# buckbaskin/parakeet_slam

Measured on AMD Instinct MI355X. Metric: particle*landmark EKF updates/sec (whole filter step), higher is better.
Workload: dtype f64

## Files before the change

include/parakeet_slam.h:

```cpp
#ifndef PARAKEET_SLAM_H_
#define PARAKEET_SLAM_H_

#include <stddef.h>
#include <stdint.h>

#ifdef __cplusplus
extern "C" {
#endif
#if defined(__GNUC__)
#pragma GCC visibility push(default)
#endif

#define PK_ABI_VERSION 1

typedef enum pk_status {
  PK_OK = 0,
  PK_ERR_INVALID = -1,
  PK_ERR_HIP = -2,
  PK_ERR_STATE = -3,
  PK_ERR_UNSUPPORTED = -4,
  PK_ERR_NOMEM = -5
} pk_status;

#define PK_LANDMARK_POTENTIAL 0x40000000
// ... 154 lines not shown
int pk_proposal_ranges_state(const pk_filter* f, int32_t* on);

int pk_proposal_grow(pk_filter* f, int32_t on);
int pk_proposal_grow_state(const pk_filter* f, int32_t* on);

int pk_assoc_unique(pk_filter* f, int32_t on);
int pk_assoc_unique_state(const pk_filter* f, int32_t* on);
int pk_assoc_unique_stats(pk_filter* f, int64_t out[4]);

int pk_set_shard(pk_filter* f, int64_t global_offset);
int pk_shard_max_logw(pk_filter* f, double* max_logw);
int64_t pk_shard_num_blocks(const pk_filter* f);
int pk_shard_block_totals(pk_filter* f, double gmax, int32_t weight_domain, double* totals);
int pk_shard_offspring(pk_filter* f, const double* global_totals, int64_t n_global_blocks,
                       int64_t first_block, int64_t global_particles, double u, int32_t last_shard,
                       int64_t* slot_hi);
int64_t pk_particle_bytes(const pk_filter* f);
int pk_pack_particles(pk_filter* f, const int64_t* local_idx, int64_t n, void* dev_buf);
int pk_adopt_particles(pk_filter* f, const int64_t* src, const void* dev_buf, int64_t n_received);

int pk_shard_max_logw_dev(pk_filter* f, double* dev_out);
int pk_shard_block_totals_dev(pk_filter* f, const double* dev_gmax, int32_t weight_domain,
                              double* dev_totals);
int pk_shard_plan_dev(pk_filter* f, const double* dev_global_totals, int64_t n_global_blocks,
                      int64_t first_block, int64_t global_particles, double u, int32_t last_shard,
                      int32_t world, int64_t* dev_ranges);
int pk_shard_pack_slots_dev(pk_filter* f, int64_t j0, int64_t j1, int64_t slot_lo, int64_t slot_hi, void* dev_buf);
int pk_shard_logw_dev(pk_filter* f, double* dev_out);
int pk_shard_plan_global_dev(pk_filter* f, const double* dev_global_logw, int64_t global_particles, const double* dev_gmax,
                             int32_t weight_domain, double u, int32_t last_shard, int32_t world, int64_t* dev_ranges);
int pk_shard_download_offspring(pk_filter* f, int64_t* slot_hi);
int pk_shard_pack_dev(pk_filter* f, const int64_t* ranges, int32_t world, int32_t rank, void* dev_buf);
int pk_shard_adopt_dev(pk_filter* f, int32_t rank, const void* dev_recv, int64_t n_received);

int pk_shard_local_span_dev(pk_filter* f, int64_t* dev_out2);
int pk_shard_adopt_local_dev(pk_filter* f, int32_t rank);
int pk_shard_adopt_remote_dev(pk_filter* f, int32_t rank, const void* dev_recv, int64_t n_received);
int pk_motion_range(pk_filter* f, double v, double w, double dt, uint64_t seed, uint64_t draw, int64_t p0, int64_t p1);
int pk_staged_takes_regs(pk_filter* f);
int pk_observe_staged_range(pk_filter* f, int32_t fresh, int64_t p0, int64_t p1, int32_t first, int32_t last);

int pk_shard_state_dev(pk_filter* f, double* dev_out);
int pk_shard_plan_balanced_dev(pk_filter* f, const double* dev_global_state, int64_t global_particles, const double* dev_gmax,
                               int32_t weight_domain, double u, int32_t world, int32_t rank, int64_t* dev_table);
int pk_shard_pack_balanced_dev(pk_filter* f, const int64_t* table, int32_t world, int32_t rank, void* dev_buf);
int pk_shard_adopt_balanced_dev(pk_filter* f, const int64_t* table, int32_t world, int32_t rank, const void* dev_recv,
                                int64_t n_received, int32_t mode);
int pk_shard_pack_balanced_loop_dev(pk_filter* f, int64_t keep, int64_t a0, int64_t a1, void* dev_buf);
int pk_shard_download_logical(pk_filter* f, int64_t* logical);
int pk_shard_upload_logical(pk_filter* f, const int64_t* logical);
int pk_shard_download_balanced_plan(pk_filter* f, int64_t* rel, int64_t* Hl, int32_t* alive);
int pk_shard_reset_placement(pk_filter* f);
int pk_shard_download_balanced_offspring(pk_filter* f, int64_t global_particles, int64_t* H);
int pk_shard_balanced_errors(pk_filter* f, int64_t* count);

#define PK_PROBE_LEN 79
int pk_probe(int32_t device, const double pose[3], const double mean[5], const double cov[25],
             const double blob[4], const double Qt[16], double* out);

enum {
  PK_MATH_LOG_FEW_ULP = 0,
  PK_MATH_PUB_LOG = 1,
  PK_MATH_PUB_RECIP = 2,
  PK_MATH_ATAN2 = 3,
  PK_MATH_ROUND_DOWN_F32 = 4,
  PK_MATH_KEY = 5,
  PK_MATH_FAR_BOUND = 6,
  PK_MATH_PR_FROM_PARTS = 7,
  PK_MATH_EKF_UPDATE = 9,
  PK_MATH_MATCH = 10,
  PK_MATH_COUNT = 11
};
int pk_probe_math(int32_t device, int32_t op, int64_t n, const double* in, double* out);

int pk_probe_bearing(int32_t device, int32_t what, int64_t n, const double* in, double* out);

int pk_probe_range(int32_t device, int32_t what, int64_t n, const double* in, double* out);

int pk_enable_timing(pk_filter* f, int32_t mask);
int pk_reset_timings(pk_filter* f);
int pk_timings(pk_filter* f, double ms[PK_T_COUNT], int64_t launches[PK_T_COUNT]);
int pk_observe_bytes(const pk_filter* f, int32_t num_blobs, int64_t* algorithmic, int64_t* moved);
int pk_colour_table_stats(pk_filter* f, int64_t out[4]);
enum {
  PK_ROUTE_NONE = 0,
  PK_ROUTE_KNOWN_IDS = 1,
  PK_ROUTE_ML_GENERAL = 2,
  PK_ROUTE_ML_HANDOFF = 3,
  PK_ROUTE_ML_SWEEP = 4,
  PK_ROUTE_ML_FUSED = 5,
  PK_ROUTE_ML_REGS = 6,
  PK_ROUTE_DENSE = 8,
  PK_ROUTE_ML_PUB_BIG = 9,
};
int pk_observe_route(const pk_filter* f);
int pk_download_sources(pk_filter* f, int32_t* src);
int pk_observe_flagged(pk_filter* f, int64_t* flagged, int64_t* cand_overflow);
int pk_observe_retry_rows(pk_filter* f, int64_t* wanted, int64_t* capacity);
int pk_observe_published(pk_filter* f, int32_t* published);
int pk_observe_pub_stats(pk_filter* f, int64_t stats[6]);
int pk_observe_lean_stats(pk_filter* f, int64_t out[3]);
int pk_observe_flags(pk_filter* f, uint8_t* flags);

typedef struct pk_rng pk_rng;
int pk_rng_create_numpy(uint32_t seed, pk_rng** out);
int pk_rng_create_python(uint32_t seed, pk_rng** out);
int pk_rng_destroy(pk_rng* r);
int pk_rng_standard_normal(pk_rng* r, int64_t n, double* out);
int pk_rng_random(pk_rng* r, int64_t n, double* out);

#if defined(__GNUC__)
#pragma GCC visibility pop
#endif
#ifdef __cplusplus
}
#endif
#endif
```

parakeet_slam_amd/_lib.py:

```python
from __future__ import annotations

import ctypes as C
import os

import numpy as np

from . import adaptive, mapsum, path

HERE = os.path.dirname(os.path.abspath(__file__))
LIB_PATH = os.path.join(HERE, "libparakeet_slam.so")

PK_OK = 0
PK_ERR_INVALID, PK_ERR_HIP, PK_ERR_STATE, PK_ERR_UNSUPPORTED, PK_ERR_NOMEM = -1, -2, -3, -4, -5
PK_WEIGHTS_LINEAR, PK_WEIGHTS_LOG = 0, 1
PK_PATH_UNIFORM = 2
PK_MAP_UNIFORM, PK_MAP_WEIGHTED = mapsum.UNIFORM, mapsum.WEIGHTED
PK_LANDMARK_POTENTIAL = 0x40000000
PK_GROW_VIEW_STATS_BYTES = 32
PK_T_NAMES = ("motion", "assoc", "observe", "weights", "resample", "summary", "materialise", "propose")
PK_T_COUNT = len(PK_T_NAMES)
PK_PROBE_LEN = 79
(PK_MATH_LOG_FEW_ULP, PK_MATH_PUB_LOG, PK_MATH_PUB_RECIP, PK_MATH_ATAN2, PK_MATH_ROUND_DOWN_F32, PK_MATH_KEY, PK_MATH_FAR_BOUND,
 PK_MATH_PR_FROM_PARTS) = range(8)
PK_MATH_EKF_UPDATE, PK_MATH_MATCH = 9, 10
# ... 68 lines not shown
    "pk_path_download": (C.c_int, [_h, C.c_int32, C.c_int32, _dp, _ip]),
    "pk_path_upload": (C.c_int, [_h, C.c_int32, C.c_int64, _dp, _ip]),
    "pk_path_trace": (C.c_int, [_h, _lp, C.c_int64, _dp]),
    "pk_path_summary": (C.c_int, [_h, _dp, _dp, _lp]),
    "pk_path_summary_weighted": (C.c_int, [_h, C.c_int32, _dp, _dp, _dp]),
    "pk_path_trunk_enable": (C.c_int, [_h, C.c_int32]),
    "pk_path_settle": (C.c_int, [_h, C.c_int32, C.c_int32]),
    "pk_path_trunk_shape": (C.c_int, [_h, C.POINTER(C.c_int32), _lp, _lp]),
    "pk_path_trunk_download": (C.c_int, [_h, C.c_int64, C.c_int64, _dp]),
    "pk_path_trunk_upload": (C.c_int, [_h, C.c_int64, C.c_int64, _dp]),
    "pk_path_trunk_summary": (C.c_int, [_h, C.c_int64, C.c_int64, _dp, _dp, _lp]),
    "pk_best_particle": (C.c_int, [_h, _lp, _dp]),
    "pk_step": (C.c_int, [_h, C.c_double, C.c_double, C.c_double, _dp, C.c_uint64, C.c_uint64, _dp, C.c_int32,
                          _ip, C.c_double, C.c_int32]),
    "pk_resample_adaptive": (C.c_int, [_h, C.c_double, C.c_int32, C.c_double, _lp]),
    "pk_step_adaptive": (C.c_int, [_h, C.c_double, C.c_double, C.c_double, _dp, C.c_uint64, C.c_uint64, _dp, C.c_int32,
                                   _ip, C.c_double, C.c_int32, C.c_double]),
    "pk_resample_stats": (C.c_int, [_h, _dp, C.POINTER(C.c_int32), _lp]),
    "pk_weight_sums": (C.c_int, [_h, C.c_int32, C.c_double, _dp]),
    "pk_summary_weighted": (C.c_int, [_h, C.c_int32, _dp, _dp, _dp]),
    "pk_odom_delta": (C.c_int, [_dp, _dp, C.c_double, _dp]),
    "pk_odom_sigmas": (C.c_int, [_dp, _dp, _dp]),
    "pk_motion_odom": (C.c_int, [_h, _dp, _dp, _dp, C.c_uint64, C.c_uint64]),
    "pk_propose": (C.c_int, [_h, C.c_double, C.c_double, C.c_double, _dp, C.c_uint64, C.c_uint64, _dp, C.c_int32, _ip, C.c_int32, _ip]),
    "pk_propose_odom": (C.c_int, [_h, _dp, _dp, _dp, C.c_uint64, C.c_uint64, _dp, C.c_int32, _ip, C.c_int32, _ip]),
    "pk_proposal_download": (C.c_int, [_h, _dp, _dp, _ip]),
    "pk_proposal_ranges": (C.c_int, [_h, C.c_int32]),
    "pk_proposal_ranges_state": (C.c_int, [_h, C.POINTER(C.c_int32)]),
    "pk_proposal_grow": (C.c_int, [_h, C.c_int32]),
    "pk_proposal_grow_state": (C.c_int, [_h, C.POINTER(C.c_int32)]),
    "pk_assoc_unique": (C.c_int, [_h, C.c_int32]),
    "pk_assoc_unique_state": (C.c_int, [_h, C.POINTER(C.c_int32)]),
    "pk_assoc_unique_stats": (C.c_int, [_h, _lp]),
    "pk_motion_odom_range": (C.c_int, [_h, _dp, _dp, C.c_uint64, C.c_uint64, C.c_int64, C.c_int64]),
    "pk_step_odom": (C.c_int, [_h, _dp, _dp, _dp, C.c_uint64, C.c_uint64, _dp, C.c_int32, _ip, C.c_double, C.c_int32, C.c_double]),
    "pk_shard_max_logw": (C.c_int, [_h, _dp]),
    "pk_shard_num_blocks": (C.c_int64, [_h]),
    "pk_shard_block_totals": (C.c_int, [_h, C.c_double, C.c_int32, _dp]),
    "pk_set_shard": (C.c_int, [_h, C.c_int64]),
    "pk_shard_offspring": (C.c_int, [_h, _dp, C.c_int64, C.c_int64, C.c_int64, C.c_double, C.c_int32, _lp]),
    "pk_shard_max_logw_dev": (C.c_int, [_h, C.c_void_p]),
    "pk_shard_block_totals_dev": (C.c_int, [_h, C.c_void_p, C.c_int32, C.c_void_p]),
    "pk_shard_plan_dev": (C.c_int, [_h, C.c_void_p, C.c_int64, C.c_int64, C.c_int64, C.c_double, C.c_int32, C.c_int32,
                                    C.c_void_p]),
    "pk_shard_logw_dev": (C.c_int, [_h, C.c_void_p]),
    "pk_shard_plan_global_dev": (C.c_int, [_h, C.c_void_p, C.c_int64, C.c_void_p, C.c_int32, C.c_double, C.c_int32, C.c_int32,
                                           C.c_void_p]),
    "pk_shard_download_offspring": (C.c_int, [_h, _lp]),
    "pk_shard_pack_dev": (C.c_int, [_h, _lp, C.c_int32, C.c_int32, C.c_void_p]),
    "pk_shard_pack_slots_dev": (C.c_int, [_h, C.c_int64, C.c_int64, C.c_int64, C.c_int64, C.c_void_p]),
    "pk_shard_adopt_dev": (C.c_int, [_h, C.c_int32, C.c_void_p, C.c_int64]),
    "pk_shard_local_span_dev": (C.c_int, [_h, C.c_void_p]),
    "pk_shard_adopt_local_dev": (C.c_int, [_h, C.c_int32]),
    "pk_shard_adopt_remote_dev": (C.c_int, [_h, C.c_int32, C.c_void_p, C.c_int64]),
    "pk_shard_state_dev": (C.c_int, [_h, C.c_void_p]),
    "pk_shard_plan_balanced_dev": (C.c_int, [_h, C.c_void_p, C.c_int64, C.c_void_p, C.c_int32, C.c_double, C.c_int32, C.c_int32,
                                             C.c_void_p]),
    "pk_shard_pack_balanced_dev": (C.c_int, [_h, _lp, C.c_int32, C.c_int32, C.c_void_p]),
    "pk_shard_adopt_balanced_dev": (C.c_int, [_h, _lp, C.c_int32, C.c_int32, C.c_void_p, C.c_int64, C.c_int32]),
    "pk_shard_pack_balanced_loop_dev": (C.c_int, [_h, C.c_int64, C.c_int64, C.c_int64, C.c_void_p]),
    "pk_shard_download_logical": (C.c_int, [_h, _lp]),
    "pk_shard_reset_placement": (C.c_int, [_h]),
    "pk_shard_upload_logical": (C.c_int, [_h, _lp]),
    "pk_shard_download_balanced_plan": (C.c_int, [_h, _lp, _lp, _ip]),
    "pk_shard_download_balanced_offspring": (C.c_int, [_h, C.c_int64, _lp]),
    "pk_shard_balanced_errors": (C.c_int, [_h, _lp]),
    "pk_motion_range": (C.c_int, [_h, C.c_double, C.c_double, C.c_double, C.c_uint64, C.c_uint64, C.c_int64, C.c_int64]),
    "pk_staged_takes_regs": (C.c_int, [_h]),
    "pk_observe_staged_range": (C.c_int, [_h, C.c_int32, C.c_int64, C.c_int64, C.c_int32, C.c_int32]),
    "pk_particle_bytes": (C.c_int64, [_h]),
    "pk_pack_particles": (C.c_int, [_h, _lp, C.c_int64, C.c_void_p]),
    "pk_adopt_particles": (C.c_int, [_h, _lp, C.c_void_p, C.c_int64]),
    "pk_probe": (C.c_int, [C.c_int32, _dp, _dp, _dp, _dp, _dp, _dp]),
    "pk_probe_math": (C.c_int, [C.c_int32, C.c_int32, C.c_int64, _dp, _dp]),
    "pk_probe_bearing": (C.c_int, [C.c_int32, C.c_int32, C.c_int64, _dp, _dp]),
    "pk_probe_range": (C.c_int, [C.c_int32, C.c_int32, C.c_int64, _dp, _dp]),
    "pk_scan_ranges": (C.c_int, [_h, _dp, _dp, C.c_int32]),
    "pk_scan_ranges_state": (C.c_int, [_h, C.POINTER(C.c_int32), C.POINTER(C.c_int32)]),
    "pk_enable_timing": (C.c_int, [_h, C.c_int32]),
    "pk_reset_timings": (C.c_int, [_h]),
    "pk_timings": (C.c_int, [_h, _dp, _lp]),
    "pk_observe_bytes": (C.c_int, [_h, C.c_int32, _lp, _lp]),
    "pk_colour_table_stats": (C.c_int, [_h, _lp]),
    "pk_observe_route": (C.c_int, [_h]),
    "pk_download_sources": (C.c_int, [_h, _ip]),
    "pk_observe_flagged": (C.c_int, [_h, _lp, _lp]),
    "pk_observe_retry_rows": (C.c_int, [_h, _lp, _lp]),
    "pk_grow_enable": (C.c_int, [_h, C.c_int32, C.c_int32, C.c_double]),
    "pk_grow_download": (C.c_int, [_h, C.c_int64, C.c_int64, _ip, _dp, _ip]),
    "pk_grow_upload": (C.c_int, [_h, C.c_int64, C.c_int64, _ip, _dp, _ip]),
    "pk_grow_shape": (C.c_int, [_h, C.POINTER(C.c_int32), C.POINTER(C.c_int32), C.POINTER(C.c_int32)]),
    "pk_grow_init": (C.c_int, [_h, C.c_int32, C.c_double]),
    "pk_grow_init_mode": (C.c_int, [_h, C.POINTER(C.c_int32), _dp]),
    "pk_grow_ranges": (C.c_int, [_h, C.c_int32]),
    "pk_grow_ranges_state": (C.c_int, [_h, C.POINTER(C.c_int32)]),
    "pk_grow_retire": (C.c_int, [_h, C.c_int32, C.c_int32]),
    "pk_grow_clocks_download": (C.c_int, [_h, C.c_int64, C.c_int64, _ip, _up, _ip, _ip, _up]),
    "pk_grow_clocks_upload": (C.c_int, [_h, C.c_int64, C.c_int64, _ip, _up, _ip, _ip, _up]),
    "pk_grow_view": (C.c_int, [_h, C.c_double, C.c_double, C.c_double, C.c_int32]),
    "pk_grow_view_state": (C.c_int, [_h, C.POINTER(C.c_int32), _dp, C.POINTER(C.c_int32)]),
    "pk_grow_view_stats": (C.c_int, [_h, _lp]),
    "pk_observe_published": (C.c_int, [_h, C.POINTER(C.c_int32)]),
    "pk_observe_flags": (C.c_int, [_h, _bp]),
    "pk_observe_pub_stats": (C.c_int, [_h, _lp]),
    "pk_observe_lean_stats": (C.c_int, [_h, _lp]),
    "pk_rng_create_numpy": (C.c_int, [C.c_uint32, C.POINTER(_h)]),
    "pk_rng_create_python": (C.c_int, [C.c_uint32, C.POINTER(_h)]),
    "pk_rng_destroy": (C.c_int, [_h]),
    "pk_rng_standard_normal": (C.c_int, [_h, C.c_int64, _dp]),
    "pk_rng_random": (C.c_int, [_h, C.c_int64, _dp]),
}


class PkError(RuntimeError):
    def __init__(self, status, message):
        super().__init__("parakeet_slam [%d]: %s" % (status, message))
        self.status = status


_lib = None


def load():
    global _lib
    if _lib is not None:
        return _lib
    if not os.path.exists(LIB_PATH):
        raise OSError(
            "%s is missing: build it with `python -m parakeet_slam_amd.build` (hipcc, gfx950). "
            "There is no CPU fallback for the particle update." % LIB_PATH
        )
    lib = C.CDLL(LIB_PATH)
    for name, (res, args) in SIGNATURES.items():
        fn = getattr(lib, name)
        fn.restype = res
        fn.argtypes = args
    ver = lib.pk_abi_version()
    if ver != PK_ABI_VERSION:
        raise OSError("libparakeet_slam.so has ABI %d, the binding expects %d: rebuild" % (ver, PK_ABI_VERSION))
    _lib = lib
    return lib


def check(status):
    if status != PK_OK:
        lib = load()
        msg = lib.pk_last_error().decode("utf-8", "replace") or lib.pk_status_string(status).decode()
        raise PkError(status, msg)


def dptr(a):
    return a.ctypes.data_as(_dp) if a is not None else None


def iptr(a):
    return a.ctypes.data_as(_ip) if a is not None else None


def lptr(a):
    return a.ctypes.data_as(_lp) if a is not None else None


def f64(a, shape=None):
    a = np.ascontiguousarray(a, dtype=np.float64)
    if shape is not None:
        a = a.reshape(shape)
# ... 455 lines not shown
        check(self._lib.pk_shard_state_dev(self._h, C.c_void_p(out_ptr)))

    def shard_plan_balanced_dev(self, gstate_ptr, global_particles, gmax_ptr, domain, u, world, rank, table_ptr):
        check(self._lib.pk_shard_plan_balanced_dev(self._h, C.c_void_p(gstate_ptr), int(global_particles), C.c_void_p(gmax_ptr),
                                                   int(domain), float(u), int(world), int(rank), C.c_void_p(table_ptr)))

    def shard_pack_balanced_dev(self, table, world, rank, buf_ptr):
        t = np.ascontiguousarray(table, dtype=np.int64)
        check(self._lib.pk_shard_pack_balanced_dev(self._h, lptr(t), int(world), int(rank), C.c_void_p(buf_ptr)))

    def shard_adopt_balanced_dev(self, table, world, rank, recv_ptr, n_received, mode):
        t = np.ascontiguousarray(table, dtype=np.int64)
        check(self._lib.pk_shard_adopt_balanced_dev(self._h, lptr(t), int(world), int(rank), C.c_void_p(recv_ptr), int(n_received),
                                                    int(mode)))

    def shard_pack_balanced_loop_dev(self, keep, a0, a1, buf_ptr):
        check(self._lib.pk_shard_pack_balanced_loop_dev(self._h, int(keep), int(a0), int(a1), C.c_void_p(buf_ptr)))

    def download_logical(self):
        out = np.empty(self.P, dtype=np.int64)
        check(self._lib.pk_shard_download_logical(self._h, lptr(out)))
        return out

    def upload_logical(self, logical):
        a = np.ascontiguousarray(logical, dtype=np.int64).reshape(self.P)
        check(self._lib.pk_shard_upload_logical(self._h, lptr(a)))

    def shard_download_balanced_plan(self):
        rel, Hl, alive = np.empty(self.P + 1, dtype=np.int64), np.empty(self.P, dtype=np.int64), np.empty(self.P, dtype=np.int32)
        check(self._lib.pk_shard_download_balanced_plan(self._h, lptr(rel), lptr(Hl), iptr(alive)))
        return rel, Hl, alive[alive >= 0]

    def reset_placement(self):
        check(self._lib.pk_shard_reset_placement(self._h))

    def shard_download_balanced_offspring(self, global_particles):
        out = np.empty(int(global_particles) + 1, dtype=np.int64)
        check(self._lib.pk_shard_download_balanced_offspring(self._h, int(global_particles), lptr(out)))
        return out

    def shard_balanced_errors(self):
        out = np.zeros(1, dtype=np.int64)
        check(self._lib.pk_shard_balanced_errors(self._h, lptr(out)))
        return int(out[0])

    def motion_range(self, v, w, dt, seed, draw, p0, p1):
        check(self._lib.pk_motion_range(self._h, float(v), float(w), float(dt), int(seed), int(draw), int(p0), int(p1)))

    def motion_odom_range(self, delta, alphas, seed, draw, p0, p1):
        d, a = f64(delta, (3,)), f64(alphas, (4,))
        check(self._lib.pk_motion_odom_range(self._h, dptr(d), dptr(a), int(seed), int(draw), int(p0), int(p1)))

    def staged_takes_regs(self):
        return bool(self._lib.pk_staged_takes_regs(self._h))

    def observe_staged_range(self, fresh, p0, p1, first, last):
        check(self._lib.pk_observe_staged_range(self._h, 1 if fresh else 0, int(p0), int(p1), 1 if first else 0, 1 if last else 0))

    ROUTES = {0: "none", 1: "known_ids", 2: "ml_general", 3: "ml_handoff", 4: "ml_sweep", 5: "ml_fused", 6: "ml_regs", 8: "dense", 9: "ml_pub_big"}

    def observe_route(self):
        return self.ROUTES[int(self._lib.pk_observe_route(self._h))]

    def observe_flagged(self):
        a, b = C.c_int64(), C.c_int64()
        check(self._lib.pk_observe_flagged(self._h, C.byref(a), C.byref(b)))
        return int(a.value), int(b.value)

    def observe_pub_stats(self):
        a = np.zeros(6, dtype=np.int64)
        check(self._lib.pk_observe_pub_stats(self._h, lptr(a)))
        return dict(zip(("entries", "contested_blobs", "multi_landmarks", "longest_list", "entry_capacity", "instance"), (int(v) for v in a)))

    def observe_lean_stats(self):
        a = np.zeros(3, dtype=np.int64)
        check(self._lib.pk_observe_lean_stats(self._h, lptr(a)))
        return dict(zip(("marked", "in_use", "fallbacks"), (int(v) for v in a)))

    def colour_table_stats(self):
        a = np.zeros(4, dtype=np.int64)
        check(self._lib.pk_colour_table_stats(self._h, lptr(a)))
        return dict(zip(("engaged", "depth", "scans", "materialisations"), (int(v) for v in a)))

    def grow_enable(self, preset_landmarks, reading_capacity=64, pair_threshold=30.0):
        check(self._lib.pk_grow_enable(self._h, int(preset_landmarks), int(reading_capacity), float(pair_threshold)))

    def grow_shape(self):
        a, b, c = C.c_int32(), C.c_int32(), C.c_int32()
        check(self._lib.pk_grow_shape(self._h, C.byref(a), C.byref(b), C.byref(c)))
        return int(a.value), int(b.value), int(c.value)

    def grow_init(self, mode, min_parallax=0.0):
        if isinstance(mode, str):
            if mode not in LANDMARK_INITS:
                raise ValueError("grow_init: %r is neither %s" % (mode, " nor ".join(repr(k) for k in LANDMARK_INITS)))
            mode = LANDMARK_INITS[mode]
        check(self._lib.pk_grow_init(self._h, int(mode), float(min_parallax)))

    def grow_init_mode(self):
        m, a = C.c_int32(), C.c_double()
        check(self._lib.pk_grow_init_mode(self._h, C.byref(m), C.byref(a)))
        return {v: k for k, v in LANDMARK_INITS.items()}[int(m.value)], float(a.value)

    def grow_ranges(self, on=True):
        check(self._lib.pk_grow_ranges(self._h, int(on)))

    def grow_ranges_state(self):
        on = C.c_int32()
        check(self._lib.pk_grow_ranges_state(self._h, C.byref(on)))
        return bool(on.value)

    def grow_download(self, p0=0, p1=None, counters=True, readings=True, slot_ids=True):
        p1 = self.P if p1 is None else p1
        _, S, R = self.grow_shape()
        n = p1 - p0
        c = np.empty((n, 4), dtype=np.int32) if counters else None
        r = np.empty((n, R, 8), dtype=np.float64) if readings else None
        s = np.empty((n, S), dtype=np.int32) if slot_ids else None
        check(self._lib.pk_grow_download(self._h, int(p0), int(p1), iptr(c), dptr(r), iptr(s)))
        return c, r, s

    def grow_upload(self, p0, p1, counters=None, readings=None, slot_ids=None):
        _, S, R = self.grow_shape()
        n = p1 - p0
        c = None if counters is None else np.ascontiguousarray(counters, dtype=np.int32).reshape(n, 4)
        r = None if readings is None else f64(readings, (n, R, 8))
        s = None if slot_ids is None else np.ascontiguousarray(slot_ids, dtype=np.int32).reshape(n, S)
        check(self._lib.pk_grow_upload(self._h, int(p0), int(p1), iptr(c), dptr(r), iptr(s)))

    def grow_retire(self, reading_max_age=0, potential_max_idle=0):
        check(self._lib.pk_grow_retire(self._h, int(reading_max_age), int(potential_max_idle)))

    def grow_clocks_download(self, p0=0, p1=None):
        p1 = self.P if p1 is None else p1
        _, S, R = self.grow_shape()
        n = p1 - p0
        c, sc = np.empty((n, 4), dtype=np.int32), np.empty((n, R), dtype=np.uint32)
        se, si = np.empty((n, S), dtype=np.int32), np.empty((n, S), dtype=np.int32)
        now = C.c_uint32(0)
        check(self._lib.pk_grow_clocks_download(self._h, int(p0), int(p1), iptr(c), sc.ctypes.data_as(_up), iptr(se), iptr(si), C.byref(now)))
        return c, sc, se, si, int(now.value)

    def grow_clocks_upload(self, p0, p1, counters=None, reading_scan=None, slot_seen=None, slot_idle=None, scan_now=None):
        _, S, R = self.grow_shape()
        n = p1 - p0
        c = None if counters is None else np.ascontiguousarray(counters, dtype=np.int32).reshape(n, 4)
        sc = None if reading_scan is None else np.ascontiguousarray(reading_scan, dtype=np.uint32).reshape(n, R)
        se = None if slot_seen is None else np.ascontiguousarray(slot_seen, dtype=np.int32).reshape(n, S)
        si = None if slot_idle is None else np.ascontiguousarray(slot_idle, dtype=np.int32).reshape(n, S)
        now = None if scan_now is None else C.byref(C.c_uint32(int(scan_now) & 0xFFFFFFFF))
        check(self._lib.pk_grow_clocks_upload(self._h, int(p0), int(p1), iptr(c), None if sc is None else sc.ctypes.data_as(_up), iptr(se),
                                              iptr(si), now))

    def grow_view(self, half_fov, range_min=0.0, range_max=float("inf"), confirmed_max_misses=0):
        check(self._lib.pk_grow_view(self._h, float(half_fov), float(range_min), float(range_max), int(confirmed_max_misses)))

    def grow_view_state(self):
        on, c, v = C.c_int32(), C.c_int32(), np.zeros(3, dtype=np.float64)
        check(self._lib.pk_grow_view_state(self._h, C.byref(on), dptr(v), C.byref(c)))
        return bool(on.value), (float(v[0]), float(v[1]), float(v[2])), int(c.value)

    def grow_view_stats(self):
        out = np.zeros(4, dtype=np.int64)
        check(self._lib.pk_grow_view_stats(self._h, out.ctypes.data_as(_lp)))
        return out

# ... 121 lines not shown
```

parakeet_slam_amd/csrc/pk_api.hip:

```cpp
#include "pk_filter.hpp"

extern "C" {
int pk_download_landmarks(pk_filter* f, int64_t p0, int64_t p1, double* means, double* covs, int32_t* counts);
int pk_upload_landmarks(pk_filter* f, int64_t p0, int64_t p1, const double* means, const double* covs, const int32_t* counts);
}

#ifdef PK_STAMPS
namespace pk { void debug_read_stamps(unsigned long long* out, bool reset); void debug_read_fused_stamps(unsigned long long* out, bool reset); void debug_read_regs_stamps(unsigned long long* out, bool reset); void debug_read_pub_stamps(unsigned long long* out, bool reset); void debug_read_pub_wave_stamps(unsigned long long* out, bool reset); }
#endif

namespace {
thread_local std::string g_last_error;
}

int fail(int code, const char* fmt, ...) {
  char buf[512];
  va_list ap;
  va_start(ap, fmt);
  vsnprintf(buf, sizeof(buf), fmt, ap);
  va_end(ap);
  g_last_error = buf;
  return code;
}

// ... 264 lines not shown
  delete f;
  return PK_OK;
}

int pk_set_stream(pk_filter* f, void* hip_stream) {
  if (!f) return fail(PK_ERR_INVALID, "pk_set_stream: NULL handle");
  int rc;
  if ((rc = use_device(f))) return rc;
  if ((rc = drain_timings(f))) return rc;
  PK_HIP(hipStreamSynchronize(f->stream));
  f->stream = hip_stream ? (hipStream_t)hip_stream : f->own_stream;
  return PK_OK;
}

int pk_synchronize(pk_filter* f) {
  if (!f) return fail(PK_ERR_INVALID, "pk_synchronize: NULL handle");
  int rc;
  if ((rc = use_device(f))) return rc;
  PK_HIP(hipStreamSynchronize(f->stream));
  return unique_error(f, "pk_synchronize");
}

int64_t pk_num_particles(const pk_filter* f) { return f ? f->d.P : -1; }
int32_t pk_num_landmarks(const pk_filter* f) { return f ? f->d.lay.L : -1; }
int64_t pk_device_bytes(const pk_filter* f) { return f ? (int64_t)f->mem.device_bytes() : -1; }

int pk_set_measurement_noise(pk_filter* f, const double Qt[16]) {
  if (!f || !Qt) return fail(PK_ERR_INVALID, "pk_set_measurement_noise: NULL argument");
  for (int i = 0; i < 16; ++i)
    if (!std::isfinite(Qt[i])) return fail(PK_ERR_INVALID, "Qt is not finite");
  double scale = 0;
  for (int i = 0; i < 4; ++i) scale = fmax(scale, fabs(Qt[i * 5]));
  bool coupled = false;
  for (int j = 1; j < 4; ++j)
    if (fabs(Qt[j]) > 1e-14 * scale || fabs(Qt[j * 4]) > 1e-14 * scale) coupled = true;
  for (int i = 1; i < 4; ++i)
    for (int j = i + 1; j < 4; ++j)
      if (fabs(Qt[i * 4 + j] - Qt[j * 4 + i]) > 1e-9 * (scale > 0 ? scale : 1.0)) coupled = true;
  int rc;
  if ((rc = use_device(f))) return rc;
  if (f->ct_updated) {
    bool untouched = false;
    if (f->ct_eligible && f->ct_built && !coupled && (rc = ct_maps_untouched(f, &untouched))) return rc;
    if (untouched) f->ct_updated = false;
    else if ((rc = ct_end(f))) return rc;
  }
  if (coupled && !f->dense && (rc = relayout(f, true, f->map_loaded))) return rc;
  for (int i = 0; i < 16; ++i) f->qt16[i] = Qt[i];
  f->qt_dense = coupled;
  f->qt = NoiseD{Qt[0], Qt[5], 0.5 * (Qt[6] + Qt[9]), 0.5 * (Qt[7] + Qt[13]), Qt[10], 0.5 * (Qt[11] + Qt[14]), Qt[15]};
  return PK_OK;
}

int pk_upload_map(pk_filter* f, const double* means, const double* covs, const uint8_t* immutable) {
  if (!f) return fail(PK_ERR_INVALID, "pk_upload_map: NULL handle");
  const MapLayout& lay = f->d.lay;
  const int L = lay.L;
  if (L > 0 && (!means || !covs)) return fail(PK_ERR_INVALID, "pk_upload_map: NULL means/covs");
  int rc;
  if ((rc = use_device(f))) return rc;
  bool need_dense = f->qt_dense;
  for (int l = 0; l < L; ++l) {
    for (int i = 0; i < 5; ++i)
      if (!std::isfinite(means[l * 5 + i])) return fail(PK_ERR_INVALID, "landmark %d: mean is not finite", l + 1);
    const int c = classify_covariance(covs + (size_t)l * 25, l);
    if (c < 0) return c;
    need_dense |= c == 1;
  }
  if ((rc = relayout(f, need_dense, false))) return rc;
  std::vector<unsigned char> slot(lay.slot_bytes, 0);
  std::vector<unsigned char> imm((size_t)lay.Lp, 0);
  for (int l = 0; l < L; ++l) {
    pack_landmark(lay, slot.data(), l, means + (size_t)l * 5, covs + (size_t)l * 25);
    imm[l] = immutable ? (immutable[l] != 0) : 0;
  }
  PK_HIP(hipMemcpyAsync(f->slot_tmp, slot.data(), lay.slot_bytes, hipMemcpyHostToDevice, f->stream));
  PK_HIP(hipMemcpyAsync(f->d.immutable, imm.data(), imm.size(), hipMemcpyHostToDevice, f->stream));
  launch_broadcast_slot(f->stream, f->d, f->slot_tmp);
  f->colour_rows_valid = true;
  f->ct_engaged = false;
  f->ct_built = false;
  f->ct_updated = false;
  f->ct_eligible = false;
  if (!f->dense && lay.Lp > 2 * kPubSmallThreads && L <= kRegsMaxL) {
    if ((rc = dev_lazy(f, &f->ct_base, (size_t)6 * lay.Lp))) return rc;
    PK_HIP(hipMemcpyAsync(f->ct_base, slot.data() + (size_t)F_CRR * lay.Lp * sizeof(double), (size_t)6 * lay.Lp * sizeof(double),
                          hipMemcpyHostToDevice, f->stream));
    f->ct_eligible = true;
  }
  PK_HIP(hipStreamSynchronize(f->stream));
  f->src_identity = true;
  f->map_loaded = true;
  return PK_OK;
}

int pk_upload_poses(pk_filter* f, const double* xyhw) {
  poses_change(f);
  if (!f || !xyhw) return fail(PK_ERR_INVALID, "pk_upload_poses: NULL argument");
  int rc;
  if ((rc = use_device(f))) return rc;
  const int64_t P = f->d.P;
  std::vector<double> soa((size_t)P * 4);
  for (int64_t i = 0; i < P; ++i) {
    soa[i] = xyhw[4 * i];
    soa[P + i] = xyhw[4 * i + 1];
    soa[2 * P + i] = xyhw[4 * i + 2];
    double w = xyhw[4 * i + 3];
    if (!(w >= 0.0) || !std::isfinite(w)) return fail(PK_ERR_INVALID, "pk_upload_poses: weight of particle %lld is negative, infinite or NaN", (long long)i);
    soa[3 * P + i] = std::log(w);
  }
  const int c = f->d.cur;
  PK_HIP(hipMemcpyAsync(f->d.x[c], soa.data(), P * 8, hipMemcpyHostToDevice, f->stream));
  PK_HIP(hipMemcpyAsync(f->d.y[c], soa.data() + P, P * 8, hipMemcpyHostToDevice, f->stream));
  PK_HIP(hipMemcpyAsync(f->d.h[c], soa.data() + 2 * P, P * 8, hipMemcpyHostToDevice, f->stream));
  PK_HIP(hipMemcpyAsync(f->d.logw[c], soa.data() + 3 * P, P * 8, hipMemcpyHostToDevice, f->stream));
  PK_HIP(hipStreamSynchronize(f->stream));
  f->gmax_fused = false;
  path_clear(f);
  return PK_OK;
}

int pk_upload_pose(pk_filter* f, int64_t p, const double xyhw[4]) {
  if (!f || !xyhw) return fail(PK_ERR_INVALID, "pk_upload_pose: NULL argument");
  if (p < 0 || p >= f->d.P) return fail(PK_ERR_INVALID, "pk_upload_pose: particle %lld of %lld", (long long)p, (long long)f->d.P);
  for (int i = 0; i < 3; ++i)
    if (!std::isfinite(xyhw[i])) return fail(PK_ERR_INVALID, "pk_upload_pose: pose component %d is not finite", i);
  if (!(xyhw[3] >= 0.0) || !std::isfinite(xyhw[3])) return fail(PK_ERR_INVALID, "pk_upload_pose: the weight is negative, infinite or NaN");
  int rc;
  if ((rc = use_device(f))) return rc;
  f->pose_part_ok = false;
  const double v4[4] = {xyhw[0], xyhw[1], xyhw[2], std::log(xyhw[3])};
  const int c = f->d.cur;
  double* const dst[4] = {f->d.x[c] + p, f->d.y[c] + p, f->d.h[c] + p, f->d.logw[c] + p};
  for (int i = 0; i < 4; ++i) PK_HIP(hipMemcpyAsync(dst[i], &v4[i], 8, hipMemcpyHostToDevice, f->stream));
  PK_HIP(hipStreamSynchronize(f->stream));
  f->gmax_fused = false;
  return PK_OK;
}

int pk_download_poses(pk_filter* f, double* xyhw) {
  if (!f || !xyhw) return fail(PK_ERR_INVALID, "pk_download_poses: NULL argument");
  int rc;
  if ((rc = use_device(f))) return rc;
  const int64_t P = f->d.P;
  std::vector<double> soa((size_t)P * 4);
  const int c = f->d.cur;
  PK_HIP(hipMemcpyAsync(soa.data(), f->d.x[c], P * 8, hipMemcpyDeviceToHost, f->stream));
  PK_HIP(hipMemcpyAsync(soa.data() + P, f->d.y[c], P * 8, hipMemcpyDeviceToHost, f->stream));
  PK_HIP(hipMemcpyAsync(soa.data() + 2 * P, f->d.h[c], P * 8, hipMemcpyDeviceToHost, f->stream));
  PK_HIP(hipMemcpyAsync(soa.data() + 3 * P, f->d.logw[c], P * 8, hipMemcpyDeviceToHost, f->stream));
  PK_HIP(hipStreamSynchronize(f->stream));
  for (int64_t i = 0; i < P; ++i) {
    xyhw[4 * i] = soa[i];
    xyhw[4 * i + 1] = soa[P + i];
    xyhw[4 * i + 2] = soa[2 * P + i];
    xyhw[4 * i + 3] = std::exp(soa[3 * P + i]);
  }
  return PK_OK;
}

int pk_download_log_weights(pk_filter* f, double* logw) {
  if (!f || !logw) return fail(PK_ERR_INVALID, "pk_download_log_weights: NULL argument");
  int rc;
  if ((rc = use_device(f))) return rc;
  PK_HIP(hipMemcpyAsync(logw, f->d.logw[f->d.cur], (size_t)f->d.P * sizeof(double), hipMemcpyDeviceToHost, f->stream));
  PK_HIP(hipStreamSynchronize(f->stream));
  return PK_OK;
}

int pk_upload_log_weights(pk_filter* f, const double* logw) {
  if (!f || !logw) return fail(PK_ERR_INVALID, "pk_upload_log_weights: NULL argument");
// ... 607 lines not shown
```

parakeet_slam_amd/csrc/pk_api_observe.hip:

```cpp
#include "pk_filter.hpp"

static int host_word(pk_filter* f, unsigned** p) {
  if (*p) return PK_OK;
  int rc;
  if ((rc = host_alloc(f, p, 16, hipHostMallocDefault))) return rc;
  **p = 0u;
  return PK_OK;
}

int refuse_bearing(const pk_filter* f, const char* who, const char* what) {
  if (f && f->model == PK_MODEL_BEARING)
    return fail(PK_ERR_UNSUPPORTED, "%s: the bearing measurement model (pk_set_measurement_model) has no kernel for %s; "
                                    "pk_set_measurement_model(f, PK_MODEL_REFERENCE) takes it", who, what);
  return PK_OK;
}

static void observe_done(pk_filter* f) {
  f->src_identity = true;
  f->d.alt = nullptr;
  f->gmax_fused = true;
}

static ColourTable ct_view(const pk_filter* f) { return ColourTable{f->ct_tab, f->ct_depth}; }
static int ensure_colour_rows(pk_filter* f) {
  if (f->colour_rows_valid) return PK_OK;
  {
    Span t(f, PK_T_MATERIALISE);
    launch_colour_rows(f->stream, f->d, ct_view(f), f->ct_qt);
  }
  PK_LAUNCH_CHECK("ensure_colour_rows");
  f->colour_rows_valid = true;
  f->ct_whole += 1;
  return PK_OK;
}
int colour_rows_for_download(pk_filter* f, int64_t p0, int64_t p1) {
  if (f->colour_rows_valid || p0 >= p1) return PK_OK;
  if (p0 == 0 && p1 == f->d.P) return ensure_colour_rows(f);
  {
    Span t(f, PK_T_MATERIALISE);
    ParticleRange range;
    range.p0 = p0;
    range.p1 = p1;
    launch_colour_rows(f->stream, f->d, ct_view(f), f->ct_qt, range);
  }
  PK_LAUNCH_CHECK("colour_rows_for_download");
  return PK_OK;
}
int ct_end(pk_filter* f) {
  f->ct_eligible = false;
  f->ct_engaged = false;
  return ensure_colour_rows(f);
}
static bool ct_state_ok(const pk_filter* f) {
  if (f->opt.colour_table == 0 || !f->ct_eligible || f->ct_sharded || f->grow_on || f->dense || !f->ct_base) return false;
  if (f->d.lay.Lp <= 2 * kPubSmallThreads) return false;
  const int margin = f->opt.colour_table_margin >= 0 ? f->opt.colour_table_margin : std::min(16, f->ct_depth > 0 ? f->ct_depth / 2 : 16);
  if (margin > 0 && f->ct_built && f->ct_seen && (int64_t)*reinterpret_cast<volatile unsigned*>(f->ct_seen) + margin >= f->ct_depth) return false;
  return true;
}
int ct_maps_untouched(pk_filter* f, bool* untouched) {
  *untouched = false;
  if (!f->ct_max_dev || !f->ct_seen) return PK_OK;
  PK_HIP(hipMemsetAsync(f->ct_max_dev + 1, 0, sizeof(unsigned), f->stream));
  launch_colour_counts_any(f->stream, f->d, f->ct_max_dev + 1);
  PK_LAUNCH_CHECK("colour counts");
  PK_HIP(hipMemcpyAsync(f->ct_seen + 1, f->ct_max_dev + 1, sizeof(unsigned), hipMemcpyDeviceToHost, f->stream));
  PK_HIP(hipStreamSynchronize(f->stream));
  *untouched = f->ct_seen[1] == 0u;
  return PK_OK;
}
static int ct_engage(pk_filter* f) {
  int rc;
  const int Lp = f->d.lay.Lp;
  const int depth = f->ct_built ? f->ct_depth : f->opt.colour_table_depth;
  if ((rc = host_word(f, &f->ct_seen))) return rc;
  if ((rc = dev_lazy(f, &f->ct_max_dev, 16))) return rc;
  const bool same_qt = memcmp(&f->ct_qt, &f->qt, sizeof(NoiseD)) == 0;
  if (f->ct_built && same_qt && f->ct_depth == depth) return PK_OK;
  if (!f->ct_tab || f->ct_depth != depth) {
    PK_HIP(hipStreamSynchronize(f->stream));
    dev_free(f, &f->ct_tab);
    if ((rc = dev_alloc(f, &f->ct_tab, (size_t)depth * 6 * Lp))) return rc;
    f->ct_depth = depth;
  }
  f->ct_qt = f->qt;
  launch_colour_table(f->stream, f->ct_base, f->ct_tab, depth, Lp, f->ct_qt);
  PK_HIP(hipMemsetAsync(f->ct_max_dev, 0, 16, f->stream));
  *f->ct_seen = 0u;
  PK_LAUNCH_CHECK("colour table");
  f->ct_built = true;
  return PK_OK;
}

static int64_t retry_rows(const pk_filter* f) {
  return std::min<int64_t>(f->d.P, std::max<int64_t>(std::max<int64_t>(1024, f->d.P / 16), f->retry_rows_min));
}
static int ensure_handoff(pk_filter* f, int B, int slots, bool lists = true, bool retry_only = false) {
  if (retry_only && f->retry_seen) {
    const int64_t wanted = *reinterpret_cast<volatile unsigned*>(f->retry_seen);
    if (wanted > retry_rows(f)) f->retry_rows_min = std::min<int64_t>(f->d.P, wanted + wanted / 4);
  }
  const int64_t rows = retry_only ? retry_rows(f) : f->d.P;
  const int64_t need_l = lists ? rows * (int64_t)f->d.lay.Lp * (slots == kSweepSlots ? 2 : 1) : 0;
  const int64_t need_b = lists ? rows * (int64_t)std::max(B, 1) : 0;
  int rc;
  if (retry_only && (rc = dev_lazy(f, &f->fh.row_of, (size_t)f->d.P))) return rc;
  if ((rc = dev_reserve(f, &f->fh.lmpass, &f->fh_cap_l, need_l, need_l))) return rc;
  if ((rc = dev_reserve(f, &f->fh.bcount, &f->fh_cap_b, need_b, need_b))) return rc;
  return dev_lazy(f, &f->fh.pflag, (size_t)f->d.P);
}

constexpr int64_t kPubSmallAutoWork = 5000000;
constexpr int kPubSmallAutoLandmarks = 128;

static ScanPlan plan_scan(const pk_filter* f, int B, bool use_grid, int ncell, int n9, bool want_fast, bool finalize, bool grow, bool whole) {
  ScanPlan p;
  if (!use_grid) return p;
  p.kind = ScanKind::General;
  if (f->model == PK_MODEL_BEARING) return p;
  if (f->uq.on) return p;
  const int L = f->d.lay.L, Lp = f->d.lay.Lp;
  const bool sweep = L > kFastMaxL || f->opt.fast_observe >= 2;
  auto sweep_fits = [&] { return observe_sweep_plan(f->d, B).grid > 0; };
  auto limited = [&](int ecap) { return f->opt.pub_entry_limit > 0 && ecap > f->opt.pub_entry_limit ? f->opt.pub_entry_limit : ecap; };
  const bool lists_both_ways = f->opt.pub_step && f->opt.cand_lists;
  const bool onepass = want_fast && !finalize && f->opt.fast_observe == 1 && B > 0 && (!grow || (lists_both_ways && B <= 32 * 176));
  if (onepass && f->opt.fused_step && !sweep && n9 > 0 && fused_lds_bytes(ncell, B, n9) <= kFusedMaxLds &&
      (!grow || (step_pub_entry_capacity_small(B) > 0 && B <= 32 * 32))) {
    const bool wanted = grow || (f->opt.pub_small >= 0 ? f->opt.pub_small != 0
                                                   : f->d.P * (int64_t)L >= kPubSmallAutoWork && L >= kPubSmallAutoLandmarks);
    p.kind = wanted && lists_both_ways && step_pub_entry_capacity_small(B) > 0 ? ScanKind::PubSmall : ScanKind::Fused;
    p.route = PK_ROUTE_ML_FUSED;
    if (p.kind == ScanKind::PubSmall) {
      p.cand_slots = kCandSlots;
      p.ecap = limited(step_pub_entry_capacity_small(B));
    }
  } else if (onepass && f->opt.regs_step && L > kFastMaxL && L <= kRegsMaxL && n9 > 0 && regs_lds_bytes(ncell, B, n9) <= kMaxDynLds &&
             (!grow || (step_pub_entry_capacity(B) > 0 && regs_cand_lds_bytes(Lp, B) <= kMaxDynLds && B <= 32 * 96))) {
    p.lists = f->opt.regs_retry && sweep_fits();
    p.retry = p.lists && !grow;
    p.slots = p.lists ? kSweepSlots : kFastSlots;
    p.kind = ScanKind::Regs;
    p.route = PK_ROUTE_ML_REGS;
    if (f->opt.cand_lists && regs_cand_lds_bytes(Lp, B) <= kMaxDynLds) {
      p.cand_slots = kCandSlots;
      p.ecap = f->opt.pub_step ? limited(step_pub_entry_capacity(B)) : 0;
      if (p.ecap > 0) p.kind = f->opt.far_prune || grow ? ScanKind::Pub : ScanKind::PubRegs;
    }
  } else if (onepass && lists_both_ways && L > kRegsMaxL && L <= kPubBigMaxL && step_pub_big_entry_capacity(B) > 0 && sweep_fits()) {
    p.kind = ScanKind::PubBig;
    p.route = PK_ROUTE_ML_PUB_BIG;
    p.lists = true;
    p.retry = !grow;
    p.slots = kSweepSlots;
    p.cand_slots = 2 * kCandSlots;
    p.ecap = limited(step_pub_big_entry_capacity(B));
    if (f->opt.duo_on) {
      step_pub_duo_limits(B, Lp, f->opt.duo_on, &p.duo);
      p.duo.ecap = limited(p.duo.ecap);
      p.duo.park_limit = f->opt.duo_park_limit;
    }
  } else if (want_fast && !grow && !finalize && f->opt.fast_observe && B > 0 && (sweep ? sweep_fits() : observe_fast_lds_bytes(B) <= kMaxDynLds)) {
    p.kind = sweep ? ScanKind::HandoffSweep : ScanKind::HandoffFast;
    p.route = sweep ? PK_ROUTE_ML_SWEEP : PK_ROUTE_ML_HANDOFF;
    p.lists = true;
    p.slots = sweep && (B >= 3000 || f->opt.fast_observe == 3) ? kSweepSlots : kFastSlots;
    if (f->opt.cand_lists && L < 65535) p.cand_slots = 2 * kCandSlots;
  }
  p.publish = p.ecap > 0;
// ... 148 lines not shown
  if ((rc = dev_lazy(f, &f->cand_dev, Lpp * 3))) return rc;
  if (!plan.publish) return PK_OK;
  if ((rc = big ? dev_lazy(f, &f->erec_dev2, Lpp * 2) : dev_lazy(f, &f->erec_dev, Lpp))) return rc;
  if ((rc = dev_lazy(f, &f->npass_dev, Lpp))) return rc;
  if ((rc = dev_lazy(f, &f->far_dev, Lpp * 3))) return rc;
  if (big && (rc = dev_lazy(f, &f->prim_dev, prim_table_uint4(f->d.lay.Lp)))) return rc;
  return ensure_inverse_lists(f, B, plan.cand_slots);
}
static int onepass_prepare(pk_filter* f, const AssocLaunch& al, PubTables* pub, int64_t ref = 0) {
  int rc;
  const ScanPlan& plan = al.plan;
  *pub = PubTables();
  f->pub_ecap = plan.ecap;
  if (!plan.cand_slots) return PK_OK;
  if ((rc = ensure_list_buffers(f, plan, al.scan.B))) return rc;
  Span t(f, PK_T_ASSOC);
  CandidatesLaunch cl{};
  cl.rec = f->cand_dev;
  cl.over = ctl_cand_over(f);
  cl.slots = plan.cand_slots;
  cl.ref_particle = ref;
  cl.pose_sums4 = f->out4;
  if (f->pose_part_ok)
    cl.pose_part = f->pose_part;
  else
    launch_summary_partials(f->stream, f->d, f->partial, f->out4);
  CandTable& cand = pub->cand;
  cand.rec = f->cand_dev;
  cand.over = ctl_cand_over(f);
  cand.slots = plan.cand_slots;
  if (!plan.publish) {
    launch_candidates(f->stream, f->d, al.scan, cl);
    return PK_OK;
  }
  const bool big = plan.kind == ScanKind::PubBig;
  pub->erec = big ? f->erec_dev2 : f->erec_dev;
  pub->glist = f->glist_dev;
  pub->bcnt = f->bcnt_dev;
  pub->brec = f->brec_dev;
  pub->binfo = f->binfo_dev;
  pub->npass = f->npass_dev;
  pub->stats = ctl_pub_stats(f);
  pub->skip_pub = ctl_skip_pub(f);
  pub->skip_cand = ctl_skip_cand(f);
  pub->ecap = plan.ecap;
  if (big) {
    pub->gate4 = f->gate4_dev;
    pub->prim = f->prim_dev;
    pub->skip_duo = ctl_skip_duo(f);
    pub->skip_big = ctl_skip_big(f);
  }
  pub->duo = plan.duo;
  cl.bcnt = pub->bcnt;
  cl.brec = pub->brec;
  cl.npass = pub->npass;
  if (plan.far) cl.far = f->far_dev;
  if (plan.colour_table) cl.ct = ct_view(f);
  if (!big) cl.qt = &f->ct_qt;
  launch_candidates(f->stream, f->d, al.scan, cl);
  CandEntriesLaunch ce;
  ce.pub = *pub;
  ce.pruned = plan.far;
  if (plan.flag_fold) {
    ce.flag_all = f->fh.pflag;
    ce.n_flagged = ctl_n_flagged(f);
  }
  launch_cand_entries(f->stream, f->d, al.scan, ce);
  cand.far = cl.far;
  if (!big) cand.skip_cand = ctl_skip_cand(f);
  return PK_OK;
}
static int onepass_launch(pk_filter* f, const AssocLaunch& al, const ObserveExtras& ex, const PubTables& pub, const ParticleRange& range) {
  const ScanPlan& plan = al.plan;
  FastHandoff fh = f->fh;
  fh.n_flagged = ctl_n_flagged(f);
  fh.flags_only = true;
  Span t(f, PK_T_OBSERVE);
  ObserveExtras e1 = ex;
  e1.flip = false;
  if (plan.colour_table) {
    e1.ctab = f->ct_tab;
    e1.ctab_depth = f->ct_depth;
    e1.ctab_max = f->ct_max_dev;
  }
  e1.lean = f->opt.pub_lean;
  e1.lean_stats = ctl_pub_stats(f);
  switch (plan.kind) {
    case ScanKind::PubBig:
      if (plan.duo.tbytes > 0) launch_step_pub_duo(f->stream, f->d, al.scan, fh, f->qt, e1, pub, range);
      launch_step_pub_big(f->stream, f->d, al.scan, fh, f->qt, e1, pub, range);
      break;
    case ScanKind::PubSmall:
    case ScanKind::Pub:
    case ScanKind::PubRegs:
      launch_step_pub(f->stream, f->d, al.scan, fh, f->qt, e1, pub, range);
      if (plan.kind != ScanKind::PubRegs) break;
      [[fallthrough]];
    case ScanKind::Regs:
      launch_step_regs(f->stream, f->d, al.scan, fh, f->qt, e1, f->opt.regs_warm, pub.cand, range);
      break;
    case ScanKind::Fused:
      launch_step_fused(f->stream, f->d, al.scan, fh, f->qt, e1);
      break;
    default:
      break;
  }
  if (plan.flag_range) launch_flag_range_if(f->stream, ctl_skip_pub(f), fh.pflag, fh.n_flagged, range.p0, range.end(f->d.P));
  return PK_OK;
}
static int ensure_sweep_results(pk_filter* f, const SweepPlan& plan) {
  const size_t need = (size_t)plan.grid * plan.results_per_wg;
  return dev_reserve(f, &f->sweep_results, &f->sweep_cap, need, need);
}
static int onepass_finish(pk_filter* f, const AssocLaunch& al, const ObserveExtras& ex, const CandTable& cand) {
  int rc;
  FastHandoff fh = f->fh;
  fh.n_flagged = ctl_n_flagged(f);
  fh.flags_only = true;
  if (al.plan.retry) {
    Span t(f, PK_T_ASSOC);
    const SweepPlan plan = observe_sweep_plan(f->d, al.scan.B);
    if ((rc = ensure_sweep_results(f, plan))) return rc;
    FastHandoff fr = f->fh;
    fr.slots = kSweepSlots;
    fr.retry = true;
    fr.n_flagged = ctl_n_flagged(f);
    fr.row_next = ctl_retry_rows(f);
    fr.row_cap = retry_rows(f);
    const CandTable unpruned = cand.far ? CandTable() : cand;
    launch_assoc_grid(f->stream, f->d, al.scan, f->ids_dev, false, fr, unpruned);
    ObserveExtras e3 = ex;
    e3.flip = false;
    e3.sweep_only_value = 2;
    e3.n_flagged = ctl_n_flagged(f);
    launch_observe_sweep(f->stream, f->d, al.scan, fr, f->qt, e3, plan, f->sweep_results);
    (void)host_word(f, &f->retry_seen);
    if (f->retry_seen) (void)hipMemcpyAsync(f->retry_seen, ctl_retry_rows(f), sizeof(unsigned), hipMemcpyDeviceToHost, f->stream);
    (void)hipGetLastError();
  }
  Span t(f, PK_T_ASSOC);
  launch_assoc_grid(f->stream, f->d, al.scan, f->ids_dev, false, fh);
  ObserveExtras e2 = ex;
  e2.only_flagged = f->fh.pflag;
  e2.n_flagged = ctl_n_flagged(f);
  launch_observe(f->stream, f->d, al.scan, f->ids_dev, f->qt, e2);
  return PK_OK;
}

int grow_bookkeeping(pk_filter* f, const char* who, const ScanTables& scan, int32_t B) {
  {
    Span t(f, PK_T_OBSERVE);
    launch_new_landmarks(f->stream, f->d, f->grow, f->grow_init, f->qt.q00, f->ids_dev, scan.blobs, B, f->grow_bits ? f->unm_dev : nullptr,
                         f->unm_words, f->grow_bits ? f->fh.pflag : nullptr,
                         f->grow_ranges ? scan.rng : nullptr);
    if (f->retire.on()) {
      f->retire.t += 1u;
      if (f->view.on)
        PK_HIP(hipMemsetAsync(f->view.stats, 0, 2 * sizeof(unsigned long long), f->stream));
      launch_grow_retire(f->stream, f->d, f->grow, f->retire, f->view);
    }
  }
  const std::string what = std::string(who) + " (new landmarks)";
  PK_LAUNCH_CHECK(what.c_str());
  return PK_OK;
}

int observe_impl(pk_filter* f, const double* blobs, int32_t B, const int32_t* ids, int32_t* ids_out,
                        bool reset) {
  if (!f) return fail(PK_ERR_INVALID, "pk_observe: NULL handle");
  int rc;
  RangeScan rs;
  if (!is_staged_scan(f, blobs, B)) {
    if ((rc = ranges_take(f, "pk_observe", B, &rs))) return rc;
  } else if (f->staged.with_ranges && (rc = refuse_ranges(f, "pk_observe", B, f->staged.B))) {
    f->staged.valid = false;
    return rc;
  }
  if ((rc = check_scan_shape(f, "pk_observe", blobs, B))) return rc;
  if (f->split.active) return fail(PK_ERR_STATE, "pk_observe: a split observe is in progress (pk_observe_staged_range with last = 1 ends it)");
  if ((rc = use_device(f))) return rc;
  if ((rc = check_scan_values(f, "pk_observe", blobs, B, &ids))) return rc;
  const bool grow = f->grow_on && B > 0;
  if (grow && ids) return refuse_grow_ids("pk_observe");
  if (grow && f->dense)
    return fail(PK_ERR_STATE, "pk_observe: the new-landmark bookkeeping (pk_grow_enable) writes the compact landmark layout; this filter "
                              "is on the dense one (a covariance or Qt that couples position and colour)");
  f->uq.last = false;
  if (!ids && B > 0 && (rc = unique_check(f, "pk_observe", B))) {
    f->staged.valid = false;
    f->dense_staged.clear();
    return rc;
  }
  f->ct_updated = true;
  if (f->dense) return dense_observe(f, blobs, B, ids, ids_out, reset, true);
  ObserveExtras ex;
  ex.reset = reset;
  ex.model = f->model;
  if (ids) {
    if ((rc = ct_end(f))) return rc;
    f->staged.valid = false;
    KnownScan ks;
    if ((rc = upload_known_scan(f, blobs, B, ids, false, &ks, &rs))) return rc;
    if (ks.lay.rng) ex.rng = reinterpret_cast<const double*>(f->scan_dev + ks.lay.rng);
    ex.single_sightings = ks.single_sightings;
    ex.gmax_key = ctl_gmax_key(f);
    {
      Span t(f, PK_T_OBSERVE);
      launch_observe(f->stream, f->d, known_scan_tables(f, ks, B), known_chains(f, ks), f->qt, ex);
    }
    PK_LAUNCH_CHECK("pk_observe");
    observe_done(f);
    f->route = PK_ROUTE_KNOWN_IDS;
    return return_ids(f, ids_out, B, ids);
  }
  AssocLaunch al;
  if ((rc = enqueue_association(f, blobs, B, false, ids_out == nullptr, &al, grow, true, &rs))) return rc;
  ex.rng = al.scan.rng;
  const ScanPlan& plan = al.plan;
  if (plan.colour_table ? (rc = ct_engage(f)) : (rc = ct_end(f))) return rc;
  f->grow_bits = false;
  if (grow && plan.onepass()) {
    const int words = 2 * ((B + 63) / 64);
    if ((rc = dev_reserve(f, &f->unm_dev, &f->unm_cap, (int64_t)f->d.P * words, (int64_t)f->d.P * (words + words / 4 + 2)))) return rc;
    f->unm_words = words;
    ex.unm = f->unm_dev;
    ex.unm_words = words;
    f->grow_bits = true;
  }
  ex.gmax_key = ctl_gmax_key(f);
  if (plan.onepass()) {
    PubTables pub;
    if ((rc = onepass_prepare(f, al, &pub))) return rc;
    if ((rc = onepass_launch(f, al, ex, pub, ParticleRange()))) return rc;
    if (plan.colour_table) {
      Span t(f, PK_T_ASSOC);
      launch_colour_rows(f->stream, f->d, ct_view(f), f->ct_qt, ParticleRange(), f->fh.pflag, ctl_n_flagged(f));
      (void)hipMemcpyAsync(f->ct_seen, f->ct_max_dev, sizeof(unsigned), hipMemcpyDeviceToHost, f->stream);
      (void)hipGetLastError();
      f->colour_rows_valid = false;
      f->ct_engaged = true;
      f->ct_scans += 1;
    }
    if ((rc = onepass_finish(f, al, ex, pub.cand))) return rc;
  } else {
    Span t(f, PK_T_OBSERVE);
    if (plan.lists) {
      ObserveExtras e1 = ex;
      e1.flip = false;
      if (plan.kind == ScanKind::HandoffSweep) {
        const SweepPlan sweep = observe_sweep_plan(f->d, B);
        if ((rc = ensure_sweep_results(f, sweep))) return rc;
        launch_observe_sweep(f->stream, f->d, al.scan, f->fh, f->qt, e1, sweep, f->sweep_results);
      } else {
        launch_observe_fast(f->stream, f->d, al.scan, f->fh, f->qt, e1);
      }
      ex.only_flagged = f->fh.pflag;
      ex.n_flagged = ctl_n_flagged(f);
    }
    launch_observe(f->stream, f->d, al.scan, f->ids_dev, f->qt, ex);
  }
  PK_LAUNCH_CHECK("pk_observe");
  observe_done(f);
  if (grow && (rc = grow_bookkeeping(f, "pk_observe", al.scan, B))) return rc;
  if ((rc = return_ids(f, ids_out, B, nullptr))) return rc;
  return ids_out && B > 0 ? unique_error(f, "pk_observe") : PK_OK;
}

int proposal_scan(pk_filter* f, const double* blobs, int32_t B, const int32_t* ids, ProposalScan* out, const RangeScan* rs, bool grow) {
  int rc;
  *out = ProposalScan();
  f->ct_updated = true;
  f->uq.last = false;
  if (ids) {
    if ((rc = ct_end(f))) return rc;
    f->staged.valid = false;
    KnownScan ks;
    if ((rc = upload_known_scan(f, blobs, B, ids, true, &ks, rs))) return rc;
    if (ks.lay.rng) out->rng = reinterpret_cast<const double*>(f->scan_dev + ks.lay.rng);
    f->gmax_fused = false;
    out->scan = known_scan_tables(f, ks, B);
    out->known = known_chains(f, ks);
    out->known.n_unmatched = 0;
    out->ids = reinterpret_cast<int32_t*>(f->scan_dev + ks.lay.ids);
    return PK_OK;
  }
  AssocLaunch al;
  if ((rc = enqueue_association(f, blobs, B, false, false, &al, grow, true, rs))) return rc;
  if (al.plan.onepass()) return fail(PK_ERR_UNSUPPORTED, "pk_propose: the scan did not take the general association");
  f->grow_bits = false;
  if ((rc = ct_end(f))) return rc;
  out->scan = al.scan;
  out->rng = al.scan.rng;
  out->ids = f->ids_dev;
  return PK_OK;
}
void proposal_observed(pk_filter* f, bool known) {
  observe_done(f);
  f->route = known ? PK_ROUTE_KNOWN_IDS : PK_ROUTE_ML_GENERAL;
}

extern "C" {

int pk_observe(pk_filter* f, const double* blobs, int32_t B, const int32_t* ids, int32_t* ids_out) {
  return observe_impl(f, blobs, B, ids, ids_out, false);
}

int pk_observe_fresh(pk_filter* f, const double* blobs, int32_t B, const int32_t* ids, int32_t* ids_out) {
  return observe_impl(f, blobs, B, ids, ids_out, true);
}

int pk_observe_staged(pk_filter* f, int32_t fresh) {
  if (!f) return fail(PK_ERR_INVALID, "pk_observe_staged: NULL handle");
  if (f->dense && !f->dense_staged.empty()) {
    std::vector<double> b;
    b.swap(f->dense_staged);
    return observe_impl(f, b.data(), (int32_t)(b.size() / 4), nullptr, nullptr, fresh != 0);
  }
  if (!f->staged.valid) return fail(PK_ERR_STATE, "pk_observe_staged: no staged scan (pk_stage_scan)");
  return observe_impl(f, staged_blobs(f->staged), f->staged.B, nullptr, nullptr, fresh != 0);
}

int pk_staged_takes_regs(pk_filter* f) {
  if (!f || f->dense || f->grow_on || !f->staged.valid) return 0;
// ... 95 lines not shown
    PK_HIP(hipMemcpyAsync(w, ctl_n_flagged(f), sizeof(w), hipMemcpyDeviceToHost, f->stream));
    PK_HIP(hipStreamSynchronize(f->stream));
  }
  if (flagged) *flagged = w[0];
  if (cand_overflow) *cand_overflow = w[1];
  return PK_OK;
}
int pk_observe_retry_rows(pk_filter* f, int64_t* wanted, int64_t* capacity) {
  if (!f) return fail(PK_ERR_INVALID, "pk_observe_retry_rows: NULL handle");
  int rc;
  if ((rc = use_device(f))) return rc;
  PK_HIP(hipStreamSynchronize(f->stream));
  if (wanted) *wanted = f->retry_seen ? (int64_t)*f->retry_seen : 0;
  if (capacity) *capacity = retry_rows(f);
  return PK_OK;
}
int pk_observe_flags(pk_filter* f, uint8_t* flags) {
  if (!f || !flags) return fail(PK_ERR_INVALID, "pk_observe_flags: NULL argument");
  int rc;
  if ((rc = use_device(f))) return rc;
  const bool onepass = f->route == PK_ROUTE_ML_REGS || f->route == PK_ROUTE_ML_FUSED || f->route == PK_ROUTE_ML_PUB_BIG;
  if (onepass && f->fh.pflag) {
    PK_HIP(hipMemcpyAsync(flags, f->fh.pflag, (size_t)f->d.P, hipMemcpyDeviceToHost, f->stream));
    PK_HIP(hipStreamSynchronize(f->stream));
  } else {
    memset(flags, 0, (size_t)f->d.P);
  }
  return PK_OK;
}
int pk_observe_published(pk_filter* f, int32_t* published) {
  if (!f || !published) return fail(PK_ERR_INVALID, "pk_observe_published: NULL argument");
  int rc;
  if ((rc = use_device(f))) return rc;
  *published = 0;
  if (f->scan_dev && (f->route == PK_ROUTE_ML_REGS || f->route == PK_ROUTE_ML_FUSED || f->route == PK_ROUTE_ML_PUB_BIG) && f->pub_ecap > 0) {
    unsigned w = 1u;
    PK_HIP(hipMemcpyAsync(&w, ctl_skip_pub(f), sizeof(w), hipMemcpyDeviceToHost, f->stream));
    PK_HIP(hipStreamSynchronize(f->stream));
    *published = w == 0u ? 1 : 0;
  }
  return PK_OK;
}
int pk_observe_pub_stats(pk_filter* f, int64_t stats[6]) {
  if (!f || !stats) return fail(PK_ERR_INVALID, "pk_observe_pub_stats: NULL argument");
  int rc;
  if ((rc = use_device(f))) return rc;
  for (int i = 0; i < 6; ++i) stats[i] = 0;
  if (f->scan_dev && (f->route == PK_ROUTE_ML_REGS || f->route == PK_ROUTE_ML_FUSED || f->route == PK_ROUTE_ML_PUB_BIG) && f->pub_ecap > 0) {
    unsigned w[4] = {0u, 0u, 0u, 0u}, sk[2] = {1u, 1u};
    PK_HIP(hipMemcpyAsync(w, ctl_pub_stats(f), sizeof(w), hipMemcpyDeviceToHost, f->stream));
    PK_HIP(hipMemcpyAsync(&sk[0], ctl_skip_pub(f), sizeof(unsigned), hipMemcpyDeviceToHost, f->stream));
    PK_HIP(hipMemcpyAsync(&sk[1], ctl_skip_duo(f), sizeof(unsigned), hipMemcpyDeviceToHost, f->stream));
    PK_HIP(hipStreamSynchronize(f->stream));
    for (int i = 0; i < 4; ++i) stats[i] = w[i];
    stats[4] = f->pub_ecap;
    stats[5] = sk[0] != 0u ? 0 : (f->route == PK_ROUTE_ML_PUB_BIG && f->opt.duo_on && sk[1] == 0u) ? 1 + f->opt.duo_on : 1;
  }
  return PK_OK;
}
int pk_observe_lean_stats(pk_filter* f, int64_t out[3]) {
  if (!f || !out) return fail(PK_ERR_INVALID, "pk_observe_lean_stats: NULL argument");
  int rc;
  if ((rc = use_device(f))) return rc;
  for (int i = 0; i < 3; ++i) out[i] = 0;
  if (f->scan_dev && f->route == PK_ROUTE_ML_REGS && f->pub_ecap > 0 && f->d.lay.Lp > 2 * kPubThreads && f->d.lay.Lp <= 4 * kPubThreads) {
    unsigned w[3] = {0u, 0u, 0u}, sk = 1u;
    PK_HIP(hipMemcpyAsync(w, ctl_pub_stats(f) + 4, sizeof(w), hipMemcpyDeviceToHost, f->stream));
    PK_HIP(hipMemcpyAsync(&sk, ctl_skip_pub(f), sizeof(unsigned), hipMemcpyDeviceToHost, f->stream));
    PK_HIP(hipStreamSynchronize(f->stream));
    if (sk == 0u)
      for (int i = 0; i < 3; ++i) out[i] = w[i];
  }
  return PK_OK;
}
int pk_observe_bytes(const pk_filter* f, int32_t B, int64_t* algorithmic, int64_t* moved) {
  if (!f) return fail(PK_ERR_INVALID, "pk_observe_bytes: NULL handle");
  const int64_t P = f->d.P, L = f->d.lay.L;
  if (algorithmic) *algorithmic = P * L * 28 * (int64_t)sizeof(double);
  const int64_t rows = f->ct_engaged ? 16 : 28;
  if (moved) *moved = P * (L * (rows * (int64_t)sizeof(double) + 8) + (int64_t)B * 32);
  return PK_OK;
}

int pk_colour_table_stats(pk_filter* f, int64_t out[4]) {
  if (!f || !out) return fail(PK_ERR_INVALID, "pk_colour_table_stats: NULL argument");
  out[0] = f->ct_engaged ? 1 : 0;
  out[1] = f->ct_built ? f->ct_depth : f->opt.colour_table_depth;
  out[2] = f->ct_scans;
  out[3] = f->ct_whole;
  return PK_OK;
}

}
```

parakeet_slam_amd/csrc/pk_colour.hpp:

```cpp
#pragma once
#include "pk_math.hpp"

namespace pk {

__device__ __forceinline__ unsigned colour_level(int count) { return (unsigned)(count & ~kPotentialBit) >> 1; }

constexpr unsigned kColourBeyondMax = 4096;

__device__ inline Sym3<double> colour_block_at(const double* tab, int depth, int Lp, int l, unsigned level, const Noise<double>& qt) {
  if (level > (unsigned)depth + kColourBeyondMax) level = (unsigned)depth + kColourBeyondMax;
  unsigned k = level < (unsigned)depth ? level : (unsigned)depth - 1u;
  const double* t = tab + ((size_t)k * 6) * Lp + l;
  Sym3<double> C{t[0], t[(size_t)Lp], t[2 * (size_t)Lp], t[3 * (size_t)Lp], t[4 * (size_t)Lp], t[5 * (size_t)Lp]};
#pragma unroll 1
  for (; k < level; ++k) C = colour_block_step(C, qt);
  return C;
}

}
```

parakeet_slam_amd/csrc/pk_filter.hpp:

```cpp
#pragma once
#include <hip/hip_runtime.h>

#include <cmath>
#include <cstdarg>
#include <cstdio>
#include <cstring>
#include <functional>
#include <new>
#include <string>
#include <vector>

#include "../../include/parakeet_slam.h"
#include "pk_devmem.hpp"
#include "pk_kernels.hpp"
#include "pk_pub_layout.hpp"
#include "pk_scan_block.hpp"

using namespace pk;

int fail(int code, const char* fmt, ...);

#define PK_HIP(call)                                                                         \
  do {                                                                                       \
    hipError_t e_ = (call);                                                                  \
// ... 14 lines not shown
struct TimedSpan {
  int slot;
  hipEvent_t a, b;
};

struct HipRaw {
  int device_alloc(void** p, size_t bytes) {
    hipError_t e = hipMalloc(p, bytes);
    if (e == hipSuccess) return PK_OK;
    (void)hipGetLastError();
    return fail(PK_ERR_NOMEM, "hipMalloc of %zu bytes failed: %s", bytes, hipGetErrorString(e));
  }
  void device_free(void* p) { (void)hipFree(p); }
  int host_alloc(void** p, size_t bytes, unsigned flags) {
    hipError_t e = hipHostMalloc(p, bytes, flags);
    if (e == hipSuccess) return PK_OK;
    (void)hipGetLastError();
    return fail(e == hipErrorOutOfMemory ? PK_ERR_NOMEM : PK_ERR_HIP, "hipHostMalloc of %zu bytes failed: %s", bytes, hipGetErrorString(e));
  }
  void host_free(void* p) { (void)hipHostFree(p); }
};

enum class ScanKind {
  Brute,
  General,
  HandoffFast,
  HandoffSweep,
  Fused,
  PubSmall,
  Regs,
  PubRegs,
  Pub,
  PubBig,
};
struct ScanPlan {
  ScanKind kind = ScanKind::Brute;
  int route = PK_ROUTE_ML_GENERAL;
  int slots = kFastSlots;
  bool lists = false;
  bool retry = false;
  int cand_slots = 0;
  bool publish = false;
  int ecap = 0;
  bool far = false;
  DuoLimits duo;
  bool flag_fold = false, flag_range = false;
  bool colour_table = false;
  bool onepass() const { return kind >= ScanKind::Fused; }
  bool ranged() const { return kind >= ScanKind::Regs; }
};

struct AssocLaunch {
  ScanTables scan;
  ScanPlan plan;
};

struct RangeScan {
  bool armed = false, any = false;
  std::vector<double> rv;
};

struct Options {
  int assoc_kernel = 0;
  int assoc_dup = 1;
  int fast_observe = 1;
  int timing_stride = 1;
  int upload_kernel = 1;
  int fused_step = 1;
  int cand_lists = 1;
  int pub_step = 1;
  int pub_small = -1;
  int pub_lean = 1;
  int far_prune = 1;
  int duo_on = 0;
  int duo_park_limit = -1;
  int pub_entry_limit = 0;
  int regs_step = 1;
  int regs_retry = 1;
  int regs_warm = 1;
  int split_reserve_cus = 16;
  int colour_table_depth = 1024;
  int colour_table_margin = -1;
  int colour_table = -1;
  int map_sum_groups = 0;
  int map_match_groups = 0;
};

enum class Take {
  Range,
  Flag,
  Tri,
};
struct OptionRow {
  const char* name;
  int Options::*member;
  Take take;
  int64_t lo, hi;
  const char* refusal;
};
inline constexpr OptionRow kOptionTable[] = {
    {"assoc_kernel", &Options::assoc_kernel, Take::Range, 0, 1, "assoc_kernel: 0 (colour grid) or 1 (brute force)"},
    {"assoc_dup", &Options::assoc_dup, Take::Flag, 0, 0, nullptr},
    {"fast_observe", &Options::fast_observe, Take::Range, 0, 3,
     "fast_observe: 0 (general kernels), 1 (default), 2 (always the sweep kernel) or 3 (... with eight slots)"},
    {"timing_stride", &Options::timing_stride, Take::Range, 1, 1000000, "timing_stride: 1 .. 1000000"},
    {"upload_kernel", &Options::upload_kernel, Take::Flag, 0, 0, nullptr},
    {"fused_step", &Options::fused_step, Take::Flag, 0, 0, nullptr},
    {"cand_lists", &Options::cand_lists, Take::Flag, 0, 0, nullptr},
    {"pub_step", &Options::pub_step, Take::Flag, 0, 0, nullptr},
    {"pub_small", &Options::pub_small, Take::Tri, 0, 0, nullptr},
    {"far_prune", &Options::far_prune, Take::Flag, 0, 0, nullptr},
    {"pub_lean", &Options::pub_lean, Take::Flag, 0, 0, nullptr},
    {"pub_duo", &Options::duo_on, Take::Range, 0, 2,
     "pub_duo: 0 (off), 1 (two 512-lane workgroups per CU) or 2 (three 256-lane workgroups per CU)"},
    {"pub_duo_park_limit", &Options::duo_park_limit, Take::Range, -1, 65535, "pub_duo_park_limit: -1 (what LDS holds) .. 65535"},
    {"pub_entry_limit", &Options::pub_entry_limit, Take::Range, 0, 65534, "pub_entry_limit: 0 (what LDS holds) .. 65534"},
    {"regs_step", &Options::regs_step, Take::Flag, 0, 0, nullptr},
    {"regs_retry", &Options::regs_retry, Take::Range, 0, 1, "regs_retry: 0 or 1"},
    {"regs_warm", &Options::regs_warm, Take::Range, 0, 2, "regs_warm: 0 (off), 1 (mean rows) or 2 (whole slot)"},
    {"split_reserve_cus", &Options::split_reserve_cus, Take::Range, 0, 128, "split_reserve_cus: 0..128"},
    {"colour_table_depth", &Options::colour_table_depth, Take::Range, 8, 32768,
     "colour_table_depth: 8 .. 32768 levels (the table stays below 4 GB: 32-bit offsets)"},
    {"colour_table_margin", &Options::colour_table_margin, Take::Range, -1, 32768,
     "colour_table_margin: -1 (auto), 0 (the host never leaves the mode for the table's end) or levels"},
    {"map_sum_groups", &Options::map_sum_groups, Take::Range, 0, 1024, "map_sum_groups: 0 (chosen from the shape) .. 1024"},
    {"map_match_groups", &Options::map_match_groups, Take::Range, 0, 1024, "map_match_groups: 0 (chosen from the shape) .. 1024"},
};

struct pk_filter {
  int device = 0;
  hipStream_t own_stream = nullptr;
  hipStream_t stream = nullptr;
  DeviceState d{};
  NoiseD qt{0.1, 0.1, 0.0, 0.0, 0.1, 0.0, 0.1};
  double qt16[16] = {0.1, 0, 0, 0, 0, 0.1, 0, 0, 0, 0, 0.1, 0, 0, 0, 0, 0.1};
  int model = PK_MODEL_REFERENCE;
  bool qt_dense = false;
  bool dense = false;
  std::vector<double> dense_staged;
  bool map_loaded = false;
  bool src_identity = true;
  int64_t nblocks = 0;
  DevMem<HipRaw> mem;
  double* z_dev = nullptr;
  unsigned char* scan_dev = nullptr;
  size_t scan_cap = 0;
  bool gmax_fused = false;
  int32_t* ids_dev = nullptr;
  int64_t ids_cap = 0;
  double* g_totals = nullptr;
  double* g_offsets = nullptr;
  int64_t gblocks_cap = 0;
  double* gl_clocal = nullptr;
  double* gl_totals = nullptr;
  double* gl_offsets = nullptr;
  int64_t gl_cap = 0;
  int64_t* hi_dev = nullptr;
  unsigned* plan_ticket = nullptr;
  int64_t* idx_dev = nullptr;
  int64_t* srcs_dev = nullptr;
  int64_t* rlohi_dev = nullptr;
  int64_t rlohi_cap = 0;
  BalancedBuffers bal{};
  int64_t bal_m = -1;
  int64_t bal_loop_keep = -1;
  int64_t loop_lo = INT64_MIN, loop_hi = INT64_MAX;
  Options opt;
  struct Staged {
    bool valid = false;
    int B = 0;
    unsigned char* st = nullptr;
    int slot = 0;
    BlobGrid g{};
    int n9 = 0;
    bool use_grid = false;
    MlScanLayout lay{};
    bool uploaded = false;
    bool with_ranges = false;
    bool ranged = false;
  } staged;
  struct Ranges {
    bool armed = false, any = false;
    int32_t B = 0;
    std::vector<double> rv;
  } rng;
  int route = PK_ROUTE_NONE;
  unsigned* bcnt_dev = nullptr;
  uint4* brec_dev = nullptr;
  int64_t bcand_cap = 0;
  uint4* cand_dev = nullptr;
  uint4* erec_dev = nullptr;
  uint4* erec_dev2 = nullptr;
  unsigned* binfo_dev = nullptr;
  unsigned char* npass_dev = nullptr;
  unsigned* unm_dev = nullptr;
  int unm_words = 0;
  int64_t unm_cap = 0;
  bool grow_bits = false;
  uint4* prim_dev = nullptr;
  float4* gate4_dev = nullptr;
  uint4* far_dev = nullptr;
  unsigned* glist_dev = nullptr;
  struct Split {
    bool active = false;
    AssocLaunch al;
    PubTables pub;
    bool reset = false;
  } split;
  bool ct_eligible = false;
  bool ct_updated = false;
  bool ct_sharded = false;
  bool ct_built = false;
  bool ct_engaged = false;
  bool colour_rows_valid = true;
  double* ct_base = nullptr;
  double* ct_tab = nullptr;
  int ct_depth = 0;
  NoiseD ct_qt{};
  unsigned* ct_max_dev = nullptr;
  unsigned* ct_seen = nullptr;
  int64_t ct_scans = 0, ct_whole = 0;
  bool adopt_local_done = false;
  int pub_ecap = 0;
  uint4* sweep_results = nullptr;
  size_t sweep_cap = 0;
  unsigned* retry_seen = nullptr;
  int64_t retry_rows_min = 0;
  FastHandoff fh{};
  int64_t fh_cap_l = 0, fh_cap_b = 0;
  static constexpr int kRing = 8;
  unsigned char* stage[kRing] = {nullptr};
  hipEvent_t stage_done[kRing] = {nullptr};
  uint64_t upload_seq = 0;
  uint64_t slot_seq[kRing] = {0};
  uint64_t event_seq[kRing] = {0};
  size_t stage_cap = 0;
  int stage_next = 0;
  double* partial = nullptr;
  double* gmax = nullptr;
  double* clocal = nullptr;
  double* totals = nullptr;
  double* offsets = nullptr;
  double* sum = nullptr;
  double* out4 = nullptr;
  double* pose_part = nullptr;
  bool pose_part_ok = false;
  double* ms_part = nullptr;
  double* ms_res = nullptr;
  size_t ms_cap = 0;
  double* mm_ref = nullptr;
  int32_t* mm_refi = nullptr;
  double* mm_res = nullptr;
  size_t mm_rows = 0;
  double* mm_part = nullptr;
  size_t mm_part_cap = 0;
  int32_t* mm_match = nullptr;
  size_t mm_match_cap = 0;
  PathRing path{};
  int64_t* pt_idx = nullptr;
  double* pt_out = nullptr;
  int64_t pt_cap = 0, pt_out_cap = 0;
  unsigned* ps_cnt = nullptr;
  double* ps_ref = nullptr;
  double* ps_part = nullptr;
  double* ps_res = nullptr;
  int64_t ps_rows = 0;
  int32_t* pw_idx = nullptr;
  double* pw_wgt = nullptr;
  double* pw_ref = nullptr;
  double* pw_part = nullptr;
  double* pw_res = nullptr;
  int64_t pw_rows = 0;
  PathTrunk trunk{};
  double* ad_s2 = nullptr;
  double* ad_words = nullptr;
  double* ad_part = nullptr;
  GateOutcome* ad_out = nullptr;
  int64_t ad_calls = 0;
  GrowState grow{};
  GrowInit grow_init{};
  bool grow_on = false;
  bool grow_ranges = false;
  RetireState retire{};
  RetireView view{};
  struct Proposal {
    double* pose = nullptr;
    double* zero = nullptr;
    double* xi = nullptr;
    double* dlogw = nullptr;
    int32_t* used = nullptr;
    bool valid = false;
    bool ranges = false;
    bool grow = false;
  } prop;
  struct Unique {
    bool on = false;
    bool last = false;
    unsigned long long* stats = nullptr;
    unsigned long long* seen = nullptr;
  } uq;
  int32_t* anc = nullptr;
  unsigned char* slot_tmp = nullptr;
  uint32_t timing_mask = 0;
  int64_t timing_seen[PK_T_COUNT] = {0};
// ... 154 lines not shown
```

parakeet_slam_amd/csrc/pk_k_colour.hip:

```cpp
#include <algorithm>

#include "pk_colour.hpp"
#include "pk_device.hpp"

namespace pk {

__global__ void __launch_bounds__(64) k_colour_table(const double* base, double* tab, int depth, int Lp, Noise<double> qt) {
  const int l = blockIdx.x * 64 + threadIdx.x;
  if (l >= Lp) return;
  Sym3<double> C{base[l], base[(size_t)Lp + l], base[2 * (size_t)Lp + l], base[3 * (size_t)Lp + l], base[4 * (size_t)Lp + l],
                 base[5 * (size_t)Lp + l]};
#pragma unroll 1
  for (int k = 0; k < depth; ++k) {
    double* t = tab + ((size_t)k * 6) * Lp + l;
    t[0] = C.a;
    t[(size_t)Lp] = C.b;
    t[2 * (size_t)Lp] = C.c;
    t[3 * (size_t)Lp] = C.d;
    t[4 * (size_t)Lp] = C.e;
    t[5 * (size_t)Lp] = C.f;
    C = colour_block_step(C, qt);
  }
}

void launch_colour_table(hipStream_t s, const double* base_dev, double* tab_dev, int depth, int Lp, const NoiseD& qt) {
  if (depth <= 0 || Lp <= 0) return;
  hipLaunchKernelGGL(k_colour_table, dim3((unsigned)((Lp + 63) / 64)), dim3(64), 0, s, base_dev, tab_dev, depth, Lp,
                     make_noise(qt.q00, qt.rr, qt.rg, qt.rb, qt.gg, qt.gb, qt.bb));
}

struct ColourRowsArgs {
  unsigned char* map;
  size_t slot_bytes, count_off;
  const int32_t* src;
  const unsigned char* pflag;
  const unsigned* n_flagged;
  const double* tab;
  int depth, Lp;
  int64_t P;
  int64_t p0, p1;
  Noise<double> qt;
};
__global__ void __launch_bounds__(256) k_colour_rows(ColourRowsArgs a) {
  if (a.pflag && *a.n_flagged == 0u) return;
  for (int64_t p = a.p0 + blockIdx.x; p < a.p1; p += gridDim.x) {
    int64_t sl = p;
    if (a.pflag) {
      if (a.pflag[p] == 0) continue;
      sl = a.src[p];
      if (sl < 0 || sl >= a.P) continue;
    }
    unsigned char* slot = a.map + (size_t)sl * a.slot_bytes;
    double* f = reinterpret_cast<double*>(slot);
    const int* cnt = reinterpret_cast<const int*>(slot + a.count_off);
    for (int l = threadIdx.x; l < a.Lp; l += 256) {
      const Sym3<double> C = colour_block_at(a.tab, a.depth, a.Lp, l, colour_level(cnt[l]), a.qt);
      f[(size_t)F_CRR * a.Lp + l] = C.a;
      f[(size_t)F_CRG * a.Lp + l] = C.b;
      f[(size_t)F_CRB * a.Lp + l] = C.c;
      f[(size_t)F_CGG * a.Lp + l] = C.d;
      f[(size_t)F_CGB * a.Lp + l] = C.e;
      f[(size_t)F_CBB * a.Lp + l] = C.f;
    }
  }
}

void launch_colour_rows(hipStream_t s, DeviceState& d, const ColourTable& ct, const NoiseD& qt, const ParticleRange& range,
                        const unsigned char* pflag_dev, const unsigned* n_flagged_dev) {
  const int64_t p0 = range.p0, p1 = range.end(d.P);
  if (!ct.tab || d.P == 0 || p0 < 0 || p1 > d.P || p0 >= p1) return;
  ColourRowsArgs a;
  a.map = d.map[d.mcur];
  a.slot_bytes = d.lay.slot_bytes;
  a.count_off = d.lay.count_off;
  a.src = d.src[d.cur];
  a.pflag = pflag_dev;
  a.n_flagged = n_flagged_dev;
  a.tab = ct.tab;
  a.depth = ct.depth;
  a.Lp = d.lay.Lp;
  a.P = d.P;
  a.p0 = p0;
  a.p1 = p1;
  a.qt = make_noise(qt.q00, qt.rr, qt.rg, qt.rb, qt.gg, qt.gb, qt.bb);
  const int64_t grid = std::min<int64_t>(p1 - p0, 4 * (int64_t)device_cu_count());
  hipLaunchKernelGGL(k_colour_rows, dim3((unsigned)grid), dim3(256), 0, s, a);
}

__global__ void __launch_bounds__(256) k_colour_counts_any(const unsigned char* map, size_t slot_bytes, size_t count_off, int L, int64_t P,
                                                           unsigned* any_dev) {
  bool any = false;
  for (int64_t p = blockIdx.x; p < P; p += gridDim.x) {
    const int* cnt = reinterpret_cast<const int*>(map + (size_t)p * slot_bytes + count_off);
    for (int l = threadIdx.x; l < L; l += 256) any |= cnt[l] != 0;
  }
  if (any) atomicOr(any_dev, 1u);
}

void launch_colour_counts_any(hipStream_t s, DeviceState& d, unsigned* any_dev) {
  if (d.P <= 0 || d.lay.L <= 0) return;
  const int64_t grid = std::min<int64_t>(d.P, 4 * (int64_t)device_cu_count());
  hipLaunchKernelGGL(k_colour_counts_any, dim3((unsigned)grid), dim3(256), 0, s, d.map[d.mcur], d.lay.slot_bytes, d.lay.count_off, d.lay.L,
                     d.P, any_dev);
}

}
```

parakeet_slam_amd/csrc/pk_k_mathprobe.hip:

```cpp
#include "pk_device.hpp"
#include "pk_filter.hpp"
#include "pk_pub_math.hpp"
#include "pk_range_math.hpp"

namespace pk {

__device__ __forceinline__ double bits_to_double(unsigned long long b) {
  double x;
  memcpy(&x, &b, 8);
  return x;
}

__device__ __forceinline__ Landmark<double> landmark_of_row(const double* __restrict__ r, int count) {
  Landmark<double> lm;
  lm.mx = r[F_MX];
  lm.my = r[F_MY];
  lm.mr = r[F_MR];
  lm.mg = r[F_MG];
  lm.mb = r[F_MB];
  lm.pxx = r[F_PXX];
  lm.pxy = r[F_PXY];
  lm.pyy = r[F_PYY];
  lm.crr = r[F_CRR];
  lm.crg = r[F_CRG];
  lm.crb = r[F_CRB];
  lm.cgg = r[F_CGG];
  lm.cgb = r[F_CGB];
  lm.cbb = r[F_CBB];
  lm.count = count;
  return lm;
}
__device__ __forceinline__ void row_of_landmark(const Landmark<double>& lm, double* __restrict__ r) {
  r[F_MX] = lm.mx;
  r[F_MY] = lm.my;
  r[F_MR] = lm.mr;
  r[F_MG] = lm.mg;
  r[F_MB] = lm.mb;
  r[F_PXX] = lm.pxx;
  r[F_PXY] = lm.pxy;
  r[F_PYY] = lm.pyy;
  r[F_CRR] = lm.crr;
  r[F_CRG] = lm.crg;
  r[F_CRB] = lm.crb;
  r[F_CGG] = lm.cgg;
  r[F_CGB] = lm.cgb;
  r[F_CBB] = lm.cbb;
}

constexpr int kEkfIn = 31, kEkfOut = 17, kMatchIn = 23, kMatchOut = 5;

template <bool COLOUR, bool KNOWN, bool FRO>
__device__ __forceinline__ double ekf_variant(Landmark<double>& lm, double sx, double sy, const BlobT<double>& z,
                                              const Noise<double>& qt, bool immutable, double zhat0, double& prod) {
  return ekf_update<double, COLOUR>(lm, sx, sy, z, qt, immutable, nullptr, KNOWN ? &zhat0 : nullptr, FRO ? &prod : nullptr);
}

template <int OP>
__global__ void __launch_bounds__(256) k_probe_math(const double* __restrict__ in, double* __restrict__ out, int64_t n) {
  const int64_t i = (int64_t)blockIdx.x * blockDim.x + threadIdx.x;
  if (i >= n) return;
  if constexpr (OP == PK_MATH_LOG_FEW_ULP) {
    out[i] = log_few_ulp(in[i]);
  } else if constexpr (OP == PK_MATH_PUB_LOG) {
    out[i] = pub_log(in[i]);
  } else if constexpr (OP == PK_MATH_PUB_RECIP) {
    out[i] = pub_recip(in[i]);
  } else if constexpr (OP == PK_MATH_ATAN2) {
    out[i] = pk_atan2(in[2 * i], in[2 * i + 1]);
  } else if constexpr (OP == PK_MATH_ROUND_DOWN_F32) {
    out[i] = (double)pub_round_down_to_float(in[i]);
  } else if constexpr (OP == PK_MATH_KEY) {
    const unsigned long long k = double_to_key(in[i]);
    out[2 * i] = bits_to_double(k);
    out[2 * i + 1] = key_to_double(k);
  } else if constexpr (OP == PK_MATH_FAR_BOUND) {
    Landmark<double> lm = landmark_of_row(in + (int64_t)F_COUNT_FIELDS * i, 0);
    double fk, fi;
    pub_far_bound(lm, fk, fi);
    out[2 * i] = fk;
    out[2 * i + 1] = fi;
  } else if constexpr (OP == PK_MATH_PR_FROM_PARTS) {
    out[i] = pr_from_parts(in[4 * i], in[4 * i + 1], in[4 * i + 2], in[4 * i + 3]);
  } else if constexpr (OP == PK_MATH_EKF_UPDATE) {
    const double* r = in + (int64_t)kEkfIn * i;
    Landmark<double> lm = landmark_of_row(r + 2, (int)r[16]);
    const BlobT<double> z{r[17], r[18], r[19], r[20]};
    const Noise<double> qt = make_noise(r[21], r[22], r[23], r[24], r[25], r[26], r[27]);
    const double zhat0 = r[28];
    const int flags = (int)r[29];
    double prod = r[30];
    const bool immutable = (flags & 1) != 0;
    double logw;
    switch ((flags >> 1) & 7) {
      case 0: logw = ekf_variant<true, false, false>(lm, r[0], r[1], z, qt, immutable, zhat0, prod); break;
      case 1: logw = ekf_variant<true, true, false>(lm, r[0], r[1], z, qt, immutable, zhat0, prod); break;
      case 2: logw = ekf_variant<false, false, false>(lm, r[0], r[1], z, qt, immutable, zhat0, prod); break;
      case 3: logw = ekf_variant<false, true, false>(lm, r[0], r[1], z, qt, immutable, zhat0, prod); break;
      case 4: logw = ekf_variant<true, false, true>(lm, r[0], r[1], z, qt, immutable, zhat0, prod); break;
      case 5: logw = ekf_variant<true, true, true>(lm, r[0], r[1], z, qt, immutable, zhat0, prod); break;
      case 6: logw = ekf_variant<false, false, true>(lm, r[0], r[1], z, qt, immutable, zhat0, prod); break;
      default: logw = ekf_variant<false, true, true>(lm, r[0], r[1], z, qt, immutable, zhat0, prod); break;
    }
    double* o = out + (int64_t)kEkfOut * i;
    o[0] = logw;
    row_of_landmark(lm, o + 1);
    o[15] = (double)lm.count;
    o[16] = prod;
  } else {
    static_assert(OP == PK_MATH_MATCH, "unknown op");
    const double* r = in + (int64_t)kMatchIn * i;
    const double sx = r[0], sy = r[1], heading = r[2], ux = r[21], uy = r[22];
    const Landmark<double> lm = landmark_of_row(r + 3, 0);
    const BlobT<double> z{r[17], r[18], r[19], r[20]};
    const double pse = pk_atan2(lm.my - sy, lm.mx - sx);
    double nx, ny;
    closest_point(lm.mx, lm.my, sx, sy, ux, uy, nx, ny);
    double* o = out + (int64_t)kMatchOut * i;
    o[0] = probability_of_match(lm, sx, sy, heading, z, ux, uy);
    o[1] = prob_position_match(lm, sx, sy, pse, z.bearing, ux, uy);
    o[2] = prob_color_match(lm, z.r, z.g, z.b);
    o[3] = nx;
    o[4] = ny;
  }
}

constexpr int kBearingEkfIn = 32;
template <int WHAT>
__global__ void __launch_bounds__(256) k_probe_bearing(const double* __restrict__ in, double* __restrict__ out, int64_t n) {
  const int64_t i = (int64_t)blockIdx.x * blockDim.x + threadIdx.x;
  if (i >= n) return;
  if constexpr (WHAT == 0) {
    const double* r = in + (int64_t)kMatchIn * i;
    const double sx = r[0], sy = r[1], heading = r[2];
    const Landmark<double> lm = landmark_of_row(r + 3, 0);
    const BlobT<double> z{r[17], r[18], r[19], r[20]};
    double sn, ch, wx, wy;
    sincos(heading, &sn, &ch);
    rotate_ray(r[21], r[22], ch, sn, wx, wy);
    const double pse = pk_atan2(lm.my - sy, lm.mx - sx);
    double nx, ny;
    closest_point<double, kModelBearing>(lm.mx, lm.my, sx, sy, wx, wy, nx, ny);
    double* o = out + (int64_t)kMatchOut * i;
    o[0] = probability_of_match<double, kModelBearing>(lm, sx, sy, heading, z, wx, wy);
    o[1] = prob_position_match<double, kModelBearing>(lm, sx, sy, pse, z.bearing, wx, wy);
    o[2] = prob_color_match(lm, z.r, z.g, z.b);
    o[3] = nx;
    o[4] = ny;
  } else {
    const double* r = in + (int64_t)kBearingEkfIn * i;
    Landmark<double> lm = landmark_of_row(r + 3, (int)r[17]);
    const BlobT<double> z{r[18], r[19], r[20], r[21]};
    const Noise<double> qt = make_noise(r[22], r[23], r[24], r[25], r[26], r[27], r[28]);
    const double pse = r[29];
    const int flags = (int)r[30];
    const bool immutable = (flags & 1) != 0;
    double logw;
    if (flags & 2)
      logw = ekf_update<double, true, kModelBearing>(lm, r[0], r[1], z, qt, immutable, nullptr, &pse, nullptr, r[2]);
    else
      logw = ekf_update<double, true, kModelBearing>(lm, r[0], r[1], z, qt, immutable, nullptr, nullptr, nullptr, r[2]);
    double* o = out + (int64_t)kEkfOut * i;
    o[0] = logw;
    row_of_landmark(lm, o + 1);
    o[15] = (double)lm.count;
    o[16] = r[31];
  }
}

constexpr int kRangeMatchIn = 26, kRangeEkfIn = 33, kRangeEkfOut = 16;
template <int WHAT>
__global__ void __launch_bounds__(256) k_probe_range(const double* __restrict__ in, double* __restrict__ out, int64_t n) {
  const int64_t i = (int64_t)blockIdx.x * blockDim.x + threadIdx.x;
  if (i >= n) return;
  if constexpr (WHAT == 0) {
    const double* r = in + (int64_t)kRangeMatchIn * i;
// ... 188 lines not shown
```

parakeet_slam_amd/csrc/pk_k_step_pub.hip:

```cpp
#include <type_traits>

#include "pk_colour.hpp"
#include "pk_device.hpp"
#include "pk_launch.hpp"
#include "pk_pub_math.hpp"
#include "pk_pub_layout.hpp"

namespace pk {

#ifndef PK_PUB_ABLATE
#define PK_PUB_ABLATE 0
#endif

typedef double Double2 __attribute__((ext_vector_type(2)));
typedef int Int2 __attribute__((ext_vector_type(2)));

__device__ __forceinline__ double pose_scalar(const double* a, int64_t p) {
  return ((const __attribute__((address_space(4))) double*)a)[p];
}
__device__ __forceinline__ int32_t regs_source_pub(const int32_t* src, int64_t p) {
  return ((const __attribute__((address_space(4))) int32_t*)src)[p];
}

struct PubArgs {
// ... 724 lines not shown
  for (int s = 0; s < kPubSlots; ++s) {
    const unsigned e = sw[s] >> 16;
    m[s] = pub[e == 0xFFFFu ? dump : e];
  }
#pragma unroll
  for (int s = 0; s < kPubSlots; ++s) {
    const unsigned e = sw[s] >> 16;
    const bool pos = ((q.st >> (4 * s)) & 1u) != 0u;
    if (pos && (e == 0xFFFFu || m[s] == pub_marker())) q.st |= 4u << (4 * s);
  }
}

#ifndef PK_DIAG_LOG_PER_UPDATE
#define PK_PROD_PTR(p_) (&(p_))
#else
#define PK_PROD_PTR(p_) ((double*)nullptr)
#endif
__device__ __forceinline__ void pub_fold_norms(double& acc, double& prod) {
#ifndef PK_DIAG_LOG_PER_UPDATE
  acc -= 0.25 * log_few_ulp(prod);
  prod = 1.0;
#else
  (void)acc;
  (void)prod;
#endif
}
template <bool TAB = false>
__device__ __forceinline__ double pub_apply(const PubSlots& q, const double* ex, const unsigned short* order, const Noise<double>& qt,
                                            Landmark<double>& lm, bool imm, double sx, double sy, double pse, double* prod = nullptr) {
  double acc = 0.0;
  const unsigned tk = q.st & 0x4444u;
  if (__ballot(tk != 0u) == 0ull) return acc;
  if (__ballot((tk & (tk - 1u)) != 0u) == 0ull) {
    if (tk != 0u) {
      const unsigned w = (tk & 0x0004u) ? q.s[0] : (tk & 0x0040u) ? q.s[1] : (tk & 0x0400u) ? q.s[2] : q.s[3];
      const double* rec = ex + 6 * (w & 0xFFFFu);
      const double2 z01 = *reinterpret_cast<const double2*>(rec);
      const double2 z23 = *reinterpret_cast<const double2*>(rec + 2);
      BlobT<double> z{z01.x, z01.y, z23.x, z23.y};
      acc = ekf_update<double, !TAB>(lm, sx, sy, z, qt, imm, (EkfAux<double>*)nullptr, &pse, prod);
    }
    return acc;
  }
  const unsigned sw[kPubSlots] = {q.s[0], q.s[1], q.s[2], q.s[3]};
  unsigned key[kPubSlots];
#pragma unroll
  for (int s = 0; s < kPubSlots; ++s) {
    const bool take = ((q.st >> (4 * s)) & 4u) != 0u;
    const unsigned t = sw[s] & 0xFFFFu;
    const unsigned o = order[take ? t : 0u];
    key[s] = take ? ((o << 16) | t) : 0xFFFFFFFFu;
  }
  auto cswap = [&](unsigned& u, unsigned& v) {
    const unsigned lo = min(u, v), hi = max(u, v);
    u = lo;
    v = hi;
  };
  cswap(key[0], key[1]);
  cswap(key[2], key[3]);
  cswap(key[0], key[2]);
  cswap(key[1], key[3]);
  cswap(key[1], key[2]);
  bool fresh = true;
#pragma unroll 1
  for (int it = 0; it < kPubSlots; ++it) {
    const unsigned kk = key[0];
    if (__ballot(kk != 0xFFFFFFFFu) == 0ull) break;
    key[0] = key[1];
    key[1] = key[2];
    key[2] = key[3];
    key[3] = 0xFFFFFFFFu;
    if (kk != 0xFFFFFFFFu) {
      const double* rec = ex + 6 * (kk & 0xFFFFu);
      const double2 z01 = *reinterpret_cast<const double2*>(rec);
      const double2 z23 = *reinterpret_cast<const double2*>(rec + 2);
      BlobT<double> z{z01.x, z01.y, z23.x, z23.y};
      acc += ekf_update(lm, sx, sy, z, qt, imm, (EkfAux<double>*)nullptr, fresh ? &pse : (const double*)nullptr, prod);
      fresh = imm;
    }
  }
  return acc;
}

template <bool PRIM = false>
__device__ __forceinline__ double pub_apply_loop(const PubSlots& q, const double* ex, const unsigned short* order, const Noise<double>& qt,
                                            Landmark<double>& lm, bool imm, double sx, double sy, double pse,
                                            const char* ptab = nullptr, size_t pstride = 0, int pidx = 0, unsigned t0 = 0xFFFFu,
                                            double* prod = nullptr) {
  double acc = 0.0;
  unsigned tk = q.st & 0x4444u;
  bool fresh = true;
#pragma unroll 1
  for (int it = 0; it < kPubSlots; ++it) {
    if (__ballot(tk != 0u) == 0ull) break;
    unsigned w, bit;
    if (__ballot((tk & (tk - 1u)) != 0u) == 0ull) {
      w = (tk & 0x0004u) ? q.s[0] : (tk & 0x0040u) ? q.s[1] : (tk & 0x0400u) ? q.s[2] : q.s[3];
      bit = tk;
    } else {
      const unsigned sw[kPubSlots] = {q.s[0], q.s[1], q.s[2], q.s[3]};
      unsigned best = 0xFFFFFFFFu;
      w = 0u;
      bit = 0u;
#pragma unroll
      for (int s = 0; s < kPubSlots; ++s) {
        const bool on = ((tk >> (4 * s)) & 4u) != 0u;
        const unsigned o = order[on ? (sw[s] & 0xFFFFu) : 0u];
        const bool first = on && o < best;
        best = first ? o : best;
        w = first ? sw[s] : w;
        bit = first ? (4u << (4 * s)) : bit;
      }
    }
    const char* rb0 = reinterpret_cast<const char*>(ex);
    size_t rks = 16;
    bool onp = false;
    if constexpr (PRIM) {
      onp = __ballot(tk != 0u && (w & 0xFFFFu) != t0) == 0ull;
      rb0 = onp ? ptab : rb0;
      rks = onp ? pstride : rks;
    }
    if (tk != 0u) {
      const unsigned roff = (PRIM && onp) ? (unsigned)pidx * 16u : (w & 0xFFFFu) * 48u;
      const double2 z01 = *reinterpret_cast<const double2*>(rb0 + roff);
      const double2 z23 = *reinterpret_cast<const double2*>(rb0 + rks + roff);
      BlobT<double> z{z01.x, z01.y, z23.x, z23.y};
      acc += ekf_update(lm, sx, sy, z, qt, imm, (EkfAux<double>*)nullptr, fresh ? &pse : (const double*)nullptr, prod);
      fresh = imm;
    }
    tk &= ~bit;
  }
  return acc;
}

#ifdef PK_STAMPS
__device__ unsigned long long pk_pstamp_wave[8][12];
#define PK_PSTAMP(slot, a, b) pst[slot] += (b) - (a);
void debug_read_pub_wave_stamps(unsigned long long* out, bool reset) {
  (void)hipDeviceSynchronize();
  (void)hipMemcpyFromSymbol(out, HIP_SYMBOL(pk_pstamp_wave), sizeof(unsigned long long) * 96);
  if (reset) {
    unsigned long long z[96] = {0};
    (void)hipMemcpyToSymbol(HIP_SYMBOL(pk_pstamp_wave), z, sizeof(z));
  }
}
void debug_read_pub_stamps(unsigned long long* out, bool reset) {
  (void)hipDeviceSynchronize();
  (void)hipMemcpyFromSymbol(out, HIP_SYMBOL(pk_pstamp_acc), sizeof(unsigned long long) * 16);
  if (reset) {
    unsigned long long z[16] = {0};
    (void)hipMemcpyToSymbol(HIP_SYMBOL(pk_pstamp_acc), z, sizeof(z));
  }
}
#else
#define PK_PSTAMP(slot, a, b)
#endif

typedef const __attribute__((address_space(4))) PubArgs* PubArgsPtr;
__device__ __forceinline__ PubArgsPtr pub_args_now(PubArgsPtr rp) {
  asm volatile("" : "+s"(rp));
  return rp;
}
__device__ __forceinline__ SlotSource pub_slot_source(PubArgsPtr R) {
  return SlotSource{R->ss.map, R->ss.slot_bytes, R->ss.alt, R->ss.alt_stride, R->ss.alt_off};
}
__device__ __forceinline__ Noise<double> pub_noise(PubArgsPtr R) {
  return Noise<double>{R->qt.q00, R->qt.rr, R->qt.rg, R->qt.rb, R->qt.gg, R->qt.gb, R->qt.bb, R->qt.diag};
}

#ifdef PK_DIAG_NO_XCD_RUNS
__device__ __forceinline__ int64_t pub_walk_first(int64_t p_begin, int64_t) { return p_begin + blockIdx.x; }
__device__ __forceinline__ int64_t pub_walk_stride() { return (int64_t)gridDim.x; }
__device__ __forceinline__ int64_t pub_walk_limit(int64_t, int64_t p_end) { return p_end; }
#else
__device__ __forceinline__ int64_t pub_walk_first(int64_t p_begin, int64_t p_end) {
  const unsigned g = gridDim.x, b = blockIdx.x;
  if ((g & 7u) != 0u) return p_begin + b;
  const int64_t chunk = (p_end - p_begin + 7) / 8;
  return p_begin + (int64_t)(b & 7u) * chunk + (int64_t)(b >> 3);
}
__device__ __forceinline__ int64_t pub_walk_stride() { return (gridDim.x & 7u) != 0u ? (int64_t)gridDim.x : (int64_t)(gridDim.x >> 3); }
__device__ __forceinline__ int64_t pub_walk_limit(int64_t p_begin, int64_t p_end) {
  const unsigned g = gridDim.x, b = blockIdx.x;
  if ((g & 7u) != 0u) return p_end;
  const int64_t chunk = (p_end - p_begin + 7) / 8, e = p_begin + (int64_t)((b & 7u) + 1u) * chunk;
  return e < p_end ? e : p_end;
}
#endif
template <int NP, int THREADS, bool TAB>
__device__ __forceinline__ void step_pub_body() {
  static_assert(!TAB || THREADS == 512, "table mode: the 512-lane instances");
  constexpr int kPubThreads = THREADS, kPubWaves = THREADS / kWave;
  extern __shared__ __align__(16) unsigned char smem[];
  __shared__ double red[2][kPubWaves];
  __shared__ int wg_flag[2];
  constexpr bool kPerm = NP == 2 && THREADS == 512;
  __shared__ unsigned short s_perm[kPerm ? 2 * kPubOctets : 1];
  __shared__ unsigned s_rb[kCandSlots];
  constexpr int kUnmWords = THREADS == kPubSmallThreads ? 32 : 96;
  __shared__ unsigned s_ubits[kUnmWords];
  __shared__ unsigned s_kmax;
#ifdef PK_DIAG_NO_LEAN_BODY
  constexpr bool kLean = false;
#else
  constexpr bool kLean = kPerm;
#endif
  __shared__ unsigned s_fallbacks;
#define PK_PUB_L0(q_, t_) (!kPerm ? 2 * kPubThreads * (q_) + 2 * (t_) : (int)(((lw >> (16 + 8 * (q_))) & 0xFFu) << 4) + 2 * ((t_)&7))
  PubArgsPtr rp = (PubArgsPtr)__builtin_amdgcn_kernarg_segment_ptr();
  const int tid0 = threadIdx.x;
  int B, Lp, L, ecap;
  {
    PubArgsPtr R = pub_args_now(rp);
    if (*R->skip != 0u) return;
    B = R->B;
    Lp = R->Lp;
    L = R->L;
    ecap = R->ecap;
  }
  const unsigned Bp = ((unsigned)B + 15u) & ~15u;
  const unsigned o_pub = Bp * 48u, o_binfo = o_pub + ((unsigned)ecap + 2u) * 8u, o_order = o_binfo + Bp * 4u, o_any = o_order + Bp * 2u;
  const unsigned o_imm = o_any + 2u * (Bp + 16u);
  const unsigned o_bnd = o_imm + (unsigned)kPubImmBytes;
  const unsigned dump = (unsigned)ecap, anydump = Bp;
  unsigned G;
  {
    const int tid = tid0;
    PubArgsPtr R = pub_args_now(rp);
    {
      const uint4* gf = R->far;
      float2* bnd = reinterpret_cast<float2*>(smem + o_bnd);
      for (int i = tid; i < Lp; i += kPubThreads) {
        float2 v = make_float2(-3.0e38f, 0.f);
        if (gf) {
          const uint4 hdr = gf[2 * (size_t)i];
          if (hdr.z != 0u) v = make_float2(__uint_as_float(hdr.x), __uint_as_float(hdr.y));
        }
        bnd[i] = v;
      }
    }
    double* ex = reinterpret_cast<double*>(smem);
    const double* gex = R->exact;
    for (int i = tid; i < 6 * B; i += kPubThreads) ex[i] = gex[i];
    unsigned* glist = reinterpret_cast<unsigned*>(smem + o_binfo);
    unsigned short* order = reinterpret_cast<unsigned short*>(smem + o_order);
    const unsigned* gb = R->glist;
    const unsigned short* go = R->order;
    G = gb[B];
    for (int i = tid; i < B; i += kPubThreads) {
      glist[i] = (unsigned)i < G ? gb[i] : 0u;
      order[i] = go[i];
    }
    for (unsigned i = (unsigned)tid; i < 2u * (Bp + 16u) / 4u; i += kPubThreads) reinterpret_cast<unsigned*>(smem + o_any)[i] = 0u;
    const unsigned char* gi = R->immutable;
    for (int i = tid; i < Lp; i += kPubThreads) smem[o_imm + (unsigned)i] = i < L ? gi[i] : (unsigned char)0;
    if constexpr (kPerm) {
      if (tid < 2 * kPubOctets) s_perm[tid] = reinterpret_cast<const unsigned short*>(gb + B + 1)[tid];
    }
    if (tid < kCandSlots) s_rb[tid] = gb[B + 1 + kPubTailWords + tid];
    for (int i = tid; i < kUnmWords; i += kPubThreads) s_ubits[i] = 0u;
    if (tid == 0) {
      wg_flag[0] = 0;
      wg_flag[1] = 0;
      s_kmax = 0u;
      if constexpr (kLean) s_fallbacks = 0u;
    }
  }
  unsigned lean_bits = 0u;
  if constexpr (kLean) {
    PubArgsPtr R = pub_args_now(rp);
    if (R->lean != 0) {
      const unsigned m = R->glist[B + 1 + kPubLeanWord], wave = (unsigned)tid0 / kWave;
      lean_bits = __builtin_amdgcn_readfirstlane(((m >> wave) & 1u) | (((m >> (8u + wave)) & 1u) << 1));
    }
// ... 50 lines not shown
      const unsigned bo_ = (min(k_, D_ - 1u) * 6u * (unsigned)Lp + (unsigned)(lbt_ + j_)) * 8u;   \
      const char* tc_ = reinterpret_cast<const char*>(tb_);                                       \
      const size_t rs_ = (size_t)Lp * 8;                                                          \
      S[2 * (q_) + j_].crr = *reinterpret_cast<const double*>(tc_ + bo_);                         \
      S[2 * (q_) + j_].crg = *reinterpret_cast<const double*>(tc_ + rs_ + bo_);                   \
      S[2 * (q_) + j_].crb = *reinterpret_cast<const double*>(tc_ + 2 * rs_ + bo_);               \
      S[2 * (q_) + j_].cgg = *reinterpret_cast<const double*>(tc_ + 3 * rs_ + bo_);               \
      S[2 * (q_) + j_].cgb = *reinterpret_cast<const double*>(tc_ + 4 * rs_ + bo_);               \
      S[2 * (q_) + j_].cbb = *reinterpret_cast<const double*>(tc_ + 5 * rs_ + bo_);               \
    }                                                                                             \
    if (__ballot(beyond_) != 0ull) {                                                              \
      const Noise<double> qtt_ = pub_noise(pub_args_now(rp));                                     \
      _Pragma("unroll 1") for (int j_ = 0; j_ < 2; ++j_) {                                        \
        Landmark<double>& lmt_ = j_ == 0 ? S[2 * (q_)] : S[2 * (q_) + 1];                         \
        const unsigned k_ = min(colour_level(lmt_.count), D_ + kColourBeyondMax);                 \
        Sym3<double> C_{lmt_.crr, lmt_.crg, lmt_.crb, lmt_.cgg, lmt_.cgb, lmt_.cbb};              \
        _Pragma("unroll 1") for (unsigned kk_ = D_ - 1u; kk_ < k_; ++kk_) C_ = colour_block_step(C_, qtt_); \
        lmt_.crr = C_.a;                                                                          \
        lmt_.crg = C_.b;                                                                          \
        lmt_.crb = C_.c;                                                                          \
        lmt_.cgg = C_.d;                                                                          \
        lmt_.cgb = C_.e;                                                                          \
        lmt_.cbb = C_.f;                                                                          \
      }                                                                                           \
    }                                                                                             \
    asm volatile("" ::: "memory");                                                                \
  }
#define PK_PUB_LOAD_COVS(q_, sslot_, coff_, lb_)                                                  \
  {                                                                                               \
    const double* sf_ = reinterpret_cast<const double*>(sslot_);                                  \
    const int lbq_ = (lb_);                                                                       \
    PK_PUB_ROW(q_, pxx, F_PXX)                                                                    \
    PK_PUB_ROW(q_, pxy, F_PXY)                                                                    \
    PK_PUB_ROW(q_, pyy, F_PYY)                                                                    \
    if constexpr (!TAB) {                                                                         \
      const int* sc_ = reinterpret_cast<const int*>((sslot_) + (coff_));                          \
      PK_PUB_ROW(q_, crr, F_CRR)                                                                  \
      PK_PUB_ROW(q_, crg, F_CRG)                                                                  \
      PK_PUB_ROW(q_, crb, F_CRB)                                                                  \
      PK_PUB_ROW(q_, cgg, F_CGG)                                                                  \
      PK_PUB_ROW(q_, cgb, F_CGB)                                                                  \
      PK_PUB_ROW(q_, cbb, F_CBB)                                                                  \
      const Int2 c_ = *reinterpret_cast<const Int2*>(sc_ + lbq_);                                 \
      S[2 * (q_)].count = c_.x;                                                                   \
      S[2 * (q_) + 1].count = c_.y;                                                               \
      asm volatile("" ::: "memory");                                                              \
    } else {                                                                                      \
      PK_PUB_TAB_ROWS(q_, lbq_)                                                                   \
    }                                                                                             \
  }
#define PK_PUB_LOAD_PAIR(q_, sslot_, coff_, lb_)                                                  \
  {                                                                                               \
    const double* sf_ = reinterpret_cast<const double*>(sslot_);                                  \
    const int* sc_ = reinterpret_cast<const int*>((sslot_) + (coff_));                            \
    const int lbq_ = (lb_);                                                                       \
    if constexpr (TAB) {                                                                          \
      const Int2 c_ = *reinterpret_cast<const Int2*>(sc_ + lbq_);                                 \
      S[2 * (q_)].count = c_.x;                                                                   \
      S[2 * (q_) + 1].count = c_.y;                                                               \
    }                                                                                             \
    PK_PUB_ROW(q_, mx, F_MX)                                                                      \
    PK_PUB_ROW(q_, my, F_MY)                                                                      \
    PK_PUB_ROW(q_, mr, F_MR)                                                                      \
    PK_PUB_ROW(q_, mg, F_MG)                                                                      \
    PK_PUB_ROW(q_, mb, F_MB)                                                                      \
    asm volatile("" ::: "memory");                                                                \
    PK_PUB_ROW(q_, pxx, F_PXX)                                                                    \
    PK_PUB_ROW(q_, pxy, F_PXY)                                                                    \
    PK_PUB_ROW(q_, pyy, F_PYY)                                                                    \
    if constexpr (!TAB) {                                                                         \
      PK_PUB_ROW(q_, crr, F_CRR)                                                                  \
      PK_PUB_ROW(q_, crg, F_CRG)                                                                  \
      PK_PUB_ROW(q_, crb, F_CRB)                                                                  \
      PK_PUB_ROW(q_, cgg, F_CGG)                                                                  \
      PK_PUB_ROW(q_, cgb, F_CGB)                                                                  \
      PK_PUB_ROW(q_, cbb, F_CBB)                                                                  \
      const Int2 c_ = *reinterpret_cast<const Int2*>(sc_ + lbq_);                                 \
      S[2 * (q_)].count = c_.x;                                                                   \
      S[2 * (q_) + 1].count = c_.y;                                                               \
    }                                                                                             \
    asm volatile("" ::: "memory");                                                                \
  }
  Landmark<double> S[2 * NP];
  constexpr int kPipe = 1;
  unsigned lane_word = (unsigned)tid0;
  if constexpr (kPerm) {
    const unsigned octs = (unsigned)(s_perm[tid0 >> 3] & 0xFFu) | ((unsigned)(s_perm[kPubOctets + (tid0 >> 3)] & 0xFFu) << 8);
    lane_word = (unsigned)tid0 | (octs << 16);
  }
  {
    const unsigned lw = lane_word;
    PubArgsPtr R = pub_args_now(rp);
    const unsigned char* ns = pub_slot_source(R).at(nsrc);
    const int coff = R->count_off;
#pragma unroll
    for (int q = 0; q < kPipe; ++q) PK_PUB_LOAD_PAIR(q, ns, coff, min(PK_PUB_L0(q, tid0), Lp - 2))
  }
  for (int64_t p = pub_walk_first(pub_args_now(rp)->p_begin, pub_args_now(rp)->P);; p += pub_walk_stride(), cur ^= 1) {
    unsigned lw = lane_word;
    asm volatile("" : "+v"(lw));
    int tid;
    if constexpr (!kPerm) {
      tid = (int)lw;
    } else {
      tid = (int)(lw & 0xFFFFu);
    }
    double* ex = reinterpret_cast<double*>(smem);
    double* pub = reinterpret_cast<double*>(smem + o_pub);
    const unsigned* glist = reinterpret_cast<const unsigned*>(smem + o_binfo);
    const unsigned short* order = reinterpret_cast<const unsigned short*>(smem + o_order);
    unsigned char* anyc = smem + o_any + (unsigned)cur * (Bp + 16u);
    PubSlots Q[2 * NP];
    double pse[2 * NP];
    bool done;
    unsigned lean_ok = 0u;
    PK_STAMP(s0)
#ifdef PK_STAMPS
    unsigned long long s3 = s0;
#endif
    {
      PubArgsPtr R = pub_args_now(rp);
      const int64_t Pn = pub_walk_limit(R->p_begin, R->P);
      done = p >= Pn;
      const int64_t pc = done ? Pn - 1 : p;
      {
        const SlotSource ss = pub_slot_source(R);
        const unsigned char* sslot = ss.at(nsrc);
        const double sx = pose_scalar(R->x, pc), sy = pose_scalar(R->y, pc), sh = pose_scalar(R->h, pc);
        int lbase[NP];
#pragma unroll
        for (int q = 0; q < NP; ++q) lbase[q] = min(PK_PUB_L0(q, tid), Lp - 2);
        uint4 cref[2 * NP], ccw[2 * NP], cew[2 * NP];
        auto request_cand = [&](int q) {
          PubArgsPtr R2 = pub_args_now(rp);
#ifdef PK_DIAG_TAIL_LISTS
          const int lc = lbase[q];
#else
          const int lc = min(PK_PUB_L0(q, tid), Lp);
#endif
          const uint4* cr = R2->cand + 2 * (size_t)lc;
          const uint4* er = R2->erec + lc;
          cref[2 * q] = cr[0];
          ccw[2 * q] = cr[1];
          cref[2 * q + 1] = cr[2];
          ccw[2 * q + 1] = cr[3];
          cew[2 * q] = er[0];
          cew[2 * q + 1] = er[1];
        };
        request_cand(0);
        asm volatile("" ::: "memory");
        if constexpr (TAB) {
          static_assert(kPipe == 1, "the pairs asked for ahead take their table rows here");
          PK_PUB_TAB_ROWS(0, lbase[0])
        }
        {
          PubArgsPtr R4 = pub_args_now(rp);
          const int64_t pn = p + pub_walk_stride(), pl = pub_walk_limit(R4->p_begin, R4->P);
          nsrc = regs_source_pub(R4->src, pn < pl ? pn : pl - 1);
          asm volatile("" : "+s"(nsrc));
        }
        PK_STAMP(s1)
        PK_PSTAMP(0, s0, s1)
        auto do_pair = [&](auto qc) {
          constexpr int q = decltype(qc)::value;

    const int l0 = PK_PUB_L0(q, tid);
    const PubGateIn gi[2] = {{cref[2 * q], {ccw[2 * q], ccw[2 * q]}, {cew[2 * q], cew[2 * q]}, S[2 * q].mx, S[2 * q].my,
                              S[2 * q].mr, S[2 * q].mg, S[2 * q].mb, l0 < L},
                             {cref[2 * q + 1], {ccw[2 * q + 1], ccw[2 * q + 1]}, {cew[2 * q + 1], cew[2 * q + 1]},
                              S[2 * q + 1].mx, S[2 * q + 1].my, S[2 * q + 1].mr, S[2 * q + 1].mg, S[2 * q + 1].mb,
                              l0 + 1 < L}};
    PubSlots qq[2] = {kPubNoSlots,
                      kPubNoSlots};
    double pp[2] = {0.0, 0.0};
    if constexpr (THREADS == kPubSmallThreads) {
      
#pragma unroll
      for (int j_ = 0; j_ < 2; ++j_) {
        const PubGateIn g1[1] = {gi[j_]};
        PubSlots q1[1] = {qq[j_]};
        double p1[1] = {0.0};
        const Landmark<double>* const l1[1] = {&S[2 * q + j_]};
        if (PK_PUB_ABLATE < 4) pub_gatesN<1>(q1, p1, g1, ex, pub, dump, &wg_flag[cur], sx, sy, sh);
        if (PK_PUB_ABLATE < 3) {
          struct Chk1 {
            const float2* bnd_;
            int l_, L_, Lp_;
            PubArgsPtr rp_;
            double sh;
            __device__ __forceinline__ float2 bnd(int) const { return bnd_[min(l_, Lp_ - 1)]; }
            __device__ __forceinline__ bool has(int) const { return l_ < L_; }
            __device__ __forceinline__ const uint4* far_row() const {
              const uint4* fr = pub_args_now(rp_)->far;
              return fr ? fr + 2 * (size_t)min(l_, Lp_) : nullptr;
            }
          };
          const Chk1 chk{reinterpret_cast<const float2*>(smem + o_bnd), l0 + j_, L, Lp, rp, sh};
          pub_keysN<1, kPubSlots, false, true, 1, Chk1>(q1, l1, p1, ex, pub, dump, anyc, anydump, &wg_flag[cur], sx, sy, nullptr, nullptr, chk);
        }
        qq[j_] = q1[0];
        pp[j_] = p1[0];
      }
    } else {
      const Landmark<double>* const l2[2] = {&S[2 * q], &S[2 * q + 1]};
      bool usual = true;
      if constexpr (kLean) {
        if (((lean_bits >> q) & 1u) != 0u && PK_PUB_ABLATE == 0) {
          const float2* bt = reinterpret_cast<const float2*>(smem + o_bnd);
          const float2 b2[2] = {bt[min(l0, Lp - 1)], bt[min(l0 + 1, Lp - 1)]};
          usual = !pub_lean_pair(qq, pp, gi, l2, b2, ex, anyc, anydump, sx, sy, sh);
          lean_ok |= usual ? 0u : (1u << q);
          if (usual && (tid & (kWave - 1)) == 0) atomicAdd(&s_fallbacks, 1u);
        }
      }
      if (usual) {
      if (PK_PUB_ABLATE < 4) pub_gatesN<2, 1, kPubSlots, true>(qq, pp, gi, ex, pub, dump, &wg_flag[cur], sx, sy, sh);
      PK_STAMP(sk0_)
      if (PK_PUB_ABLATE < 3) {
        struct Chk2 {
          const float2* bnd_;
          unsigned lw, tid_;
          int L_, Lp_;
          PubArgsPtr rp_;
          double sh;
          __device__ __forceinline__ int l0() const { const unsigned lw = this->lw; const int tid = (int)tid_; (void)tid; return PK_PUB_L0(q, tid); }
          __device__ __forceinline__ float2 bnd(int j) const { return bnd_[min(l0() + j, Lp_ - 1)]; }
          __device__ __forceinline__ bool has(int j) const { return l0() + j < L_; }
          __device__ __forceinline__ const uint4* far_row() const {
            const uint4* fr = pub_args_now(rp_)->far;
            return fr ? fr + 2 * (size_t)min(l0(), Lp_) : nullptr;
          }
        };
        const Chk2 chk{reinterpret_cast<const float2*>(smem + o_bnd), lw, (unsigned)tid, L, Lp, rp, sh};
        pub_keysN<2, kPubSlots, false, true, 1, Chk2>(qq, l2, pp, ex, pub, dump, anyc, anydump, &wg_flag[cur], sx, sy, nullptr, nullptr, chk);
        {
          PubArgsPtr R9 = pub_args_now(rp);
          const int lc9 = min(l0, Lp);
          if (pub_refill_slots<2>(qq, R9->cand + 2 * (size_t)lc9, R9->erec + lc9, &wg_flag[cur]))
            pub_keysN<2>(qq, l2, pp, ex, pub, dump, anyc, anydump, &wg_flag[cur], sx, sy);
        }
      }
      PK_STAMP(sk1_)
      PK_PSTAMP(2, sk0_, sk1_)
      }
    }
    Q[2 * q] = qq[0];
    Q[2 * q + 1] = qq[1];
    pse[2 * q] = pp[0];
    pse[2 * q + 1] = pp[1];
  
        };
        if (!done) {
          do_pair(std::integral_constant<int, 0>{});
          if constexpr (NP > 1) {
            if constexpr (TAB) {
              PubArgsPtr R8 = pub_args_now(rp);
              PK_PUB_LOAD_COUNT(1, sslot, R8->count_off, lbase[1])
              asm volatile("" ::: "memory");
            }
            PK_PUB_LOAD_MEANS(1, sslot, lbase[1])
            request_cand(NP - 1);
            {
              asm volatile("" ::: "memory");
              PubArgsPtr R7 = pub_args_now(rp);
              PK_PUB_LOAD_COVS(1, sslot, R7->count_off, lbase[1])
            }
            do_pair(std::integral_constant<int, 1>{});
            if constexpr (TAB) {
              PK_PUB_TAB_ROWS(0, lbase[0])
            }
          }
        }
        PK_STAMP(s2)
        PK_PSTAMP(1, s1, s2)
#ifdef PK_STAMPS
        s3 = s2;
#endif
      }
    }
    lds_barrier();
    PK_STAMP(s4)
    PK_PSTAMP(3, s3, s4)
    if (prev >= 0 && tid == 0) {
      PubArgsPtr R = pub_args_now(rp);
      double tot = red[cur ^ 1][0];
#pragma unroll
      for (int i = 1; i < kPubWaves; ++i) tot += red[cur ^ 1][i];
      double* logw = R->logw;
      const double w = (R->reset ? 0.0 : logw[prev]) + tot;
      logw[prev] = w;
      unsigned long long* gk = R->gmax_key;
      if (gk) atomicMax(gk + (prev & (kGmaxKeys - 1)), double_to_key(w));
      R->src[prev] = (int32_t)prev;
    }
    if (done) break;
    prev = -1;
    double acc;
    {
      int nun = 0;
      for (unsigned w = (unsigned)tid; w < Bp / 4u; w += kPubThreads) {
        const unsigned v = reinterpret_cast<const unsigned*>(anyc)[w];
#pragma unroll
        for (int b = 0; b < 4; ++b) nun += ((int)(4 * w + b) < B && ((v >> (8 * b)) & 0xFFu) == 0u) ? 1 : 0;
      }
      acc = (double)nun * Consts<double>::log_no_match;
      unsigned* anyn = reinterpret_cast<unsigned*>(smem + o_any + (unsigned)(cur ^ 1) * (Bp + 16u));
      for (unsigned w = (unsigned)tid; w < Bp / 4u; w += kPubThreads) anyn[w] = 0u;
      if (tid == 0) wg_flag[cur ^ 1] = 0;
    }
    if (pub_args_now(rp)->unm != nullptr) pub_note_unmatched<THREADS>(tid, anyc, order, B, Bp, s_ubits);
    if (PK_PUB_ABLATE < 2) pub_settle_blobs<THREADS>(tid, glist, G, pub, dump, &wg_flag[cur], s_rb);
    PK_STAMP(s5)
    PK_PSTAMP(4, s4, s5)
    lds_barrier();
    {
      PubArgsPtr Ru = pub_args_now(rp);
      if (Ru->unm != nullptr) pub_store_unmatched<THREADS>(tid, s_ubits, Ru->unm + (size_t)p * Ru->unm_words, Ru->unm_words);
    }
#pragma unroll
    for (int i = 0; i < 2 * NP; ++i)
      if (PK_PUB_ABLATE < 2 && (!kLean || ((lean_ok >> (i / 2)) & 1u) == 0u)) pub_take(Q[i], pub, dump);
    lds_barrier();
    PK_STAMP(s6)
    PK_PSTAMP(5, s5, s6)
    if (wg_flag[cur] && PK_PUB_ABLATE == 0) {
      if (tid == 0) {
        PubArgsPtr R = pub_args_now(rp);
        R->pflag_out[p] = 1;
        atomicAdd(R->n_flagged, 1u);
      }
      {
        PubArgsPtr R6 = pub_args_now(rp);
        const unsigned char* ns = pub_slot_source(R6).at(nsrc);
        const int coff = R6->count_off;
#pragma unroll
        for (int q = 0; q < kPipe; ++q) PK_PUB_LOAD_PAIR(q, ns, coff, min(PK_PUB_L0(q, tid), Lp - 2))
      }
      continue;
    }
    {
      PubArgsPtr R = pub_args_now(rp);
      if (tid == 0) R->pflag_out[p] = 0;
      const Noise<double> qt = pub_noise(R);
      const double sx = pose_scalar(R->x, p), sy = pose_scalar(R->y, p);
      unsigned char* dslot = R->map_dst + (size_t)p * R->ss.slot_bytes;
      double* df = reinterpret_cast<double*>(dslot);
      int* dc = reinterpret_cast<int*>(dslot + R->count_off);
      const unsigned char* immutable = smem + o_imm;
      {
        double nprod = 1.0;
        auto do_apply = [&](auto qc) {
          constexpr int q = decltype(qc)::value;
          const int l0 = PK_PUB_L0(q, tid);
#pragma unroll
          for (int j = 0; j < 2; ++j) {
            const int i = 2 * q + j;
            const bool imm = immutable[min(l0 + j, Lp - 1)] != 0;
            if (PK_PUB_ABLATE < 1)
              acc += THREADS == kPubSmallThreads ? pub_apply_loop(Q[i], ex, order, qt, S[i], imm, sx, sy, pse[i], nullptr, 0, 0, 0xFFFFu, PK_PROD_PTR(nprod))
                                                 : pub_apply<TAB>(Q[i], ex, order, qt, S[i], imm, sx, sy, pse[i], PK_PROD_PTR(nprod));
          }
          if constexpr (q == NP - 1) pub_fold_norms(acc, nprod);
        };
        auto do_store = [&](auto qc) {
          constexpr int q = decltype(qc)::value;
          const int l0 = PK_PUB_L0(q, tid);
          PK_STAMP(su0_)
          if (l0 < Lp) {
#define PK_PUB_STORE(field, F)                                                             \
    {                                                                                        \
      const Double2 v = {S[2 * q].field, S[2 * q + 1].field};                                \
      __builtin_nontemporal_store(v, reinterpret_cast<Double2*>(df + (size_t)F * Lp + l0)); \
    }
            PK_PUB_STORE(mx, F_MX)
            PK_PUB_STORE(my, F_MY)
            PK_PUB_STORE(mr, F_MR)
            PK_PUB_STORE(mg, F_MG)
            PK_PUB_STORE(mb, F_MB)
            PK_PUB_STORE(pxx, F_PXX)
            PK_PUB_STORE(pxy, F_PXY)
            PK_PUB_STORE(pyy, F_PYY)
            if constexpr (!TAB) {
              PK_PUB_STORE(crr, F_CRR)
              PK_PUB_STORE(crg, F_CRG)
              PK_PUB_STORE(crb, F_CRB)
              PK_PUB_STORE(cgg, F_CGG)
              PK_PUB_STORE(cgb, F_CGB)
              PK_PUB_STORE(cbb, F_CBB)
            }
#undef PK_PUB_STORE
            const Int2 c = {S[2 * q].count, S[2 * q + 1].count};
            __builtin_nontemporal_store(c, reinterpret_cast<Int2*>(dc + l0));
          }
          if (q < kPipe) {
            PubArgsPtr R6 = pub_args_now(rp);
            const unsigned char* ns = pub_slot_source(R6).at(nsrc);
            PK_PUB_LOAD_PAIR(q, ns, R6->count_off, min(PK_PUB_L0(q, tid), Lp - 2))
          }
          PK_STAMP(su1_)
          PK_PSTAMP(10, su0_, su1_)
        };
        using Q0 = std::integral_constant<int, 0>;
        using Q1 = std::integral_constant<int, 1>;
        do_apply(Q0{});
        do_store(Q0{});
        if constexpr (NP == 2) {
          do_apply(Q1{});
          do_store(Q1{});
        }
      }
    }
    PK_STAMP(s7)
    PK_PSTAMP(6, s6, s7)
    {
      const double ws = wave_sum(acc);
      if ((tid & (kWave - 1)) == 0) red[cur][tid / kWave] = ws;
      prev = p;
    }
    PK_STAMP(s8)
    PK_PSTAMP(7, s7, s8)
    PK_PSTAMP(8, s0, s8)
#ifdef PK_STAMPS
    pst[9] += 1ull;
#endif
  }
#ifdef PK_STAMPS
  if ((tid0 & 63) == 0)
    for (int k = 0; k < 12; ++k) {
      atomicAdd(&pk_pstamp_acc[k], pst[k]);
      if (THREADS == 512) atomicAdd(&pk_pstamp_wave[tid0 >> 6][k], pst[k]);
    }
#endif
  if constexpr (TAB) {
    if (tid0 == 0) atomicMax(pub_args_now(rp)->ctab_max, s_kmax);
  }
  if constexpr (kLean) {
    if (tid0 == 0 && s_fallbacks != 0u) {
      unsigned* st = const_cast<unsigned*>((const unsigned*)pub_args_now(rp)->stats);
      if (st) atomicAdd(st + 6, s_fallbacks);
    }
  }
}
template <int NP, int THREADS>
__global__ void __launch_bounds__(THREADS, THREADS == 256 ? 3 : 1) k_step_pub(PubArgs a_unused) {
  step_pub_body<NP, THREADS, false>();
}
template <int NP, int THREADS, bool TAB>
__global__ void __launch_bounds__(THREADS, 1) k_step_pub(PubArgs a_unused) {
  static_assert(TAB, "the plain instances are k_step_pub<NP, THREADS>");
  step_pub_body<NP, THREADS, true>();
}

constexpr int kPubBigSlots = 2 * kCandSlots;
constexpr int kPubBigGateSlots = 8;
__device__ __forceinline__ PubSlots pub_keep_positive(const PubSlotsT<kPubBigGateSlots>& g, int* flag) {
  PubSlots o = kPubNoSlots;
#pragma unroll
  for (int k = kPubBigGateSlots - 1; k >= 0; --k) {
    const bool pos = ((g.st >> (4 * k)) & 1u) != 0u;
    o.s[3] = pos ? o.s[2] : o.s[3];
    o.s[2] = pos ? o.s[1] : o.s[2];
    o.s[1] = pos ? o.s[0] : o.s[1];
    o.s[0] = pos ? g.s[k] : o.s[0];
    o.st = pos ? ((o.st << 4) | 1u) : o.st;
  }
  if (flag && __popc(g.st & 0x11111111u) > kPubSlots) *flag = 1;
  o.st &= 0xFFFFu;
  return o;
}
__device__ __forceinline__ uint4 pub_positive_beyond_four(const PubSlotsT<kPubBigGateSlots>& g) {
  unsigned x[4] = {0xFFFFFFFFu, 0xFFFFFFFFu, 0xFFFFFFFFu, 0xFFFFFFFFu};
  int c = 0;
#pragma unroll
  for (int k = 0; k < kPubBigGateSlots; ++k) {
    const bool pos = ((g.st >> (4 * k)) & 1u) != 0u;
    x[0] = (pos && c == 4) ? g.s[k] : x[0];
    x[1] = (pos && c == 5) ? g.s[k] : x[1];
    x[2] = (pos && c == 6) ? g.s[k] : x[2];
    x[3] = (pos && c == 7) ? g.s[k] : x[3];
    c += pos ? 1 : 0;
  }
  return make_uint4(x[0], x[1], x[2], x[3]);
}
__device__ __forceinline__ void pub_park_beyond_four(PubSlots& q, const PubSlotsT<kPubBigGateSlots>& g, uint4* ovf, unsigned n_places, unsigned* counter,
                                                     int* flag) {
  if (__popc(g.st & 0x11111111u) > kPubSlots) {
    const unsigned place = atomicAdd(counter, 1u);
    if (place < n_places) {
      ovf[place] = pub_positive_beyond_four(g);
      q.st |= (place + 1u) << 16;
    } else {
      *flag = 1;
    }
  }
}
__device__ __forceinline__ void pub_take_parked(PubSlots& q, const uint4* ovf, const double* pub, unsigned dump, int* flag) {
  const unsigned pl = q.st >> 16;
  if (__ballot(pl != 0u) == 0ull) return;
  if (pl != 0u) {
    const uint4 s4 = ovf[pl - 1u];
    const unsigned xw[4] = {s4.x, s4.y, s4.z, s4.w};
    double m[4];
#pragma unroll
    for (int x = 0; x < 4; ++x) {
      const unsigned e = xw[x] >> 16;
      m[x] = pub[e == 0xFFFFu ? dump : e];
    }
#pragma unroll
    for (int x = 0; x < 4; ++x) {
      const unsigned e = xw[x] >> 16;
      const bool take = (xw[x] & 0xFFFFu) != 0xFFFFu && (e == 0xFFFFu || m[x] == pub_marker());
      bool placed = !take;
#pragma unroll
      for (int sidx = 0; sidx < kPubSlots; ++sidx) {
        const bool here = !placed && ((q.st >> (4 * sidx)) & 4u) == 0u;
        q.s[sidx] = here ? xw[x] : q.s[sidx];
        q.st = here ? ((q.st & ~(0xFu << (4 * sidx))) | (5u << (4 * sidx))) : q.st;
        placed |= here;
      }
      if (!placed) *flag = 1;
    }
  }
  q.st &= 0xFFFFu;
}
__host__ __device__ inline size_t pub_big_fixed_lds_bytes(int B) {
  const size_t Bp = ((size_t)B + 15) & ~(size_t)15;
  return 16 + Bp * 4 + 2 * (Bp + 16);
}
int step_pub_big_entry_capacity(int B) {
  const size_t fixed = pub_big_fixed_lds_bytes(B);
  if (fixed + 64 * 8 > kMaxDynLds) return 0;
  const size_t e = (kMaxDynLds - fixed) / 8;
  return (int)(e > 65534 ? 65534 : e);
// ... 420 lines not shown
        PK_STAMP(d3)
        PK_PSTAMP(10, d2, d3)
      }
#pragma unroll
      for (int i = 0; i + 2 < 2 * NCH; ++i) {
        Q[i] = Q[i + 2];
        pse[i] = pse[i + 2];
      }
    }
#undef PK_BIG_STORE
#undef PK_BIG_ROWS
#undef PK_BIG_LOAD
    pub_fold_norms(acc, nprod);
    {
      const double ws = wave_sum(acc);
      if ((tid & (kWave - 1)) == 0) red[cur][tid / kWave] = ws;
      prev = p;
    }
#ifdef PK_STAMPS
    {
      PK_STAMP(b5)
      PK_PSTAMP(11, b0, b5)
      pst[9] += 1ull;
    }
#endif
  }
#ifdef PK_STAMPS
  if ((tid0 & 63) == 0)
    for (int k = 0; k < 12; ++k) atomicAdd(&pk_pstamp_wave[tid0 >> 6][k], pst[k]);
#endif
#undef PK_BIG_WAIT_ALL
}

static PubArgs pub_args(const DeviceState& d, const ScanTables& scan, const FastHandoff& fh, const NoiseD& qt, const ObserveExtras& ex,
                        const PubTables& pub, const ParticleRange& range) {
  PubArgs a{};
  fill_state(a, d);
  fill_scan(a, scan, ex, qt);
  a.cand = pub.cand.rec;
  a.far = pub.cand.far;
  a.erec = pub.erec;
  a.glist = pub.glist;
  a.unm = ex.unm;
  a.unm_words = ex.unm_words;
  a.pflag_out = fh.pflag;
  a.n_flagged = fh.n_flagged;
  a.P = range.end(d.P);
  a.p_begin = range.p0;
  return a;
}

void launch_step_pub_big(hipStream_t s, DeviceState& d, const ScanTables& scan, const FastHandoff& fh, const NoiseD& qt,
                         const ObserveExtras& ex, const PubTables& pub, const ParticleRange& range) {
  const int64_t grid_n = persistent_grid(device_cu_count(), 1, range, d.P);
  if (grid_n == 0) return;
  static bool attr_set[kMaxDevices] = {false};
  allow_dynamic_lds(attr_set, kMaxDynLds, k_step_pub_big<3>, k_step_pub_big<5>, k_step_pub_big<6>);
  PubArgs a = pub_args(d, scan, fh, qt, ex, pub, range);
  a.skip = pub.skip_big;
  a.gate4 = pub.gate4;
  a.prim = pub.prim;
  a.stats = pub.stats;
  a.ecap = pub.ecap;
  const size_t lds = step_pub_big_lds_bytes(scan.B, pub.ecap);
  const int nch = (d.lay.Lp + 2 * kPubThreads - 1) / (2 * kPubThreads);
  if (nch <= 3)
    hipLaunchKernelGGL(k_step_pub_big<3>, dim3((unsigned)grid_n), dim3(kPubThreads), lds, s, a);
  else if (nch <= 5)
    hipLaunchKernelGGL(k_step_pub_big<5>, dim3((unsigned)grid_n), dim3(kPubThreads), lds, s, a);
  else
    hipLaunchKernelGGL(k_step_pub_big<6>, dim3((unsigned)grid_n), dim3(kPubThreads), lds, s, a);
}

void launch_step_pub(hipStream_t s, DeviceState& d, const ScanTables& scan, const FastHandoff& fh, const NoiseD& qt,
                     const ObserveExtras& ex, const PubTables& pub, const ParticleRange& range) {
  const bool small = d.lay.Lp <= 2 * kPubSmallThreads;
  const size_t lds = step_pub_lds_bytes(scan.B, pub.ecap, small);
  int per_cu = 1;
  if (small) per_cu = (int)std::min<size_t>(3, std::max<size_t>(1, (160 * 1024 - 1024) / (lds + 256)));
  const int64_t grid_n = persistent_grid(device_cu_count(), per_cu, range, d.P);
  if (grid_n == 0) return;
  static bool attr_set[kMaxDevices] = {false};
  allow_dynamic_lds(attr_set, kMaxDynLds, k_step_pub<1, kPubSmallThreads>, k_step_pub<1, kPubThreads>, k_step_pub<2, kPubThreads>,
                    k_step_pub<1, kPubThreads, true>, k_step_pub<2, kPubThreads, true>);
  PubArgs a = pub_args(d, scan, fh, qt, ex, pub, range);
  a.skip = pub.skip_pub;
  a.stats = ex.lean_stats;
  a.ecap = pub.ecap;
  const bool tab = ex.ctab != nullptr && !small;
  a.ctab = tab ? ex.ctab : nullptr;
  a.ctab_max = ex.ctab_max;
  a.ctab_depth = ex.ctab_depth;
  a.lean = ex.lean;
  if (small)
    hipLaunchKernelGGL((k_step_pub<1, kPubSmallThreads>), dim3((unsigned)grid_n), dim3(kPubSmallThreads), lds, s, a);
  else if (d.lay.Lp <= 2 * kPubThreads) {
    if (tab)
      hipLaunchKernelGGL((k_step_pub<1, kPubThreads, true>), dim3((unsigned)grid_n), dim3(kPubThreads), lds, s, a);
    else
      hipLaunchKernelGGL((k_step_pub<1, kPubThreads>), dim3((unsigned)grid_n), dim3(kPubThreads), lds, s, a);
  } else {
    if (tab)
      hipLaunchKernelGGL((k_step_pub<2, kPubThreads, true>), dim3((unsigned)grid_n), dim3(kPubThreads), lds, s, a);
    else
      hipLaunchKernelGGL((k_step_pub<2, kPubThreads>), dim3((unsigned)grid_n), dim3(kPubThreads), lds, s, a);
  }
}

#include "pk_k_step_duo.inl"

}
```

parakeet_slam_amd/csrc/pk_kernels.hpp:

```cpp
#pragma once
#include <cmath>
#include <hip/hip_runtime.h>

#include <cstdint>

#include "pk_layout.hpp"

namespace pk {

struct NoiseD {
  double q00, rr, rg, rb, gg, gb, bb;
};

struct DeviceState {
  int64_t P;
  MapLayout lay;
  double* x[2];
  double* y[2];
  double* h[2];
  double* logw[2];
  int32_t* src[2];
  int cur;
  unsigned char* map[2];
  int mcur;
// ... 75 lines not shown
  double inv_h;
  int G[3];
  int ncell;
  float thr32;
  float thrb32;
  float thrb32w;
};
constexpr double kGridCell = 17.5;
constexpr int kGridMax = 16;
__host__ __device__ inline size_t grid_cs_bytes(int ncell) { return ((size_t)(ncell + 1) * 2 + 15) & ~(size_t)15; }
size_t blob_grid_table_bytes(int ncell, int B, int n9);
size_t assoc_grid_lds_bytes(int ncell, int B, int n9);
constexpr size_t kMaxDynLds = 156 * 1024;
constexpr int kMaxDevices = 64;
inline bool first_time_on_this_device(bool (&done)[kMaxDevices]) {
  int dev = 0;
  if (hipGetDevice(&dev) != hipSuccess || dev < 0 || dev >= kMaxDevices) return true;
  if (done[dev]) return false;
  done[dev] = true;
  return true;
}
inline int device_cu_count() {
  static int n_cu[kMaxDevices] = {0};
  int dev = 0;
  const bool known = hipGetDevice(&dev) == hipSuccess && dev >= 0 && dev < kMaxDevices;
  if (known && n_cu[dev] > 0) return n_cu[dev];
  int n = 256;
  hipDeviceProp_t prop;
  if (known && hipGetDeviceProperties(&prop, dev) == hipSuccess && prop.multiProcessorCount > 0) n = prop.multiProcessorCount;
  (void)hipGetLastError();
  if (known) n_cu[dev] = n;
  return n;
}
struct ScanTables {
  int B = 0;
  const double* blobs = nullptr;
  const double* dir = nullptr;
  BlobGrid grid{};
  int n9 = 0;
  const unsigned char* tables = nullptr;
  const double* exact = nullptr;
  const unsigned short* order = nullptr;
  const double* rng = nullptr;
  const double* rng_cell = nullptr;
};
struct ParticleRange {
  int64_t p0 = 0, p1 = -1;
  int reserve_cus = 0;
  int64_t end(int64_t P) const { return p1 < 0 ? P : p1; }
};
inline int64_t persistent_grid(int n_cu, int per_cu, const ParticleRange& r, int64_t P) {
  const int64_t n = r.end(P) - r.p0;
  if (P <= 0 || n <= 0) return 0;
  const int64_t grid = (int64_t)(n_cu - (r.reserve_cus > 0 && r.reserve_cus < n_cu ? r.reserve_cus : 0)) * per_cu;
  return grid > n ? n : grid;
}
void launch_assoc_brute(hipStream_t s, DeviceState& d, const ScanTables& scan, int32_t* ids_dev, int model = 0, double q00 = 0.0);
struct FastHandoff {
  uint4* lmpass = nullptr;
  int slots = 4;
  bool flags_only = false;
  unsigned char* bcount = nullptr;
  unsigned char* pflag = nullptr;
  unsigned* n_flagged = nullptr;
  int32_t* row_of = nullptr;
  unsigned* row_next = nullptr;
  int64_t row_cap = 0;
  bool retry = false;
};
constexpr int kGmaxKeys = 256;
struct ObserveExtras {
  const unsigned char* only_flagged = nullptr;
  const unsigned* n_flagged = nullptr;
  int sweep_only_value = 0;
  bool flip = true;
  bool reset = false;
  unsigned long long* gmax_key = nullptr;
  bool single_sightings = false;
  unsigned* unm = nullptr;
  int unm_words = 0;
  const double* ctab = nullptr;
  int ctab_depth = 0;
  unsigned* ctab_max = nullptr;
  int model = 0;
  int lean = 0;
  unsigned* lean_stats = nullptr;
  const double* rng = nullptr;
  const double* dlogw = nullptr;
};
struct ColourTable {
  const double* tab = nullptr;
  int depth = 0;
};
void launch_colour_table(hipStream_t s, const double* base_dev, double* tab_dev, int depth, int Lp, const NoiseD& qt);
void launch_colour_rows(hipStream_t s, DeviceState& d, const ColourTable& ct, const NoiseD& qt, const ParticleRange& range = ParticleRange(),
                        const unsigned char* pflag_dev = nullptr, const unsigned* n_flagged_dev = nullptr);
void launch_colour_counts_any(hipStream_t s, DeviceState& d, unsigned* any_dev);
constexpr int kFastSlots = 4;
constexpr int kSweepSlots = 8;
constexpr int kFastMaxL = 512;
void launch_assoc_grid_bearing(hipStream_t s, DeviceState& d, const ScanTables& scan, int32_t* ids_dev, bool finalize, double q00 = 0.0);
size_t observe_fast_lds_bytes(int B);
void launch_observe_fast(hipStream_t s, DeviceState& d, const ScanTables& scan, const FastHandoff& fh, const NoiseD& qt,
                         const ObserveExtras& ex = ObserveExtras());
struct KnownChains {
  const int32_t* first = nullptr;
  const int32_t* next = nullptr;
  int n_unmatched = 0;
};
void launch_observe(hipStream_t s, DeviceState& d, const ScanTables& scan, const KnownChains& known, const NoiseD& qt,
                    const ObserveExtras& ex = ObserveExtras());
void launch_observe(hipStream_t s, DeviceState& d, const ScanTables& scan, int32_t* ids_dev, const NoiseD& qt,
                    const ObserveExtras& ex = ObserveExtras());
struct ProposeLaunch {
  const double* blobs_dev = nullptr;
  const double* blobdir_dev = nullptr;
  const double* rng_dev = nullptr;
  int B = 0;
  int32_t* ids_dev = nullptr;
  bool ids_shared = false;
  const double* z_dev = nullptr;
  uint64_t seed = 0, draw = 0;
  bool odom = false;
  double u[3] = {0, 0, 0};
  double sigma[3] = {0, 0, 0};
  NoiseD qt{};
  double* xi_dev = nullptr;
  double* dlogw_dev = nullptr;
  int32_t* used_dev = nullptr;
};
void launch_propose(hipStream_t s, DeviceState& d, const ProposeLaunch& q);
struct SweepPlan {
  int grid = 0;
  size_t lds = 0;
  int qcap = 0;
  size_t results_per_wg = 0;
};
SweepPlan observe_sweep_plan(const DeviceState& d, int B);
void launch_observe_sweep(hipStream_t s, DeviceState& d, const ScanTables& scan, const FastHandoff& fh, const NoiseD& qt,
                          const ObserveExtras& ex, const SweepPlan& plan, uint4* results_dev);
size_t fused_lds_bytes(int ncell, int B, int n9, bool exact_lds = false);
constexpr size_t kFusedMaxLds = 78 * 1024;
void launch_step_fused(hipStream_t s, DeviceState& d, const ScanTables& scan, const FastHandoff& fh, const NoiseD& qt,
                       const ObserveExtras& ex, const unsigned* pub_skipped_dev = nullptr);
constexpr int kCandSlots = 8;
constexpr int kCandSpare = 2;
constexpr double kCandBearing = 0.2;
constexpr double kCandColour = 1.5;
struct CandTable {
  const uint4* rec = nullptr;
  const uint4* brec = nullptr;
  const unsigned* over = nullptr;
  const unsigned* skip_cand = nullptr;
  const unsigned* n_stray = nullptr;
  const uint4* far = nullptr;
  int slots = kCandSlots;
};
void launch_assoc_grid(hipStream_t s, DeviceState& d, const ScanTables& scan, int32_t* ids_dev, bool finalize, const FastHandoff& fh,
                       const CandTable& cand = CandTable());
struct CandidatesLaunch {
  uint4* rec;
  unsigned* over;
  int slots = kCandSlots;
  int64_t ref_particle = 0;
  const double* pose_sums4 = nullptr;
  const double* pose_part = nullptr;
  unsigned* bcnt = nullptr;
  uint4* brec = nullptr;
  unsigned char* npass = nullptr;
  uint4* far = nullptr;
  ColourTable ct;
  const NoiseD* qt = nullptr;
};
void launch_candidates(hipStream_t s, DeviceState& d, const ScanTables& scan, const CandidatesLaunch& c);
constexpr int kRegsMaxL = 2048;
size_t regs_lds_bytes(int ncell, int B, int n9);
size_t regs_cand_lds_bytes(int Lp, int B);
// ... 229 lines not shown
```

parakeet_slam_amd/csrc/pk_math.hpp:

```cpp
#pragma once
#include <hip/hip_runtime.h>

namespace pk {

template <typename T>
struct Consts;
template <>
struct Consts<double> {
  static constexpr double two_pi = 6.283185307179586476925286766559;
  static constexpr double half_pi = 1.5707963267948966192313216916398;
  static constexpr double log_two_pi = 1.8378770664093454835606594728112;
  static constexpr double log_no_match = -2.3025850929940456840179914546844;
};

template <typename T>
struct Landmark {
  T mx, my, mr, mg, mb;
  T pxx, pxy, pyy;
  T crr, crg, crb, cgg, cgb, cbb;
  int count;
};

constexpr int kPotentialBit = 0x40000000;
__device__ __forceinline__ void count_update(int& count) {
// ... 165 lines not shown
  T pse = pk_atan2(f.my - sy, f.mx - sx);
  T delb = z.bearing - (pse - heading);
  if constexpr (MODEL == kModelBearing) delb = wrap_angle(delb);
  if (fabs(delb) > T(0.5)) return T(0);
  T cd = color_distance2(f.mr, f.mg, f.mb, z.r, z.g, z.b);
  if (fabs(cd) > T(300)) return T(0);
  T bp = T(500) * prob_position_match<T, MODEL>(f, sx, sy, pse, z.bearing, ux, uy);
  T cp = T(500) * prob_color_match(f, z.r, z.g, z.b);
  return bp * cp / T(250000);
}

__device__ __forceinline__ double log_few_ulp(double x) {
  if (!(x > 2.3e-308 && x < 1.7e308)) return log(x);
  int e = 0;
  double m = frexp(x, &e);
  if (m < 0.70710678118654752440) {
    m *= 2.0;
    e -= 1;
  }
  const double s = (m - 1.0) / (m + 1.0);
  const double z = s * s;
  double p = 1.0 / 21.0;
  p = fma_k(p, z, 1.0 / 19.0);
  p = fma_k(p, z, 1.0 / 17.0);
  p = fma_k(p, z, 1.0 / 15.0);
  p = fma_k(p, z, 1.0 / 13.0);
  p = fma_k(p, z, 1.0 / 11.0);
  p = fma_k(p, z, 1.0 / 9.0);
  p = fma_k(p, z, 1.0 / 7.0);
  p = fma_k(p, z, 1.0 / 5.0);
  p = fma_k(p, z, 1.0 / 3.0);
  const double lm = 2.0 * s + 2.0 * s * (z * p);
  const double ed = (double)e;
  return ed * 0.69314718055994528623 + (ed * 2.3190468138462995584e-17 + lm);
}

__device__ __forceinline__ double pr_from_parts(double det2, double det3, double num2, double num3) {
  const double maha2 = num2 / det2, maha3 = num3 / det3;
  const double bp = 500.0 * exp(-0.5 * (2.0 * Consts<double>::log_two_pi + log_few_ulp(det2) + maha2));
  const double cp = 500.0 * exp(-0.5 * (3.0 * Consts<double>::log_two_pi + log_few_ulp(det3) + maha3));
  return bp * cp / 250000.0;
}

template <typename T>
struct EkfAux {
  T zhat0, h0, h1;
  T q00;
  Sym3<T> qc;
  T k0, k1;
  T kc[9];
};

template <typename T>
__device__ __forceinline__ Sym3<T> colour_block_update(const Sym3<T>& C, const Sym3<T>& qci, const Noise<T>& qt) {
  const T crr = C.a, crg = C.b, crb = C.c, cgg = C.d, cgb = C.e, cbb = C.f;
  T nrr, nrg, nrb, ngg, ngb, nbb;
  T m00 = qci.a * crr + qci.b * crg + qci.c * crb;
  T m01 = qci.a * crg + qci.b * cgg + qci.c * cgb;
  T m02 = qci.a * crb + qci.b * cgb + qci.c * cbb;
  T m11 = qci.b * crg + qci.d * cgg + qci.e * cgb;
  T m12 = qci.b * crb + qci.d * cgb + qci.e * cbb;
  T m22 = qci.c * crb + qci.e * cgb + qci.f * cbb;
  if (qt.diag) {
    nrr = qt.rr * m00;
    nrg = qt.rr * m01;
    nrb = qt.rr * m02;
    ngg = qt.gg * m11;
    ngb = qt.gg * m12;
    nbb = qt.bb * m22;
  } else {
    T m10 = qci.b * crr + qci.d * crg + qci.e * crb;
    T m20 = qci.c * crr + qci.e * crg + qci.f * crb;
    T m21 = qci.c * crg + qci.e * cgg + qci.f * cgb;
    nrr = crr - (crr * m00 + crg * m10 + crb * m20);
    nrg = crg - (crr * m01 + crg * m11 + crb * m21);
    nrb = crb - (crr * m02 + crg * m12 + crb * m22);
    ngg = cgg - (crg * m01 + cgg * m11 + cgb * m21);
    ngb = cgb - (crg * m02 + cgg * m12 + cgb * m22);
    nbb = cbb - (crb * m02 + cgb * m12 + cbb * m22);
  }
  return Sym3<T>{nrr, nrg, nrb, ngg, ngb, nbb};
}
template <typename T>
__device__ __forceinline__ Sym3<T> colour_block_step(const Sym3<T>& C, const Noise<T>& qt) {
  Sym3<T> qc{C.a + qt.rr, C.b + qt.rg, C.c + qt.rb, C.d + qt.gg, C.e + qt.gb, C.f + qt.bb};
  T detc;
  Sym3<T> qci = sym3_inverse(qc, detc);
  return colour_block_update(C, qci, qt);
}
template <typename T, bool COLOUR = true, int MODEL = kModelReference>
__device__ __forceinline__ T ekf_update(Landmark<T>& f, T sx, T sy, const BlobT<T>& z,
                                        const Noise<T>& qt, bool immutable,
                                        EkfAux<T>* aux = nullptr, const T* zhat0_known = nullptr, T* fro_prod = nullptr,
                                        T heading = T(0)) {
  T dx = f.mx - sx, dy = f.my - sy;
  T zhat0 = zhat0_known ? *zhat0_known : pk_atan2(dy, dx);
  if constexpr (MODEL == kModelBearing) zhat0 = zhat0 - heading;
  T q = dx * dx + dy * dy;
  T h0, h1;
  if (q == T(0)) {
    h0 = T(0);
    h1 = T(0);
  } else {
    T iq = T(1) / q;
    h0 = dy * iq;
    h1 = dx * iq;
    if constexpr (MODEL == kModelBearing) h0 = -h0;
  }
  T a0 = f.pxx * h0 + f.pxy * h1;
  T a1 = f.pxy * h0 + f.pyy * h1;
  T q00 = h0 * a0 + h1 * a1 + qt.q00;
  Sym3<T> qc{f.crr + qt.rr, f.crg + qt.rg, f.crb + qt.rb, f.cgg + qt.gg, f.cgb + qt.gb, f.cbb + qt.bb};
  T detc;
  Sym3<T> qci = sym3_inverse(qc, detc);
  T iq00 = T(1) / q00;

  T d0 = z.bearing - zhat0;
  if constexpr (MODEL == kModelBearing) d0 = wrap_angle(d0);
  T d1 = z.r - f.mr, d2 = z.g - f.mg, d3 = z.b - f.mb;

  T fro2 = q00 * q00 + qc.a * qc.a + qc.d * qc.d + qc.f * qc.f +
           T(2) * (qc.b * qc.b + qc.c * qc.c + qc.e * qc.e);
  T v0 = qci.a * d1 + qci.b * d2 + qci.c * d3;
  T v1 = qci.b * d1 + qci.d * d2 + qci.e * d3;
  T v2 = qci.c * d1 + qci.e * d2 + qci.f * d3;
  T maha = d0 * d0 * iq00 + (d1 * v0 + d2 * v1 + d3 * v2);
  T logw;
  if constexpr (MODEL == kModelBearing) {
    logw = T(-2) * Consts<T>::log_two_pi - T(0.5) * log_few_ulp(q00 * detc) - T(0.5) * maha;
    if (f.count & kPotentialBit) logw = (T)Consts<double>::log_no_match;
  } else if (fro_prod) {
    logw = T(-0.5) * Consts<T>::log_two_pi - T(0.5) * maha;
    static_assert(sizeof(T) == 8, "fro_prod: the test of the product is one of a double");
    const bool potential = (f.count & kPotentialBit) != 0;
    const T old = *fro_prod;
    const T raw = old * fro2;
    T p = potential ? old : raw;
    if (potential) logw = (T)Consts<double>::log_no_match;
    constexpr int kNotPositiveNormal = 0x3FF & ~0x100;
    if (__builtin_expect(!potential && __builtin_amdgcn_class((double)raw, kNotPositiveNormal), 0)) {
      const int e = __builtin_amdgcn_frexp_exp((double)old) + __builtin_amdgcn_frexp_exp((double)fro2);
      p = (T)(__builtin_amdgcn_frexp_mant((double)old) * __builtin_amdgcn_frexp_mant((double)fro2));
      logw -= T(0.25 * 0.69314718055994530941723212145818) * T(e);
    }
    *fro_prod = p;
  } else {
    logw = T(-0.5) * (Consts<T>::log_two_pi + T(0.5) * log_few_ulp(fro2)) - T(0.5) * maha;
    if (f.count & kPotentialBit) logw = (T)Consts<double>::log_no_match;
  }
  T k0 = a0 * iq00, k1 = a1 * iq00;

  if (aux) {
    aux->zhat0 = zhat0;
    aux->h0 = h0;
    aux->h1 = h1;
    aux->q00 = q00;
    aux->qc = qc;
    aux->k0 = k0;
    aux->k1 = k1;
    const T C[3][3] = {{f.crr, f.crg, f.crb}, {f.crg, f.cgg, f.cgb}, {f.crb, f.cgb, f.cbb}};
    const T I[3][3] = {{qci.a, qci.b, qci.c}, {qci.b, qci.d, qci.e}, {qci.c, qci.e, qci.f}};
    for (int i = 0; i < 3; ++i)
      for (int j = 0; j < 3; ++j) aux->kc[i * 3 + j] = C[i][0] * I[0][j] + C[i][1] * I[1][j] + C[i][2] * I[2][j];
  }

  if (!immutable) {
    f.mx += k0 * d0;
    f.my += k1 * d0;
    T nr = f.mr + (f.crr * v0 + f.crg * v1 + f.crb * v2);
    T ng = f.mg + (f.crg * v0 + f.cgg * v1 + f.cgb * v2);
    T nb = f.mb + (f.crb * v0 + f.cgb * v1 + f.cbb * v2);
    T nxx = f.pxx - k0 * a0;
    T nxy = f.pxy - T(0.5) * (k0 * a1 + k1 * a0);
    T nyy = f.pyy - k1 * a1;
    Sym3<T> nc{f.crr, f.crg, f.crb, f.cgg, f.cgb, f.cbb};
    if constexpr (COLOUR) nc = colour_block_update(nc, qci, qt);
    f.mr = nr;
    f.mg = ng;
    f.mb = nb;
    f.pxx = nxx;
    f.pxy = nxy;
    f.pyy = nyy;
    if constexpr (COLOUR) {
      f.crr = nc.a;
      f.crg = nc.b;
      f.crb = nc.c;
      f.cgg = nc.d;
      f.cgb = nc.e;
      f.cbb = nc.f;
    }
    count_update(f.count);
  }
  return logw;
}

template <typename T>
__device__ __forceinline__ void motion_model(T& x, T& y, T& h, T v, T w, T dt, T n0, T n1, T n2) {
// ... 26 lines not shown
```

Before: 29.79 billion.

## Use wave-uniform precomputed colour covariance levels when all landmarks share initial colour covariance

When every landmark starts with an identical colour covariance, a single-thread kernel precomputes, for each update count, the colour block, its noise-added form and its inverse. A new kernel variant checks per wave whether all landmarks sit at the same level and then reads these records through the scalar/constant address space, skipping the per-lane 3x3 inverse and the per-landmark table row loads. Waves with mixed levels or multiple updates fall back to the existing table path. It adds an extra kernel instance, ballots and atomics for stats, and relies on the uniform-initialisation property detected at upload.

```diff
diff --git a/include/parakeet_slam.h b/include/parakeet_slam.h
--- a/include/parakeet_slam.h
+++ b/include/parakeet_slam.h
@@ -260,6 +260,7 @@
 int pk_timings(pk_filter* f, double ms[PK_T_COUNT], int64_t launches[PK_T_COUNT]);
 int pk_observe_bytes(const pk_filter* f, int32_t num_blobs, int64_t* algorithmic, int64_t* moved);
 int pk_colour_table_stats(pk_filter* f, int64_t out[4]);
+int pk_colour_uniform_stats(pk_filter* f, int64_t out[4]);
 enum {
   PK_ROUTE_NONE = 0,
   PK_ROUTE_KNOWN_IDS = 1,
diff --git a/parakeet_slam_amd/_lib.py b/parakeet_slam_amd/_lib.py
--- a/parakeet_slam_amd/_lib.py
+++ b/parakeet_slam_amd/_lib.py
@@ -174,6 +174,7 @@
     "pk_timings": (C.c_int, [_h, _dp, _lp]),
     "pk_observe_bytes": (C.c_int, [_h, C.c_int32, _lp, _lp]),
     "pk_colour_table_stats": (C.c_int, [_h, _lp]),
+    "pk_colour_uniform_stats": (C.c_int, [_h, _lp]),
     "pk_observe_route": (C.c_int, [_h]),
     "pk_download_sources": (C.c_int, [_h, _ip]),
     "pk_observe_flagged": (C.c_int, [_h, _lp, _lp]),
@@ -795,6 +796,11 @@
         check(self._lib.pk_colour_table_stats(self._h, lptr(a)))
         return dict(zip(("engaged", "depth", "scans", "materialisations"), (int(v) for v in a)))
 
+    def colour_uniform_stats(self):
+        a = np.zeros(4, dtype=np.int64)
+        check(self._lib.pk_colour_uniform_stats(self._h, lptr(a)))
+        return dict(zip(("eligible", "engaged", "scalar_pairs", "fallbacks"), (int(v) for v in a)))
+
     def grow_enable(self, preset_landmarks, reading_capacity=64, pair_threshold=30.0):
         check(self._lib.pk_grow_enable(self._h, int(preset_landmarks), int(reading_capacity), float(pair_threshold)))
 
diff --git a/parakeet_slam_amd/csrc/pk_api.hip b/parakeet_slam_amd/csrc/pk_api.hip
--- a/parakeet_slam_amd/csrc/pk_api.hip
+++ b/parakeet_slam_amd/csrc/pk_api.hip
@@ -370,11 +370,19 @@
   f->ct_built = false;
   f->ct_updated = false;
   f->ct_eligible = false;
+  f->cu_eligible = false;
+  f->cu_built = false;
+  f->cu_last = false;
   if (!f->dense && lay.Lp > 2 * kPubSmallThreads && L <= kRegsMaxL) {
     if ((rc = dev_lazy(f, &f->ct_base, (size_t)6 * lay.Lp))) return rc;
     PK_HIP(hipMemcpyAsync(f->ct_base, slot.data() + (size_t)F_CRR * lay.Lp * sizeof(double), (size_t)6 * lay.Lp * sizeof(double),
                           hipMemcpyHostToDevice, f->stream));
     f->ct_eligible = true;
+    const double* rows = reinterpret_cast<const double*>(slot.data()) + (size_t)F_CRR * lay.Lp;
+    bool same = L > 0;
+    for (int r = 0; r < 6 && same; ++r)
+      for (int l = 1; l < L && same; ++l) same = memcmp(&rows[(size_t)r * lay.Lp + l], &rows[(size_t)r * lay.Lp], sizeof(double)) == 0;
+    f->cu_eligible = same;
   }
   PK_HIP(hipStreamSynchronize(f->stream));
   f->src_identity = true;
diff --git a/parakeet_slam_amd/csrc/pk_api_observe.hip b/parakeet_slam_amd/csrc/pk_api_observe.hip
--- a/parakeet_slam_amd/csrc/pk_api_observe.hip
+++ b/parakeet_slam_amd/csrc/pk_api_observe.hip
@@ -1,3 +1,4 @@
+#include "pk_colour.hpp"
 #include "pk_filter.hpp"
 
 static int host_word(pk_filter* f, unsigned** p) {
@@ -69,6 +70,9 @@
   *untouched = f->ct_seen[1] == 0u;
   return PK_OK;
 }
+static bool cu_state_ok(const pk_filter* f) {
+  return f->opt.colour_uniform != 0 && f->cu_eligible && f->cu_built && f->ct_tab;
+}
 static int ct_engage(pk_filter* f) {
   int rc;
   const int Lp = f->d.lay.Lp;
@@ -80,11 +84,16 @@
   if (!f->ct_tab || f->ct_depth != depth) {
     PK_HIP(hipStreamSynchronize(f->stream));
     dev_free(f, &f->ct_tab);
-    if ((rc = dev_alloc(f, &f->ct_tab, (size_t)depth * 6 * Lp))) return rc;
+    if ((rc = dev_alloc(f, &f->ct_tab, (size_t)depth * (6 * (size_t)Lp + kColourLevelDoubles)))) return rc;
     f->ct_depth = depth;
   }
   f->ct_qt = f->qt;
   launch_colour_table(f->stream, f->ct_base, f->ct_tab, depth, Lp, f->ct_qt);
+  f->cu_built = false;
+  if (f->cu_eligible) {
+    launch_colour_levels(f->stream, f->ct_base, const_cast<double*>(colour_levels_behind(f->ct_tab, depth, Lp)), depth, Lp, f->ct_qt);
+    f->cu_built = true;
+  }
   PK_HIP(hipMemsetAsync(f->ct_max_dev, 0, 16, f->stream));
   *f->ct_seen = 0u;
   PK_LAUNCH_CHECK("colour table");
@@ -399,6 +408,10 @@
     e1.ctab = f->ct_tab;
     e1.ctab_depth = f->ct_depth;
     e1.ctab_max = f->ct_max_dev;
+    if (cu_state_ok(f)) {
+      e1.ctab_uniform = true;
+      if (range.p0 == 0) (void)hipMemsetAsync(f->ct_max_dev + 2, 0, 2 * sizeof(unsigned), f->stream);
+    }
   }
   e1.lean = f->opt.pub_lean;
   e1.lean_stats = ctl_pub_stats(f);
@@ -556,6 +569,7 @@
       (void)hipGetLastError();
       f->colour_rows_valid = false;
       f->ct_engaged = true;
+      f->cu_last = cu_state_ok(f);
       f->ct_scans += 1;
     }
     if ((rc = onepass_finish(f, al, ex, pub.cand))) return rc;
@@ -817,6 +831,23 @@
   return PK_OK;
 }
 
+int pk_colour_uniform_stats(pk_filter* f, int64_t out[4]) {
+  if (!f || !out) return fail(PK_ERR_INVALID, "pk_colour_uniform_stats: NULL argument");
+  int rc;
+  if ((rc = use_device(f))) return rc;
+  out[0] = f->cu_eligible ? 1 : 0;
+  out[1] = f->ct_engaged && f->cu_last ? 1 : 0;
+  out[2] = out[3] = 0;
+  if (out[1] && f->ct_max_dev) {
+    unsigned w[2] = {0u, 0u};
+    PK_HIP(hipMemcpyAsync(w, f->ct_max_dev + 2, sizeof(w), hipMemcpyDeviceToHost, f->stream));
+    PK_HIP(hipStreamSynchronize(f->stream));
+    out[2] = w[0];
+    out[3] = w[1];
+  }
+  return PK_OK;
+}
+
 int pk_colour_table_stats(pk_filter* f, int64_t out[4]) {
   if (!f || !out) return fail(PK_ERR_INVALID, "pk_colour_table_stats: NULL argument");
   out[0] = f->ct_engaged ? 1 : 0;
diff --git a/parakeet_slam_amd/csrc/pk_colour.hpp b/parakeet_slam_amd/csrc/pk_colour.hpp
--- a/parakeet_slam_amd/csrc/pk_colour.hpp
+++ b/parakeet_slam_amd/csrc/pk_colour.hpp
@@ -17,4 +17,18 @@
   return C;
 }
 
+constexpr int kColourLevelDoubles = 24;
+__host__ __device__ inline const double* colour_levels_behind(const double* tab, int depth, int Lp) {
+  return tab + (size_t)depth * 6 * (size_t)Lp;
 }
+__device__ __forceinline__ ColourPre<double> colour_level_record(const double* clev, unsigned level) {
+  const __attribute__((address_space(4))) double* r =
+      (const __attribute__((address_space(4))) double*)clev + (size_t)level * kColourLevelDoubles;
+  ColourPre<double> p;
+  p.C = Sym3<double>{r[0], r[1], r[2], r[3], r[4], r[5]};
+  p.qc = Sym3<double>{r[6], r[7], r[8], r[9], r[10], r[11]};
+  p.qci = Sym3<double>{r[12], r[13], r[14], r[15], r[16], r[17]};
+  return p;
+}
+
+}
diff --git a/parakeet_slam_amd/csrc/pk_filter.hpp b/parakeet_slam_amd/csrc/pk_filter.hpp
--- a/parakeet_slam_amd/csrc/pk_filter.hpp
+++ b/parakeet_slam_amd/csrc/pk_filter.hpp
@@ -120,6 +120,7 @@
   int colour_table_depth = 1024;
   int colour_table_margin = -1;
   int colour_table = -1;
+  int colour_uniform = -1;
   int map_sum_groups = 0;
   int map_match_groups = 0;
 };
@@ -161,6 +162,7 @@
      "colour_table_depth: 8 .. 32768 levels (the table stays below 4 GB: 32-bit offsets)"},
     {"colour_table_margin", &Options::colour_table_margin, Take::Range, -1, 32768,
      "colour_table_margin: -1 (auto), 0 (the host never leaves the mode for the table's end) or levels"},
+    {"colour_uniform", &Options::colour_uniform, Take::Range, -1, 1, "colour_uniform: -1 (auto), 0 (off) or 1 (as auto)"},
     {"map_sum_groups", &Options::map_sum_groups, Take::Range, 0, 1024, "map_sum_groups: 0 (chosen from the shape) .. 1024"},
     {"map_match_groups", &Options::map_match_groups, Take::Range, 0, 1024, "map_match_groups: 0 (chosen from the shape) .. 1024"},
 };
@@ -258,6 +260,9 @@
   unsigned* ct_max_dev = nullptr;
   unsigned* ct_seen = nullptr;
   int64_t ct_scans = 0, ct_whole = 0;
+  bool cu_eligible = false;
+  bool cu_built = false;
+  bool cu_last = false;
   bool adopt_local_done = false;
   int pub_ecap = 0;
   uint4* sweep_results = nullptr;
diff --git a/parakeet_slam_amd/csrc/pk_k_colour.hip b/parakeet_slam_amd/csrc/pk_k_colour.hip
--- a/parakeet_slam_amd/csrc/pk_k_colour.hip
+++ b/parakeet_slam_amd/csrc/pk_k_colour.hip
@@ -26,6 +26,28 @@
 void launch_colour_table(hipStream_t s, const double* base_dev, double* tab_dev, int depth, int Lp, const NoiseD& qt) {
   if (depth <= 0 || Lp <= 0) return;
   hipLaunchKernelGGL(k_colour_table, dim3((unsigned)((Lp + 63) / 64)), dim3(64), 0, s, base_dev, tab_dev, depth, Lp,
+                     make_noise(qt.q00, qt.rr, qt.rg, qt.rb, qt.gg, qt.gb, qt.bb));
+}
+
+__global__ void __launch_bounds__(64) k_colour_levels(const double* base, double* clev, int depth, int Lp, Noise<double> qt) {
+  if (blockIdx.x != 0 || threadIdx.x != 0) return;
+  Sym3<double> C{base[0], base[(size_t)Lp], base[2 * (size_t)Lp], base[3 * (size_t)Lp], base[4 * (size_t)Lp], base[5 * (size_t)Lp]};
+#pragma unroll 1
+  for (int k = 0; k < depth; ++k) {
+    Sym3<double> qc, qci;
+    const Sym3<double> next = colour_block_step(C, qt, &qc, &qci);
+    double* r = clev + (size_t)k * kColourLevelDoubles;
+    const double v[kColourLevelDoubles] = {C.a,   C.b,   C.c,   C.d,   C.e,   C.f,   qc.a, qc.b, qc.c, qc.d, qc.e, qc.f,
+                                           qci.a, qci.b, qci.c, qci.d, qci.e, qci.f, 0.0,  0.0,  0.0,  0.0,  0.0,  0.0};
+#pragma unroll
+    for (int i = 0; i < kColourLevelDoubles; ++i) r[i] = v[i];
+    C = next;
+  }
+}
+
+void launch_colour_levels(hipStream_t s, const double* base_dev, double* clev_dev, int depth, int Lp, const NoiseD& qt) {
+  if (depth <= 0 || Lp <= 0) return;
+  hipLaunchKernelGGL(k_colour_levels, dim3(1), dim3(64), 0, s, base_dev, clev_dev, depth, Lp,
                      make_noise(qt.q00, qt.rr, qt.rg, qt.rb, qt.gg, qt.gb, qt.bb));
 }
 
diff --git a/parakeet_slam_amd/csrc/pk_k_mathprobe.hip b/parakeet_slam_amd/csrc/pk_k_mathprobe.hip
--- a/parakeet_slam_amd/csrc/pk_k_mathprobe.hip
+++ b/parakeet_slam_amd/csrc/pk_k_mathprobe.hip
@@ -91,6 +91,12 @@
     double prod = r[30];
     const bool immutable = (flags & 1) != 0;
     double logw;
+    if (flags & 16) {
+      ColourPre<double> pre;
+      pre.C = Sym3<double>{lm.crr, lm.crg, lm.crb, lm.cgg, lm.cgb, lm.cbb};
+      (void)colour_block_step(pre.C, qt, &pre.qc, &pre.qci);
+      logw = ekf_update<double, false, kModelReference, true>(lm, r[0], r[1], z, qt, immutable, nullptr, &zhat0, &prod, 0.0, &pre);
+    } else
     switch ((flags >> 1) & 7) {
       case 0: logw = ekf_variant<true, false, false>(lm, r[0], r[1], z, qt, immutable, zhat0, prod); break;
       case 1: logw = ekf_variant<true, true, false>(lm, r[0], r[1], z, qt, immutable, zhat0, prod); break;
diff --git a/parakeet_slam_amd/csrc/pk_k_step_pub.hip b/parakeet_slam_amd/csrc/pk_k_step_pub.hip
--- a/parakeet_slam_amd/csrc/pk_k_step_pub.hip
+++ b/parakeet_slam_amd/csrc/pk_k_step_pub.hip
@@ -830,6 +830,31 @@
   return acc;
 }
 
+__device__ __forceinline__ bool pub_apply_pre(const PubSlots& q, const double* ex, const Noise<double>& qt, Landmark<double>& lm, bool imm,
+                                              double sx, double sy, double pse, const ColourPre<double>& pre, double* prod, double& ret) {
+  ret = 0.0;
+  const unsigned tk = q.st & 0x4444u;
+  if (__ballot(tk != 0u) == 0ull) return true;
+  if (__ballot((tk & (tk - 1u)) != 0u) != 0ull) {
+    lm.crr = pre.C.a;
+    lm.crg = pre.C.b;
+    lm.crb = pre.C.c;
+    lm.cgg = pre.C.d;
+    lm.cgb = pre.C.e;
+    lm.cbb = pre.C.f;
+    return false;
+  }
+  if (tk != 0u) {
+    const unsigned w = (tk & 0x0004u) ? q.s[0] : (tk & 0x0040u) ? q.s[1] : (tk & 0x0400u) ? q.s[2] : q.s[3];
+    const double* rec = ex + 6 * (w & 0xFFFFu);
+    const double2 z01 = *reinterpret_cast<const double2*>(rec);
+    const double2 z23 = *reinterpret_cast<const double2*>(rec + 2);
+    BlobT<double> z{z01.x, z01.y, z23.x, z23.y};
+    ret = ekf_update<double, false, kModelReference, true>(lm, sx, sy, z, qt, imm, (EkfAux<double>*)nullptr, &pse, prod, 0.0, &pre);
+  }
+  return true;
+}
+
 template <bool PRIM = false>
 __device__ __forceinline__ double pub_apply_loop(const PubSlots& q, const double* ex, const unsigned short* order, const Noise<double>& qt,
                                             Landmark<double>& lm, bool imm, double sx, double sy, double pse,
@@ -935,9 +960,10 @@
   return e < p_end ? e : p_end;
 }
 #endif
-template <int NP, int THREADS, bool TAB>
+template <int NP, int THREADS, bool TAB, bool UNI = false>
 __device__ __forceinline__ void step_pub_body() {
   static_assert(!TAB || THREADS == 512, "table mode: the 512-lane instances");
+  static_assert(!UNI || TAB, "the uniform colour sequence is a sub-mode of the table's");
   constexpr int kPubThreads = THREADS, kPubWaves = THREADS / kWave;
   extern __shared__ __align__(16) unsigned char smem[];
   __shared__ double red[2][kPubWaves];
@@ -1154,6 +1180,7 @@
     asm volatile("" ::: "memory");                                                                \
   }
   Landmark<double> S[2 * NP];
+  unsigned n_uni = 0u, n_tab = 0u;
   constexpr int kPipe = 1;
   unsigned lane_word = (unsigned)tid0;
   if constexpr (kPerm) {
@@ -1186,6 +1213,20 @@
     double pse[2 * NP];
     bool done;
     unsigned lean_ok = 0u;
+    unsigned ulev[NP];
+#pragma unroll
+    for (int q = 0; q < NP; ++q) ulev[q] = ~0u;
+    auto uni_level = [&](auto qc, int l0) -> unsigned {
+      constexpr int q = decltype(qc)::value;
+      const unsigned D = (unsigned)pub_args_now(rp)->ctab_depth;
+      const bool h0 = l0 < L, h1 = l0 + 1 < L;
+      const unsigned k0 = colour_level(S[2 * q].count), k1 = colour_level(S[2 * q + 1].count);
+      const unsigned long long m = __ballot(h0);
+      if (m == 0ull) return 0u;
+      const unsigned kf = (unsigned)__builtin_amdgcn_readlane((int)k0, __builtin_ctzll(m));
+      const bool other = (h0 && k0 != kf) || (h1 && k1 != kf);
+      return (__ballot(other) == 0ull && kf < D) ? kf : ~0u;
+    };
     PK_STAMP(s0)
 #ifdef PK_STAMPS
     unsigned long long s3 = s0;
@@ -1338,8 +1379,20 @@
               PK_PUB_LOAD_COVS(1, sslot, R7->count_off, lbase[1])
             }
             do_pair(std::integral_constant<int, 1>{});
-            if constexpr (TAB) {
+            if constexpr (UNI) {
+              ulev[0] = uni_level(std::integral_constant<int, 0>{}, PK_PUB_L0(0, tid));
+              ulev[1] = uni_level(std::integral_constant<int, 1>{}, PK_PUB_L0(1, tid));
+            } else if constexpr (TAB) {
               PK_PUB_TAB_ROWS(0, lbase[0])
+            }
+          } else if constexpr (UNI) {
+            ulev[0] = uni_level(std::integral_constant<int, 0>{}, PK_PUB_L0(0, tid));
+          }
+          if constexpr (UNI) {
+#pragma unroll
+            for (int q = 0; q < NP; ++q) {
+              n_uni = (unsigned)__builtin_amdgcn_readfirstlane((int)(n_uni + (ulev[q] != ~0u ? 1u : 0u)));
+              n_tab = (unsigned)__builtin_amdgcn_readfirstlane((int)(n_tab + (ulev[q] != ~0u ? 0u : 1u)));
             }
           }
         }
@@ -1428,7 +1481,20 @@
           for (int j = 0; j < 2; ++j) {
             const int i = 2 * q + j;
             const bool imm = immutable[min(l0 + j, Lp - 1)] != 0;
-            if (PK_PUB_ABLATE < 1)
+            bool usual = true;
+            if constexpr (UNI) {
+              if (j == 0 && ulev[q] == ~0u) {
+                PK_PUB_TAB_ROWS(q, min(l0, Lp - 2))
+              }
+              if (ulev[q] != ~0u && PK_PUB_ABLATE < 1) {
+                PubArgsPtr Rc = pub_args_now(rp);
+                const ColourPre<double> pre = colour_level_record(colour_levels_behind(Rc->ctab, Rc->ctab_depth, Lp), ulev[q]);
+                double ret;
+                usual = !pub_apply_pre(Q[i], ex, qt, S[i], imm, sx, sy, pse[i], pre, PK_PROD_PTR(nprod), ret);
+                acc += ret;
+              }
+            }
+            if (PK_PUB_ABLATE < 1 && usual)
               acc += THREADS == kPubSmallThreads ? pub_apply_loop(Q[i], ex, order, qt, S[i], imm, sx, sy, pse[i], nullptr, 0, 0, 0xFFFFu, PK_PROD_PTR(nprod))
                                                  : pub_apply<TAB>(Q[i], ex, order, qt, S[i], imm, sx, sy, pse[i], PK_PROD_PTR(nprod));
           }
@@ -1506,6 +1572,13 @@
   if constexpr (TAB) {
     if (tid0 == 0) atomicMax(pub_args_now(rp)->ctab_max, s_kmax);
   }
+  if constexpr (UNI) {
+    unsigned* cs = pub_args_now(rp)->ctab_max;
+    if (__builtin_amdgcn_mbcnt_hi(~0u, __builtin_amdgcn_mbcnt_lo(~0u, 0u)) == 0u) {
+      atomicAdd(cs + 2, n_uni);
+      atomicAdd(cs + 3, n_tab);
+    }
+  }
   if constexpr (kLean) {
     if (tid0 == 0 && s_fallbacks != 0u) {
       unsigned* st = const_cast<unsigned*>((const unsigned*)pub_args_now(rp)->stats);
@@ -1521,6 +1594,10 @@
 __global__ void __launch_bounds__(THREADS, 1) k_step_pub(PubArgs a_unused) {
   static_assert(TAB, "the plain instances are k_step_pub<NP, THREADS>");
   step_pub_body<NP, THREADS, true>();
+}
+template <int NP>
+__global__ void __launch_bounds__(kPubThreads, 1) k_step_pub_uni(PubArgs a_unused) {
+  step_pub_body<NP, kPubThreads, true, true>();
 }
 
 constexpr int kPubBigSlots = 2 * kCandSlots;
@@ -2107,7 +2184,7 @@
   if (grid_n == 0) return;
   static bool attr_set[kMaxDevices] = {false};
   allow_dynamic_lds(attr_set, kMaxDynLds, k_step_pub<1, kPubSmallThreads>, k_step_pub<1, kPubThreads>, k_step_pub<2, kPubThreads>,
-                    k_step_pub<1, kPubThreads, true>, k_step_pub<2, kPubThreads, true>);
+                    k_step_pub<1, kPubThreads, true>, k_step_pub<2, kPubThreads, true>, k_step_pub_uni<1>, k_step_pub_uni<2>);
   PubArgs a = pub_args(d, scan, fh, qt, ex, pub, range);
   a.skip = pub.skip_pub;
   a.stats = ex.lean_stats;
@@ -2117,15 +2194,20 @@
   a.ctab_max = ex.ctab_max;
   a.ctab_depth = ex.ctab_depth;
   a.lean = ex.lean;
+  const bool uni = tab && ex.ctab_uniform;
   if (small)
     hipLaunchKernelGGL((k_step_pub<1, kPubSmallThreads>), dim3((unsigned)grid_n), dim3(kPubSmallThreads), lds, s, a);
   else if (d.lay.Lp <= 2 * kPubThreads) {
-    if (tab)
+    if (uni)
+      hipLaunchKernelGGL(k_step_pub_uni<1>, dim3((unsigned)grid_n), dim3(kPubThreads), lds, s, a);
+    else if (tab)
       hipLaunchKernelGGL((k_step_pub<1, kPubThreads, true>), dim3((unsigned)grid_n), dim3(kPubThreads), lds, s, a);
     else
       hipLaunchKernelGGL((k_step_pub<1, kPubThreads>), dim3((unsigned)grid_n), dim3(kPubThreads), lds, s, a);
   } else {
-    if (tab)
+    if (uni)
+      hipLaunchKernelGGL(k_step_pub_uni<2>, dim3((unsigned)grid_n), dim3(kPubThreads), lds, s, a);
+    else if (tab)
       hipLaunchKernelGGL((k_step_pub<2, kPubThreads, true>), dim3((unsigned)grid_n), dim3(kPubThreads), lds, s, a);
     else
       hipLaunchKernelGGL((k_step_pub<2, kPubThreads>), dim3((unsigned)grid_n), dim3(kPubThreads), lds, s, a);
diff --git a/parakeet_slam_amd/csrc/pk_kernels.hpp b/parakeet_slam_amd/csrc/pk_kernels.hpp
--- a/parakeet_slam_amd/csrc/pk_kernels.hpp
+++ b/parakeet_slam_amd/csrc/pk_kernels.hpp
@@ -181,6 +181,7 @@
   const double* ctab = nullptr;
   int ctab_depth = 0;
   unsigned* ctab_max = nullptr;
+  bool ctab_uniform = false;
   int model = 0;
   int lean = 0;
   unsigned* lean_stats = nullptr;
@@ -192,6 +193,7 @@
   int depth = 0;
 };
 void launch_colour_table(hipStream_t s, const double* base_dev, double* tab_dev, int depth, int Lp, const NoiseD& qt);
+void launch_colour_levels(hipStream_t s, const double* base_dev, double* clev_dev, int depth, int Lp, const NoiseD& qt);
 void launch_colour_rows(hipStream_t s, DeviceState& d, const ColourTable& ct, const NoiseD& qt, const ParticleRange& range = ParticleRange(),
                         const unsigned char* pflag_dev = nullptr, const unsigned* n_flagged_dev = nullptr);
 void launch_colour_counts_any(hipStream_t s, DeviceState& d, unsigned* any_dev);
diff --git a/parakeet_slam_amd/csrc/pk_math.hpp b/parakeet_slam_amd/csrc/pk_math.hpp
--- a/parakeet_slam_amd/csrc/pk_math.hpp
+++ b/parakeet_slam_amd/csrc/pk_math.hpp
@@ -271,17 +271,25 @@
   return Sym3<T>{nrr, nrg, nrb, ngg, ngb, nbb};
 }
 template <typename T>
-__device__ __forceinline__ Sym3<T> colour_block_step(const Sym3<T>& C, const Noise<T>& qt) {
+__device__ __forceinline__ Sym3<T> colour_block_step(const Sym3<T>& C, const Noise<T>& qt, Sym3<T>* qc_out = nullptr,
+                                                     Sym3<T>* qci_out = nullptr) {
   Sym3<T> qc{C.a + qt.rr, C.b + qt.rg, C.c + qt.rb, C.d + qt.gg, C.e + qt.gb, C.f + qt.bb};
   T detc;
   Sym3<T> qci = sym3_inverse(qc, detc);
+  if (qc_out) *qc_out = qc;
+  if (qci_out) *qci_out = qci;
   return colour_block_update(C, qci, qt);
 }
-template <typename T, bool COLOUR = true, int MODEL = kModelReference>
+template <typename T>
+struct ColourPre {
+  Sym3<T> C, qc, qci;
+};
+template <typename T, bool COLOUR = true, int MODEL = kModelReference, bool PRE = false>
 __device__ __forceinline__ T ekf_update(Landmark<T>& f, T sx, T sy, const BlobT<T>& z,
                                         const Noise<T>& qt, bool immutable,
                                         EkfAux<T>* aux = nullptr, const T* zhat0_known = nullptr, T* fro_prod = nullptr,
-                                        T heading = T(0)) {
+                                        T heading = T(0), const ColourPre<T>* pre = nullptr) {
+  static_assert(!PRE || (!COLOUR && MODEL == kModelReference), "PRE: the colour block stays as it is, the reference model");
   T dx = f.mx - sx, dy = f.my - sy;
   T zhat0 = zhat0_known ? *zhat0_known : pk_atan2(dy, dx);
   if constexpr (MODEL == kModelBearing) zhat0 = zhat0 - heading;
@@ -299,9 +307,22 @@
   T a0 = f.pxx * h0 + f.pxy * h1;
   T a1 = f.pxy * h0 + f.pyy * h1;
   T q00 = h0 * a0 + h1 * a1 + qt.q00;
-  Sym3<T> qc{f.crr + qt.rr, f.crg + qt.rg, f.crb + qt.rb, f.cgg + qt.gg, f.cgb + qt.gb, f.cbb + qt.bb};
+  Sym3<T> qc, qci;
   T detc;
-  Sym3<T> qci = sym3_inverse(qc, detc);
+  if constexpr (PRE) {
+    f.crr = pre->C.a;
+    f.crg = pre->C.b;
+    f.crb = pre->C.c;
+    f.cgg = pre->C.d;
+    f.cgb = pre->C.e;
+    f.cbb = pre->C.f;
+    qc = pre->qc;
+    qci = pre->qci;
+    detc = T(0);
+  } else {
+    qc = Sym3<T>{f.crr + qt.rr, f.crg + qt.rg, f.crb + qt.rb, f.cgg + qt.gg, f.cgb + qt.gb, f.cbb + qt.bb};
+    qci = sym3_inverse(qc, detc);
+  }
   T iq00 = T(1) / q00;
 
   T d0 = z.bearing - zhat0;
```

Result: slower. 27.42 billion (-8.0%).
